# eMWu94/ReMo3D

Hardware: AMD Instinct MI355X
Metric: measurement points/sec (3D benchmark model) (higher is better)
Workload: dtype f64

## Files before the change

include/remo3d_hip_debug.h:

```cpp
#ifndef REMO3D_HIP_DEBUG_H
#define REMO3D_HIP_DEBUG_H

#include "remo3d_hip.h"

#ifdef __cplusplus
extern "C" {
#endif

int remo_debug_stream(remo_ctx_t *ctx, int64_t bytes, double *read_gbs, double *copy_gbs);
int remo_debug_clock(remo_ctx_t *ctx, double *gfma_per_wave);
int remo_debug_cache_gather(remo_ctx_t *ctx, int64_t bytes, double *gbs);
int remo_debug_device(remo_ctx_t *ctx, int64_t *out8);
int remo_debug_xcc(remo_ctx_t *ctx, int32_t *out, int32_t nblocks);


int remo_debug_patch_phases(remo_ctx_t *ctx, remo_batch_t *batch, int32_t fp32 , double *out16);

int remo_debug_patch_phases_p(remo_ctx_t *ctx, remo_batch_t *batch, int32_t fp32, double *out16);

int remo_debug_grid_barrier(remo_ctx_t *ctx, int32_t nblocks, int32_t nbar, double *out3);

int remo_debug_sens_timing(remo_ctx_t *ctx, double *out2);
int remo_debug_sens_group_timing(remo_ctx_t *ctx, double *out4);
int remo_debug_field_timing(remo_ctx_t *ctx, double *out2);
int remo_debug_point_location(remo_ctx_t *ctx);
int remo_debug_secondary_timing(remo_ctx_t *ctx, double *ms);

int remo_debug_tune(int32_t key, int32_t value);

#ifdef __cplusplus
}
#endif
#endif
```

remo3d_amd/_lib.py:

```python
from __future__ import annotations

import ctypes as C
import os

import numpy as np

_HERE = os.path.dirname(os.path.abspath(__file__))
LIB_PATH = os.environ.get("REMO_LIB") or os.path.join(_HERE, "libremo3d_hip.so")
REMO_MAX_RHS = 8


class RemoMesh(C.Structure):
    _fields_ = [("dim", C.c_int32), ("n_nodes", C.c_int64), ("coords", C.POINTER(C.c_double)),
                ("n_elems", C.c_int64), ("conn", C.POINTER(C.c_int32)), ("mat", C.POINTER(C.c_int32)),
                ("n_bfacets", C.c_int64), ("bconn", C.POINTER(C.c_int32)), ("bdirichlet", C.POINTER(C.c_uint8))]


class RemoOpts(C.Structure):
    _fields_ = [("preconditioner", C.c_int32), ("condense", C.c_int32), ("maxsteps", C.c_int32),
                ("check_every", C.c_int32), ("rtol", C.c_double), ("time_kernels", C.c_int32),
                ("coarse_degree", C.c_int32), ("coarse_ratio", C.c_int32), ("precision", C.c_int32), ("inner_digits", C.c_int32),
                ("serialize_solves", C.c_int32), ("op", C.c_int32), ("coarse", C.c_int32), ("assemble", C.c_int32), ("quadrature", C.c_int32)]


class RemoStats(C.Structure):
    _fields_ = [("n_dof", C.c_int64), ("n_free", C.c_int64), ("nnz", C.c_int64), ("n_edges", C.c_int64),
                ("n_faces", C.c_int64), ("n_rhs", C.c_int32), ("max_iterations", C.c_int32),
                ("iterations", C.c_int32 * REMO_MAX_RHS), ("relres", C.c_double * REMO_MAX_RHS),
                ("ms_symbolic", C.c_double), ("ms_h2d", C.c_double), ("ms_assemble", C.c_double),
                ("ms_solve", C.c_double), ("ms_eval", C.c_double), ("ms_total", C.c_double),
                ("spmv_ms", C.c_double), ("spmv_launches", C.c_int64), ("spmv_bytes", C.c_double),
                ("pcg_steps", C.c_int64), ("spmv_ms_raw", C.c_double), ("event_overhead_ms", C.c_double),
                ("refinement_cycles", C.c_int64), ("op_used", C.c_int32), ("coarse_used", C.c_int32),
                ("assembled", C.c_int32), ("patch_rounds", C.c_int32)]

    def as_dict(self):
        d = {}
        for name, _ in self._fields_:
            v = getattr(self, name)
            d[name] = list(v) if hasattr(v, "__len__") else v
        return d


class RemoJob(C.Structure):
    _dp, _ip = C.POINTER(C.c_double), C.POINTER(C.c_int32)
    _fields_ = [("size", C.c_uint32), ("tensor", C.c_int32), ("n_mat", C.c_int32), ("sigma", _dp),
                ("n_rhs", C.c_int32), ("src_ptr", _ip), ("src_p", _dp), ("src_I", _dp),
                ("eval_ptr", _ip), ("eval_p", _dp), ("u_out", _dp),
                ("n_fun", C.c_int32), ("fun_rhs", _ip), ("fun_ptr", _ip), ("fun_p", _dp), ("fun_w", _dp), ("J_out", _dp), ("dJ_out", _dp),
                ("n_group", C.c_int32), ("group", _ip), ("dJg_out", _dp),
                ("warm", C.c_void_p),
                ("n_pts", C.c_int32), ("pts", _dp), ("n_frhs", C.c_int32), ("field_rhs", _ip), ("u_f", _dp), ("grad_f", _dp), ("J_f", _dp),
                ("elem_f", _ip)]


class RemoJobSecondary(C.Structure):
    _fields_ = RemoJob._fields_ + [("secondary", C.c_int32), ("sec_quad", C.c_int32), ("sec_radius", C.c_double),
                                   ("sec_sigma0", C.POINTER(C.c_double))]


EXPORTS = ["remo_abi_version", "remo_opts_default", "remo_ctx_create", "remo_ctx_destroy", "remo_last_error",
           "remo_solve_batch", "remo_solve_batch_tensor", "remo_solve_batch_sens", "remo_solve_batch_sens_tensor", "remo_solve_batch_sens_groups", "remo_solve_batch_sens_groups_tensor",
           "remo_solve_batch_field", "remo_solve_batch_field_tensor", "remo_batch_field", "remo_host_field_element",
           "remo_warm_create", "remo_warm_destroy", "remo_warm_clear", "remo_warm_info", "remo_solve_batch_sens_warm", "remo_solve_batch_sens_warm_tensor", "remo_batch_create", "remo_batch_create_tensor", "remo_batch_run", "remo_batch_fetch", "remo_batch_destroy",
           "remo_batch_eval", "remo_batch_get_system", "remo_batch_get_vectors", "remo_batch_apply_coarse", "remo_batch_spmv",
           "remo_host_element_matrix", "remo_host_element_matrix_tensor", "remo_host_sens_element", "remo_host_factor_error", "remo_host_symbolic",
           "remo_solve_job", "remo_batch_create_job", "remo_host_point_shapes", "remo_host_secondary_element"]
DEBUG_EXPORTS = ["remo_debug_stream", "remo_debug_clock", "remo_debug_device", "remo_debug_cache_gather", "remo_debug_xcc", "remo_debug_tune", "remo_debug_patch_phases", "remo_debug_patch_phases_p", "remo_debug_grid_barrier", "remo_debug_sens_timing", "remo_debug_sens_group_timing", "remo_debug_field_timing", "remo_debug_point_location", "remo_debug_secondary_timing"]

JOB_HEAD = ["n_mat", "sigma", "n_rhs", "src_ptr", "src_p", "src_I", "eval_ptr", "eval_p"]
_SENS = ["u_out", "n_fun", "fun_rhs", "fun_ptr", "fun_p", "fun_w"]
LEGACY_MEMBERS = {"": ["u_out"],
                  "_sens": _SENS + ["J_out", "dJ_out"],
                  "_sens_warm": _SENS + ["J_out", "dJ_out", "warm"],
                  "_sens_groups": _SENS + ["n_group", "group", "J_out", "dJ_out", "dJg_out"],
                  "_field": ["u_out", "n_pts", "pts", "n_frhs", "field_rhs", "u_f", "grad_f", "J_f", "elem_f"]}


def legacy_args(job, kind=None):
    return [getattr(job, name) for name in JOB_HEAD + (LEGACY_MEMBERS[kind] if kind is not None else [])]


_lib = None


def load():
    global _lib
    if _lib is not None:
        return _lib
    if not os.path.exists(LIB_PATH):
        raise ImportError(f"{LIB_PATH} is missing: build it with `make -C remo3d_amd/csrc` "
                          "(or __graft_entry__.build()); remo3d_amd has no CPU fallback")
    L = C.CDLL(LIB_PATH)
    dp, ip, i64p, u8p = C.POINTER(C.c_double), C.POINTER(C.c_int32), C.POINTER(C.c_int64), C.POINTER(C.c_uint8)
    vp = C.c_void_p
    L.remo_abi_version.restype = C.c_int
    L.remo_opts_default.argtypes = [C.POINTER(RemoOpts)]
    L.remo_ctx_create.restype = vp
    L.remo_ctx_create.argtypes = [C.c_int]
    L.remo_ctx_destroy.argtypes = [vp]
    L.remo_last_error.restype = C.c_char_p
    L.remo_last_error.argtypes = [vp]
    member = dict(RemoJob._fields_)
    batch_args = [vp, C.POINTER(RemoMesh)] + [member[name] for name in JOB_HEAD]
    for kind, names in LEGACY_MEMBERS.items():
        for entry in (getattr(L, "remo_solve_batch" + kind), getattr(L, "remo_solve_batch" + kind + "_tensor")):
            entry.restype = C.c_int
            entry.argtypes = batch_args + [member[name] for name in names] + [C.POINTER(RemoOpts), C.POINTER(RemoStats)]
    L.remo_warm_create.restype = vp
    L.remo_warm_create.argtypes = [C.c_int]
    L.remo_warm_destroy.restype = None
    L.remo_warm_destroy.argtypes = [vp]
    L.remo_warm_clear.restype = None
    L.remo_warm_clear.argtypes = [vp]
    L.remo_warm_info.restype = C.c_int
    L.remo_warm_info.argtypes = [vp, i64p, ip, i64p, ip]
    L.remo_solve_job.restype = C.c_int
    L.remo_solve_job.argtypes = [vp, C.POINTER(RemoMesh), vp, C.POINTER(RemoOpts), C.POINTER(RemoStats)]
    L.remo_batch_create_job.restype = C.c_int
    L.remo_batch_create_job.argtypes = [vp, C.POINTER(RemoMesh), vp, C.POINTER(vp)]
    L.remo_host_point_shapes.restype = C.c_int
    L.remo_host_point_shapes.argtypes = [C.c_int32, dp, dp, dp]
    L.remo_batch_field.restype = C.c_int
    L.remo_batch_field.argtypes = [vp, vp, C.c_int32, C.c_int32, dp, dp, dp, dp, ip]
    L.remo_host_field_element.restype = C.c_int
    L.remo_host_field_element.argtypes = [C.c_int32, dp, dp, C.c_double, dp, dp, dp]
    L.remo_debug_field_timing.restype = C.c_int
    L.remo_debug_field_timing.argtypes = [vp, dp]
    L.remo_debug_point_location.restype = C.c_int
    L.remo_debug_point_location.argtypes = [vp]
    L.remo_host_secondary_element.restype = C.c_int
    L.remo_host_secondary_element.argtypes = [C.c_int32, dp, dp, C.c_double, C.c_double, C.c_double, dp, C.c_int32, dp]
    L.remo_debug_secondary_timing.restype = C.c_int
    L.remo_debug_secondary_timing.argtypes = [vp, dp]
    L.remo_debug_sens_group_timing.restype = C.c_int
    L.remo_debug_sens_group_timing.argtypes = [vp, dp]
    L.remo_host_sens_element.restype = C.c_int
    L.remo_host_sens_element.argtypes = [C.c_int32, dp, C.c_int32, dp, dp, dp]
    L.remo_debug_sens_timing.restype = C.c_int
    L.remo_debug_sens_timing.argtypes = [vp, dp]
    L.remo_batch_create.restype = C.c_int
    L.remo_batch_create.argtypes = batch_args + [C.POINTER(vp)]
    L.remo_batch_create_tensor.restype = C.c_int
    L.remo_batch_create_tensor.argtypes = batch_args + [C.POINTER(vp)]
    L.remo_batch_run.restype = C.c_int
    L.remo_batch_run.argtypes = [vp, vp, C.POINTER(RemoOpts), C.POINTER(RemoStats)]
    L.remo_batch_fetch.restype = C.c_int
    L.remo_batch_fetch.argtypes = [vp, vp, dp]
    L.remo_batch_destroy.argtypes = [vp, vp]
    L.remo_batch_eval.restype = C.c_int
    L.remo_batch_eval.argtypes = [vp, vp, C.c_int32, C.c_int32, dp, dp]
    L.remo_batch_get_system.restype = C.c_int
    L.remo_batch_get_system.argtypes = [vp, vp, ip, ip, dp, dp, ip]
    L.remo_batch_get_vectors.restype = C.c_int
    L.remo_batch_get_vectors.argtypes = [vp, vp, dp, dp, ip]
    L.remo_batch_apply_coarse.restype = C.c_int
    L.remo_batch_apply_coarse.argtypes = [vp, vp, C.c_int32, dp, dp, C.c_int32, i64p]
    L.remo_debug_patch_phases.restype = C.c_int
    L.remo_debug_patch_phases.argtypes = [vp, vp, C.c_int32, dp]
    L.remo_debug_patch_phases_p.restype = C.c_int
    L.remo_debug_patch_phases_p.argtypes = [vp, vp, C.c_int32, dp]
    L.remo_debug_grid_barrier.restype = C.c_int
    L.remo_debug_grid_barrier.argtypes = [vp, C.c_int32, C.c_int32, dp]
    L.remo_debug_xcc.restype = C.c_int
    L.remo_debug_xcc.argtypes = [vp, ip, C.c_int32]
    L.remo_debug_cache_gather.restype = C.c_int
    L.remo_debug_cache_gather.argtypes = [vp, C.c_int64, dp]
    L.remo_debug_device.restype = C.c_int
    L.remo_debug_device.argtypes = [vp, i64p]
    L.remo_debug_clock.restype = C.c_int
    L.remo_debug_clock.argtypes = [vp, dp]
    L.remo_debug_stream.restype = C.c_int
    L.remo_debug_stream.argtypes = [vp, C.c_int64, dp, dp]
    L.remo_batch_spmv.restype = C.c_int
    L.remo_batch_spmv.argtypes = [vp, vp, C.c_int32, dp, dp, C.c_int32, dp]
    L.remo_host_element_matrix.restype = C.c_int
    L.remo_host_element_matrix.argtypes = [C.c_int32, dp, C.c_double, dp]
    L.remo_host_element_matrix_tensor.restype = C.c_int
    L.remo_host_element_matrix_tensor.argtypes = [C.c_int32, dp, dp, dp]
    L.remo_host_factor_error.restype = C.c_double
    L.remo_host_symbolic.restype = C.c_int
    L.remo_host_symbolic.argtypes = [C.POINTER(RemoMesh), C.c_int32, i64p, ip, ip, ip]
    L.remo_debug_tune.restype = C.c_int
    L.remo_debug_tune.argtypes = [C.c_int32, C.c_int32]
    _lib = L
    return L


def ptr(a, t):
    return a.ctypes.data_as(C.POINTER(t))


def mesh_struct(mesh):
    coords = np.ascontiguousarray(mesh.coords, dtype=np.float64)
    conn = np.ascontiguousarray(mesh.conn, dtype=np.int32)
    mat = np.ascontiguousarray(mesh.mat, dtype=np.int32)
    bconn = np.ascontiguousarray(mesh.bconn, dtype=np.int32).reshape(-1, mesh.dim)
    bdir = np.ascontiguousarray(mesh.bdirichlet, dtype=np.uint8)
    m = RemoMesh(int(mesh.dim), coords.shape[0], ptr(coords, C.c_double), conn.shape[0], ptr(conn, C.c_int32),
                 ptr(mat, C.c_int32), bconn.shape[0], ptr(bconn, C.c_int32), ptr(bdir, C.c_uint8))
    return m, (coords, conn, mat, bconn, bdir)
```

remo3d_amd/csrc/batch_run.hip:

```cpp
#include <limits.h>

#include <algorithm>
#include <cmath>
#include <cstring>
#include <mutex>

#include "pcg_host.h"
#include "patch.h"
#include "sens.h"
#include "field.h"
#include "warm.h"
#include "secondary.h"

using namespace remo;

namespace {

std::mutex g_solve_mutex;
constexpr int64_t kCompactPerRow = 48;

struct Run {
    remo_ctx *ctx;
    remo_batch *b;
    const remo_opts_t &o;
    remo_stats_t *st;
    hipStream_t s;
    int dim, N, NT;
};

int checked_opts(remo_ctx *ctx, const remo_opts_t *opts_in, remo_opts_t &o) {
    if (opts_in) o = *opts_in; else remo_opts_default(&o);
    if (o.maxsteps <= 0 || !(o.rtol > 0.0)) return fail(ctx, REMO_ERR_ARG, "maxsteps and rtol must be positive");
    if (o.coarse < 0 || o.coarse > 3) return fail(ctx, REMO_ERR_ARG, "remo_opts_t.coarse must be 0 (by dimension), 1 (polynomial), 2 (multigrid cycle) or 3 (cycle, else polynomial)");
    if (o.op != 0 && o.op != 2 && o.op != 3)
        return fail(ctx, REMO_ERR_ARG, "remo_opts_t.op must be 0 (default), 2 (CSR product) or 3 (patch operator); 1, the round-2 element-wise operator, left the library with ABI 7");
    return REMO_OK;
}

struct Points {
    int dim = 0;
    std::vector<double> P, I;
    std::vector<double> z;
    std::vector<int32_t> rhs, chunk_begin, eval_slot;
    std::vector<std::pair<int32_t, int32_t>> fun_reads;
    int forward_chunks = 0;
    std::vector<int32_t> found_init;
    bool on_axis = true;
    FieldGrid grid{};
    size_t sort_bytes = 0, locate_bytes = 0;
    int n() const { return int(I.size()); }
};

Points gather_points(const remo_batch *b) {
    Points p;
    const int dim = p.dim = b->dim;
    auto add = [&](const std::vector<double> &from, int q, double I, int rhs, int slot) {
        p.P.insert(p.P.end(), from.begin() + size_t(q) * dim, from.begin() + size_t(q + 1) * dim);
        p.I.push_back(I); p.rhs.push_back(rhs); p.eval_slot.push_back(slot);
    };
    for (int c0 = 0; c0 < b->n_rhs; c0 += REMO_MAX_RHS) {
        p.chunk_begin.push_back(int32_t(p.n()));
        const int c1 = std::min(b->n_rhs, c0 + REMO_MAX_RHS);
        for (int r = c0; r < c1; ++r)
            for (int q = b->src_ptr[r]; q < b->src_ptr[r + 1]; ++q) add(b->src_p, q, b->src_I[q], r - c0, -1);
        for (int r = c0; r < c1; ++r)
            for (int q = b->eval_ptr[r]; q < b->eval_ptr[r + 1]; ++q) add(b->eval_p, q, 0.0, r - c0, q);
        if (const remo_sens_request *sn = b->sens)
            for (int j = 0; j < sn->n_fun; ++j)
                if (sn->fun_rhs[j] >= c0 && sn->fun_rhs[j] < c1)
                    for (int q = sn->fun_ptr[j]; q < sn->fun_ptr[j + 1]; ++q) {
                        p.fun_reads.emplace_back(int32_t(p.n()), q);
                        add(b->fun_p, q, 0.0, sn->fun_rhs[j] - c0, -1);
                    }
    }
    p.forward_chunks = int(p.chunk_begin.size());
    if (const remo_sens_request *sn = b->sens)
        for (int a0 = 0; a0 < sn->n_fun; a0 += REMO_MAX_RHS) {
            p.chunk_begin.push_back(int32_t(p.n()));
            for (int j = a0; j < std::min(sn->n_fun, a0 + REMO_MAX_RHS); ++j)
                for (int q = sn->fun_ptr[j]; q < sn->fun_ptr[j + 1]; ++q) add(b->fun_p, q, sn->fun_w[q], j - a0, -1);
        }
    p.chunk_begin.push_back(int32_t(p.n()));
    p.found_init.assign(size_t(p.n()), INT_MAX);
    for (int q = 0; q < p.n(); ++q)
        for (int k = 0; k + 1 < dim; ++k)
            if (p.P[size_t(q) * dim + k] != 0.0) p.on_axis = false;
    if (p.on_axis) {
        p.z.resize(size_t(p.n()));
        for (int q = 0; q < p.n(); ++q) p.z[size_t(q)] = p.P[size_t(q) * dim + dim - 1];
    }
    return p;
}

void plan_point_location(const remo_batch *b, Points &p) {
    if (p.on_axis || p.n() == 0) return;
    p.grid = field_grid(p.dim, p.n(), p.P.data());
    p.sort_bytes = field_sort_bytes(p.n(), p.grid.ncell);
    p.locate_bytes = field_locate_bytes(p.n(), b->nt, p.grid.ncell, p.sort_bytes);
}

struct Plan {
    int kmax = 0;
    bool x_ev_only = false;
    bool want_patch = false, want_amg = false;
    int64_t vertex_block_above = -1;
    size_t field_bytes = 0;
    size_t point_locate_bytes = 0;
    size_t secondary_bytes = 0;
    size_t arena_bytes = 0;
};

size_t arena_estimate(const remo_batch *b, const remo_opts_t &o, const Plan &p, int npts) {
    const int dim = b->dim, N = (dim == 2) ? 10 : 20, NT = (dim == 2) ? 9 : 6;
    const int64_t nt = b->nt, nv = b->nv;
    const size_t kmax = size_t(p.kmax);
    const int64_t ndof_max = nv + (dim == 2 ? 7 : 16) * nt, nnz_max = nt * int64_t(N) * N;
    size_t need = symbolic_gpu_arena_bytes(dim, nv, nt, b->nbf);
    need += size_t(nt) * NT * 8;
    need += size_t(nnz_max) * 8;
    need += size_t(ndof_max) * 8 * (1 + 5 * kmax);
    need += size_t(nv + 64) * 8 * 4 * kmax;
    if (p.want_patch)
        need += patch_arena_bytes(nt, ndof_max, p.kmax) + (size_t(nt) * 21 + 64) * kmax * 8;
    need += size_t(kMaxPartialBlocks) * 8 * 8 * 3;
    need += size_t(npts) * (N + 8) * 8;
    need += p.point_locate_bytes;
    need += p.secondary_bytes;
    need += p.field_bytes;
    need += (1 << 20);
    if (p.x_ev_only) {
        need -= size_t(ndof_max) * 8 * kmax;
        need += size_t(npts + 1) * N * 16;
    }
    need += size_t(nv + 64) * 200 * 20 + size_t(nv + 64) * 8;
    need += size_t(nv + 64) * kCompactPerRow * 16 + size_t(nv + 64) * 8;
    need += size_t(nv + 64) * kEllWidth * 12 + size_t(nv + 64) * 8;
    need += size_t(nv + 64) * (4 * 4 * kmax + 8);
    if (p.want_amg) need += size_t(nv + 64) * (dim == 2 ? 1536 : 3072) * 2 + (1 << 20);
    if (b->sens) {
        const size_t ncomp = size_t(b->sigma_comp);
        need += size_t(ndof_max) * 8 * size_t(b->n_rhs + b->sens->n_fun);
        need += size_t(b->sens->n_fun) * size_t(b->n_mat) * ncomp * 8 * (size_t(sens_grid(nt)) + 1);
        if (b->sens->group) {
            const size_t ng = size_t(b->sens->n_group);
            need += size_t(nt) * 4 * 5 + (ng + 2) * 4;
            need += sens_group_sort_bytes(nt, b->sens->n_group) + 256;
            need += size_t(nt) * ncomp * 8 + size_t(sens_group_chunks(nt)) * 2 * ncomp * 8;
            need += size_t(b->sens->n_fun) * ng * ncomp * 8 + 16 * 256;
        }
    }
    if (o.precision == 1) {
        need += size_t(nv + 64) * 200 * 8;
        need += size_t(nnz_max) * 4;
        need += size_t(ndof_max) * 4 * (1 + 5 * kmax);
        need += size_t(nv + 64) * 4 * 4 * kmax + (1 << 16);
    }
    return need;
}

Plan plan_batch(const remo_batch *b, const remo_opts_t &o, const Points &pts, size_t field_bytes, size_t secondary_bytes) {
    Plan p;
    const int dim = b->dim, npts = pts.n();
    p.field_bytes = field_bytes;
    p.secondary_bytes = secondary_bytes;
    p.point_locate_bytes = pts.on_axis ? 0 : align_up(size_t(npts + 1) * dim * 8) + align_up(pts.locate_bytes);
    p.kmax = std::min<int>(std::max(b->n_rhs, b->sens ? b->sens->n_fun : 0), REMO_MAX_RHS);
    p.x_ev_only = b->eval_only && !b->sens && !b->field && g_tune.x_ev && g_tune.x_in_direction && o.precision == 0;
    p.want_patch = dim == 3 && (o.op == 3 || o.op == 0);
    p.want_amg = o.preconditioner != 0 && g_tune.amg != 1 &&
                 (g_tune.amg == 2 || o.coarse == 2 || o.coarse == 3 || (o.coarse == 0 && dim == 2 && o.coarse_degree <= 0));
    p.vertex_block_above = (p.want_patch && o.assemble != 1) ? (o.assemble == 2 ? 0 : 200000) : -1;
    p.arena_bytes = arena_estimate(b, o, p, npts);
    return p;
}

int number_dofs(const Run &r, const Plan &plan, double t_start) {
    remo_batch *b = r.b;
    remo_stats_t *st = r.st;
    std::string err;
    DeviceSymbolic &sy = b->sym;
    int rc = build_symbolic_gpu(r.ctx->ar, r.s, r.dim, b->nv, b->nt, b->d_conn, b->nbf, b->d_bconn, b->d_bdir, r.o.condense != 0, r.ctx->d_err, sy, err,
                                plan.vertex_block_above);
    if (rc != REMO_OK) return fail(r.ctx, rc, err);
    st->ms_symbolic = now_ms() - t_start;
    st->n_dof = sy.ndof; st->n_free = sy.nfree; st->nnz = sy.vertex_block_only ? 0 : sy.nnz; st->n_edges = sy.ne; st->n_faces = sy.nf;
    st->n_rhs = b->n_rhs;
    return REMO_OK;
}

struct System {
    int64_t n = 0;
    bool lite = false;
    double *d_C = nullptr, *d_val = nullptr, *d_dinv = nullptr, *d_f = nullptr;
    const double *d_M = nullptr;
    int64_t pair_begin = 0, pair_end = 0;
    CsrView view(const DeviceSymbolic &sy) const { return CsrView{n, sy.nnz, sy.rowptr, sy.col, d_val}; }
};

System take_system(const Run &r, const Plan &plan) {
    const DeviceSymbolic &sy = r.b->sym;
    System sys;
    sys.n = sy.nfree;
    sys.lite = sy.vertex_block_only;
    sys.d_C = r.ctx->take<double>(r.b->nt * r.NT);
    sys.d_val = r.ctx->take<double>(sy.nnz + 2);
    sys.d_dinv = r.ctx->take<double>(sys.n);
    sys.d_f = r.ctx->take<double>(sys.n * plan.kmax);
    return sys;
}

void assemble_system(const Run &r, System &sys) {
    remo_batch *b = r.b;
    const DeviceSymbolic &sy = b->sym;
    const int dim = r.dim;
    sys.d_M = (dim == 2) ? (r.o.quadrature == 1 ? r.ctx->d_M2q : r.ctx->d_M2) : r.ctx->d_M3;
    b->d_M_last = sys.d_M;
    if (b->sigma_comp > 1)
        launch_metric_terms_tensor(dim, b->nt, b->d_coords, sy.conn, b->d_mat, sy.eperm, b->d_sigma, b->n_mat, sys.d_C, r.ctx->d_err, r.s);
    else
        launch_metric_terms(dim, b->nt, b->d_coords, sy.conn, b->d_mat, sy.eperm, b->d_sigma, b->n_mat, sys.d_C, r.ctx->d_err, r.s);
    if (sys.lite) {
        launch_assemble(dim, sy.condense, sy.nvfree, 0, 0, sy.rowptr, sy.col, sy.adjptr, sy.adj, sy.eldof, sys.d_C, sys.d_M, sys.d_val, sys.d_dinv, r.s);
        launch_diag_rows(dim, sy.nvfree, sys.n, sy.adjptr, sy.adj, sys.d_C, sys.d_M, sys.d_dinv, r.s);
    } else {
        if (sy.nvefree > sy.nvfree && ((sy.nvefree - sy.nvfree) & 1) == 0) { sys.pair_begin = sy.nvfree; sys.pair_end = sy.nvefree; }
        launch_assemble(dim, sy.condense, sys.n, sys.pair_begin, sys.pair_end, sy.rowptr, sy.col, sy.adjptr, sy.adj, sy.eldof, sys.d_C, sys.d_M, sys.d_val,
                        sys.d_dinv, r.s);
    }
}

struct ChebDefaults { int degree; double ratio; };

ChebDefaults cheb_defaults(int dim, int64_t nvfree) {
    const double nv_rel = double(nvfree > 0 ? nvfree : 1) / 12600.0;
    const double nv2 = double(nvfree > 0 ? nvfree : 1) / 25000.0;
    const int deg2 = 2 * int(std::min(16.0, std::max(8.0, std::floor(8.0 * std::sqrt(nv2) + 0.5))));
    int deg3 = int(std::min(16.0, std::max(5.0, std::floor(5.0 * std::sqrt(nv_rel) + 0.9))));
    if (deg3 > 8) deg3 &= ~1;
    if (dim == 3) return {deg3, std::min(1200.0, std::max(60.0, 90.0 * std::pow(nv_rel, 2.0 / 3.0)))};
    return {deg2, std::min(2400.0, std::max(600.0, 600.0 * nv2 * 1.25))};
}

struct Solve {
    PcgBuffers buf{};
    bool two_level = false;
    size_t nc = 0;
    double ratio_default = 0.0;
    unsigned long long *d_bound = nullptr;
};

void take_pcg_buffers(const Run &r, const Plan &plan, const System &sys, Solve &sv) {
    remo_ctx *ctx = r.ctx;
    const DeviceSymbolic &sy = r.b->sym;
    const int64_t n = sys.n;
    const int kmax = plan.kmax;
    PcgBuffers &buf = sv.buf;
    buf.x = plan.x_ev_only ? nullptr : ctx->take<double>(n * kmax);
    buf.r = ctx->take<double>(n * kmax);
    buf.p = ctx->take<double>(n * kmax); buf.q = ctx->take<double>(n * kmax);
    buf.dinv = sys.d_dinv;
    buf.part_pq = ctx->take<double>(kMaxPartialBlocks * 8);
    buf.part_rz = ctx->take<double>(kMaxPartialBlocks * 8 * 2);
    buf.rz0 = ctx->take<double>(kScalarSlots);
    sv.two_level = (r.o.preconditioner != 0) && sy.nvfree > 0;
    buf.nv_coarse = sv.two_level ? sy.nvfree : 0;
    const ChebDefaults cd = cheb_defaults(r.dim, sy.nvfree);
    sv.ratio_default = cd.ratio;
    buf.cheb_degree = sv.two_level ? (r.o.coarse_degree > 0 ? r.o.coarse_degree : cd.degree) : 0;
    buf.cheb_lmax = buf.cheb_lmin = 0.0;
    sv.nc = size_t(buf.nv_coarse) * kmax + 2;
    buf.cz = ctx->take<double>(sv.nc); buf.cres = ctx->take<double>(sv.nc);
    buf.cd[0] = ctx->take<double>(sv.nc); buf.cd[1] = ctx->take<double>(sv.nc);
    sv.d_bound = ctx->take<unsigned long long>(2);
}

void prepare_progress(const Run &r, PcgBuffers &buf) {
    remo_ctx *ctx = r.ctx;
    ctx->ensure_progress(r.o.maxsteps + 3);
    buf.progress = ctx->progress_dev;
    buf.progress_len = ctx->progress_len;
    if (r.o.time_kernels && ctx->spmv_ev.size() < 8192) {
        const size_t old = ctx->spmv_ev.size();
        ctx->spmv_ev.resize(8192);
        for (size_t i = old; i < ctx->spmv_ev.size(); ++i) HIP_TRY(hipEventCreate(&ctx->spmv_ev[i]));
    }
}

struct DevicePoints {
    int npts = 0;
    double *d_pz = nullptr, *d_pI = nullptr;
    int32_t *d_prhs = nullptr, *d_found = nullptr;
    double *d_phi = nullptr, *d_fint = nullptr, *d_out = nullptr;
    int64_t *d_ev_at = nullptr;
    double *d_x_ev = nullptr;
    FieldLocate loc{};
    bool full = false;
};

DevicePoints take_points(const Run &r, const Plan &plan, const Points &pts) {
    remo_ctx *ctx = r.ctx;
    const int npts = pts.n();
    DevicePoints p;
    p.npts = npts;
    p.full = !pts.on_axis;
    p.d_pz = ctx->take<double>(pts.on_axis ? size_t(npts + 1) : size_t(npts + 1) * r.dim); p.d_pI = ctx->take<double>(npts + 1);
    p.d_prhs = ctx->take<int32_t>(npts + 1); p.d_found = ctx->take<int32_t>(npts + 1);
    p.d_phi = ctx->take<double>(size_t(npts + 1) * r.N); p.d_fint = ctx->take<double>(npts + 1); p.d_out = ctx->take<double>(npts + 1);
    p.d_ev_at = plan.x_ev_only ? ctx->take<int64_t>(size_t(npts + 1) * r.N) : nullptr;
    p.d_x_ev = plan.x_ev_only ? ctx->take<double>(size_t(npts + 1) * r.N) : nullptr;
    if (!pts.on_axis && npts > 0) p.loc = field_locate_carve(ctx->take<char>(pts.locate_bytes), npts, r.b->nt, pts.grid.ncell, pts.sort_bytes);
    return p;
}

void upload_points(const Run &r, const Points &pts, const DevicePoints &dp) {
    const int npts = dp.npts;
    HIP_TRY(hipMemsetAsync(r.ctx->d_err, 0, sizeof(int32_t), r.s));
    if (npts > 0) {
        if (pts.on_axis) HIP_TRY(hipMemcpyAsync(dp.d_pz, pts.z.data(), sizeof(double) * npts, hipMemcpyHostToDevice, r.s));
        else HIP_TRY(hipMemcpyAsync(dp.d_pz, pts.P.data(), sizeof(double) * size_t(npts) * r.dim, hipMemcpyHostToDevice, r.s));
        HIP_TRY(hipMemcpyAsync(dp.d_pI, pts.I.data(), sizeof(double) * npts, hipMemcpyHostToDevice, r.s));
        HIP_TRY(hipMemcpyAsync(dp.d_prhs, pts.rhs.data(), sizeof(int32_t) * npts, hipMemcpyHostToDevice, r.s));
        HIP_TRY(hipMemcpyAsync(dp.d_found, pts.found_init.data(), sizeof(int32_t) * npts, hipMemcpyHostToDevice, r.s));
    }
}

void locate_points(const Run &r, const Points &pts, const DevicePoints &dp) {
    const remo_batch *b = r.b;
    const DeviceSymbolic &sy = b->sym;
    r.ctx->point_location = pts.on_axis ? 0 : 1;
    if (dp.npts <= 0) return;
    if (!pts.on_axis) {
        field_locate(r.dim, b->nt, b->d_coords, sy.conn, dp.npts, dp.d_pz, pts.grid, dp.loc, dp.d_found, r.s);
        launch_point_shapes_at(r.dim, dp.npts, dp.d_pz, dp.d_found, b->d_coords, sy.conn, dp.d_phi, r.ctx->d_err, r.s);
        return;
    }
    for (int q0 = 0; q0 < dp.npts; q0 += kMaxPoints)
        launch_locate(r.dim, b->nt, b->d_coords, sy.conn, std::min(kMaxPoints, dp.npts - q0), dp.d_pz + q0, dp.d_found + q0, r.s);
    launch_point_shapes(r.dim, dp.npts, dp.d_pz, dp.d_found, b->d_coords, sy.conn, dp.d_phi, r.ctx->d_err, r.s);
}

struct Secondary {
    bool on = false;
// ... 250 lines not shown
    const int kmax = plan.kmax;
    if (vb.want_compact && vb.h_vb[0] == 0 && vb.h_vb[1] > 0) { buf.vb_rowptr = vb.vb_rowptr; buf.vb_col = vb.vb_col; buf.vb_val = vb.vb_val; }
    if (sys.lite && sv.two_level) { buf.vb_rowptr = sy.rowptr; buf.vb_col = sy.col; buf.vb_val = sys.d_val; vb.h_vb[0] = 0; vb.h_vb[1] = int32_t(sy.nnz); }
    if (g_tune.chain32 && o.precision == 0 && buf.vb_rowptr && (buf.nv_coarse > 32768 || g_tune.chain32 == 2)) {
        float *v32c = ctx->take<float>(size_t(vb.h_vb[1]) + 4), *d32c = ctx->take<float>(size_t(buf.nv_coarse) + 4);
        launch_to_float(vb.h_vb[1], buf.vb_val, v32c, s);
        launch_to_float(buf.nv_coarse, sys.d_dinv, d32c, s);
        buf.c32_val = v32c; buf.c32_dinv = d32c;
        buf.c32_z = ctx->take<float>(sv.nc); buf.c32_res = ctx->take<float>(sv.nc);
        buf.c32_d[0] = ctx->take<float>(sv.nc); buf.c32_d[1] = ctx->take<float>(sv.nc);
    }
    if (g_tune.ell && sv.two_level && !plan.want_amg && !vb.want_square && r.dim == 3) {
        const int64_t nvc = buf.nv_coarse;
        const bool from_block = buf.vb_rowptr != nullptr;
        int32_t *ell_col = ctx->take<int32_t>(size_t(nvc) * kEllWidth + 8);
        int32_t *ell_tail = ctx->take<int32_t>(size_t(nvc) * 2 + 8);
        double *e64 = (o.precision == 0 && !buf.c32_val) ? ctx->take<double>(size_t(nvc) * kEllWidth + 8) : nullptr;
        float *e32 = (o.precision != 0 || buf.c32_val) ? ctx->take<float>(size_t(nvc) * kEllWidth + 8) : nullptr;
        launch_vblock_ell(nvc, from_block ? buf.vb_rowptr : sy.rowptr, from_block ? buf.vb_col : sy.col, from_block ? buf.vb_val : sys.d_val,
                          ell_col, ell_tail, e64, e32, s);
        buf.ell_col = ell_col; buf.ell_tail = ell_tail; buf.ell_val = e64; buf.c32_ell_val = e32;
    }
    if (sv.two_level && plan.want_amg) {
        std::string why;
        if (amg_setup(ctx->ar, s, r.dim, buf.nv_coarse, sy.rowptr, sy.col, sys.d_val, kmax, b->amg64, why)) buf.amg = &b->amg64;
        else if (o.coarse == 2 || g_tune.amg == 2) return fail(ctx, REMO_ERR_NUMERIC, "multigrid hierarchy of the vertex block: " + why);
    }
    if (buf.amg && (o.precision == 1 || g_tune.amg32)) {
        amg_to_float(ctx->ar, s, b->amg64, kmax, b->amg32);
        vb.amg32_ready = true;
        if (o.precision == 0) buf.amg32 = &b->amg32;
    }
    r.st->coarse_used = !sv.two_level ? 0 : (buf.amg ? 2 : 1);
    if (sv.two_level) {
        double lmax;
        std::memcpy(&lmax, &vb.h_bound, sizeof lmax);
        if (!(lmax > 0.0) || !std::isfinite(lmax)) return fail(ctx, REMO_ERR_NUMERIC, "vertex block has no positive spectrum bound");
        buf.cheb_lmax = lmax;
        buf.cheb_lmin = lmax / (o.coarse_ratio > 0 ? double(o.coarse_ratio) : sv.ratio_default);
    }
    if (vb.want_square && vb.h_sq[0] == 0) {
        buf.sq_rowptr = vb.sq_rowptr; buf.sq_col = vb.sq_col; buf.sq_a = vb.sq_a; buf.sq_b = vb.sq_b;
        const double avg = double(vb.h_sq[1]) / double(buf.nv_coarse > 0 ? buf.nv_coarse : 1);
        buf.sq_lanes = g_tune.sq_lanes ? g_tune.sq_lanes : (avg > 40.0 ? 32 : (avg > 24.0 ? 16 : 8));
    }
    return REMO_OK;
}

int choose_operator(const Run &r, const Plan &plan, const System &sys, const Solve &sv, VertexBlock &vb, bool &patch_op) {
    remo_ctx *ctx = r.ctx;
    remo_batch *b = r.b;
    const DeviceSymbolic &sy = b->sym;
    const int64_t n = sys.n;
    const int kmax = plan.kmax;
    PatchTables &ptab = vb.ptab;
    const int32_t *h_patch = vb.h_patch;
    b->A = sys.view(sy);
    b->A.pair_begin = sys.pair_begin; b->A.pair_end = sys.pair_end;
    b->A.vertex_block_only = sys.lite;
    const bool x_fits = uint64_t(n) * uint64_t(kmax) * 8 < 0xFFFFF000ull;
    const size_t patch_lds = patch_lds_bytes(h_patch[1], kmax);
    const bool patch_ok = plan.want_patch && h_patch[0] == 0 && h_patch[1] > 0 && x_fits && n < (int64_t(1) << 24) && h_patch[2] < 0x7FFFFFF0 && patch_lds <= kPatchLdsLimit;
    if (sys.lite && !patch_ok) return fail(ctx, REMO_ERR_ARG, "only the P1 block was assembled but the patch operator cannot run on this batch: rerun with remo_opts_t.assemble = 1");
    if (r.o.op == 3 && r.dim == 3 && !patch_ok) return fail(ctx, REMO_ERR_ARG, "patch operator: a patch of the element list touches more distinct rows than its tables hold (or the mesh is too large)");
    patch_op = patch_ok;
    r.st->op_used = patch_op ? 3 : 0;
    r.st->patch_rounds = patch_op ? ptab.rounds : 0;
    r.st->assembled = sys.lite ? 2 : 1;
    if (patch_op) {
        ptab.nslot_cap = h_patch[2] > 0 ? h_patch[2] : 1;
        b->patch64 = PatchOpT<double>{ptab, ctx->take<double>(size_t(ptab.nslot_cap) * size_t(kmax) + 8), ctx->take<double>(size_t(ptab.npatch) * 8 + 8), h_patch[1]};
        b->A.patch = &b->patch64;
    }
    b->d_val = sys.d_val;
    b->d_dinv = sys.d_dinv;
    b->d_x = sv.buf.x;
    b->d_f = sys.d_f;
    b->d_C = sys.d_C;
    b->k_last = 0;
    b->has_system = true;
    return REMO_OK;
}

void set_launch_shape(const Run &r, const System &sys, bool patch_op, PcgBuffers &buf) {
    remo_batch *b = r.b;
    const int lpr = choose_lanes_per_row(sys.n, b->sym.nnz);
    buf.nb_spmv = spmv_grid(sys.n, lpr);
    buf.nb_vec = vec_grid(sys.n);
    buf.defer_q = patch_op && g_tune.defer_q && !pcg_update_folds(buf);
    buf.x_in_direction = g_tune.x_in_direction != 0;
    buf.pq_bins = buf.defer_q && g_tune.dot_bins != 0;
    if (patch_op) b->patch64.dot_bins = buf.pq_bins;
}

MixedBuffers mixed_buffers(const Run &r, const Plan &plan, const System &sys, const Solve &sv, const VertexBlock &vb, bool patch_op) {
    remo_ctx *ctx = r.ctx;
    remo_batch *b = r.b;
    hipStream_t s = r.s;
    const DeviceSymbolic &sy = b->sym;
    const PcgBuffers &buf = sv.buf;
    const size_t nk = size_t(sys.n) * plan.kmax;
    MixedBuffers mx;
    float *v32 = ctx->take<float>(size_t(sy.nnz) + 2);
    float *dinv32 = ctx->take<float>(size_t(sys.n));
    launch_to_float(sy.nnz, sys.d_val, v32, s);
    launch_to_float(sys.n, sys.d_dinv, dinv32, s);
    mx.A32 = CsrViewT<float>{sys.n, sy.nnz, sy.rowptr, sy.col, v32};
    mx.A32.pair_begin = b->A.pair_begin; mx.A32.pair_end = b->A.pair_end; mx.A32.vertex_block_only = sys.lite;
    PcgBuffersT<float> &f = mx.b32;
    f.x = ctx->take<float>(nk); f.r = ctx->take<float>(nk);
    f.p = ctx->take<float>(nk + 4); f.q = ctx->take<float>(nk);
    mx.f32 = ctx->take<float>(nk);
    f.dinv = dinv32;
    f.part_pq = buf.part_pq; f.part_rz = buf.part_rz; f.rz0 = buf.rz0;
    f.nv_coarse = buf.nv_coarse; f.cheb_degree = buf.cheb_degree; f.cheb_lmax = buf.cheb_lmax; f.cheb_lmin = buf.cheb_lmin;
    f.cz = ctx->take<float>(sv.nc); f.cres = ctx->take<float>(sv.nc);
    f.cd[0] = ctx->take<float>(sv.nc); f.cd[1] = ctx->take<float>(sv.nc);
    f.progress = buf.progress; f.progress_len = buf.progress_len;
    f.nb_spmv = buf.nb_spmv; f.nb_vec = buf.nb_vec;
    if (buf.amg && vb.amg32_ready) f.amg = &b->amg32;
    if (buf.vb_rowptr) {
        float *vb32 = ctx->take<float>(size_t(vb.h_vb[1]) + 1);
        launch_to_float(vb.h_vb[1], buf.vb_val, vb32, s);
        f.vb_rowptr = buf.vb_rowptr; f.vb_col = buf.vb_col; f.vb_val = vb32;
    }
    f.ell_col = buf.ell_col; f.ell_tail = buf.ell_tail; f.ell_val = buf.c32_ell_val;
    if (buf.sq_rowptr) {
        float *a32 = ctx->take<float>(size_t(vb.h_sq[1]) + 1), *b32 = ctx->take<float>(size_t(vb.h_sq[1]) + 1);
        launch_to_float(vb.h_sq[1], buf.sq_a, a32, s);
        launch_to_float(vb.h_sq[1], buf.sq_b, b32, s);
        f.sq_rowptr = buf.sq_rowptr; f.sq_col = buf.sq_col; f.sq_a = a32; f.sq_b = b32; f.sq_lanes = buf.sq_lanes;
    }
    f.defer_q = buf.defer_q; f.x_in_direction = buf.x_in_direction; f.pq_bins = buf.pq_bins;
    if (patch_op) {
        b->patch32 = patch_view32(b->patch64);
        b->patch32.dot_bins = f.pq_bins;
        mx.A32.patch = &b->patch32;
    }
    return mx;
}

struct RunTotals {
    int ret = REMO_OK;
    size_t ev_used = 0;
    float ms_solve = 0.f, ms_eval = 0.f;
};

int solve_chunk(const Run &r, const Plan &plan, const System &sys, const DevicePoints &dp, Solve &sv, MixedBuffers *mx, int k, int q0, int nq,
                std::vector<double> &h_out, RunTotals &tot, double *x_prev = nullptr, const Secondary *sec = nullptr, int chunk = 0) {
    remo_ctx *ctx = r.ctx;
    remo_batch *b = r.b;
    remo_stats_t *st = r.st;
    hipStream_t s = r.s;
    const DeviceSymbolic &sy = b->sym;
    const int dim = r.dim, N = r.N;
    PcgBuffers &buf = sv.buf;
    HIP_TRY(hipEventRecord(ctx->ev[4], s));
    HIP_TRY(hipMemsetAsync(sys.d_f, 0, sizeof(double) * sys.n * k, s));
    if (sec) {
        if (nq > 0) HIP_TRY(hipMemsetAsync(dp.d_fint + q0, 0, sizeof(double) * nq, s));
        build_secondary_rhs(r, sys, *sec, chunk, k);
    } else if (nq > 0)
        launch_build_rhs(dim, sy.condense, nq, dp.d_prhs + q0, dp.d_pI + q0, dp.d_found + q0, dp.d_phi + size_t(q0) * N, sy.eldof, sys.d_C, sys.d_M, k,
                         sys.d_f, dp.d_fint + q0, s);
    if (plan.x_ev_only) {
        launch_eval_slots(dim, sy.condense, nq, dp.d_prhs + q0, dp.d_found + q0, sy.eldof, k, dp.d_ev_at, s);
        if (nq > 0) HIP_TRY(hipMemsetAsync(dp.d_x_ev, 0, sizeof(double) * size_t(nq) * N, s));
        buf.x_ev_at = dp.d_ev_at; buf.x_ev = dp.d_x_ev; buf.x_ev_n = nq * N;
    }
    HIP_TRY(hipEventRecord(ctx->ev[5], s));
    ChunkResult cr = mx ? run_pcg_mixed(ctx, b->A, k, sys.d_f, buf, *mx, r.o, st, tot.ev_used)
                        : (x_prev ? run_pcg_warm(ctx, b->A, k, sys.d_f, buf, x_prev, r.o, st, tot.ev_used) : run_pcg(ctx, b->A, k, sys.d_f, buf, r.o, st, tot.ev_used));
    HIP_TRY(hipEventRecord(ctx->ev[6], s));
    if (nq > 0)
        launch_eval(dim, sy.condense, nq, dp.d_prhs + q0, dp.d_pI + q0, dp.d_found + q0, dp.d_phi + size_t(q0) * N, sy.eldof, sys.d_C, sys.d_M, k, buf.x,
// ... 175 lines not shown
    if (!b) return fail(ctx, REMO_ERR_ARG, "null batch");
    remo_opts_t o;
    if (int rc = checked_opts(ctx, opts_in, o)) return rc;
    remo_stats_t local;
    if (!st) st = &local;
    std::memset(st, 0, sizeof *st);
    std::fill(b->u_out.begin(), b->u_out.end(), std::nan(""));
    if (b->sens) {
        if (o.precision == 1) return fail(ctx, REMO_ERR_ARG, "sensitivities are computed in fp64: remo_opts_t.precision = 1 (mixed) is not supported by remo_solve_batch_sens");
        if (int64_t(b->n_mat) * b->sigma_comp > kSensMaxAcc) return fail(ctx, REMO_ERR_ARG, "too many materials for the sensitivity contraction");
    }
    if (b->secondary) {
        if (o.precision == 1) return fail(ctx, REMO_ERR_ARG, "the secondary formulation is fp64: remo_opts_t.precision = 1 (mixed) is not supported with remo_job_secondary_t.secondary");
        if (b->sens || b->field || b->warm) return fail(ctx, REMO_ERR_ARG, "remo_job_secondary_t.secondary does not combine with functionals, groups, a warm object or field points");
        ctx->sec_ms = 0.0;
    }
    if (b->field && o.precision == 1)
        return fail(ctx, REMO_ERR_ARG, "field sections are formed from the fp64 solution: remo_opts_t.precision = 1 (mixed) is not supported by remo_solve_batch_field");
    b->has_system = false;
    b->amg64 = AmgT<double>{};
    b->amg32 = AmgT<float>{};
    b->run_id = ++ctx->run_id;
    const double t_start = now_ms();
    try {
        HIP_TRY(hipSetDevice(ctx->device));
        const Run r{ctx, b, o, st, ctx->stream, b->dim, (b->dim == 2) ? 10 : 20, (b->dim == 2) ? 9 : 6};
        hipStream_t s = r.s;

        Points points = gather_points(b);
        const int npts = points.n();
        for (double c : points.P)
            if (!std::isfinite(c)) return fail(ctx, REMO_ERR_POINT, "non-finite point coordinate");
        plan_point_location(b, points);
        Field fld = field_plan(b);
        Secondary sec;
        if (int rc = plan_secondary(ctx, b, sec)) return rc;
        const int kmax_plan = std::min<int>(std::max(b->n_rhs, b->sens ? b->sens->n_fun : 0), REMO_MAX_RHS);
        const Plan plan = plan_batch(b, o, points, fld.bytes(b->dim), sec.bytes(b, kmax_plan));
        ctx->reserve(plan.arena_bytes);

        if (int rc = number_dofs(r, plan, t_start)) return rc;
        System sys = take_system(r, plan);
        Solve sv;
        take_pcg_buffers(r, plan, sys, sv);
        const DevicePoints dp = take_points(r, plan, points);
        take_secondary(r, plan, sec);
        field_take(r, fld);
        prepare_progress(r, sv.buf);
        HIP_TRY(hipEventRecord(ctx->ev[0], s));
        upload_points(r, points, dp);
        upload_secondary(r, sec);
        HIP_TRY(hipEventRecord(ctx->ev[1], s));
        assemble_system(r, sys);
        HIP_TRY(hipEventRecord(ctx->ev[2], s));
        locate_points(r, points, dp);
        check_secondary_sources(r, sec);
        field_locate_points(r, fld);
        HIP_TRY(hipEventRecord(ctx->ev[3], s));
        VertexBlock vb;
        vertex_block_enqueue(r, plan, sys, sv, vb);
        HIP_TRY(hipStreamSynchronize(s));
        patch_tables_one_round(r, plan, sys, vb);

        if (int rc = vertex_block_accept(r, plan, sys, sv, vb)) return rc;
        if (vb.h_err & 1) return fail(ctx, REMO_ERR_MESH, "degenerate element or material index out of range");
        if (vb.h_err & 2) return fail(ctx, REMO_ERR_POINT, "source or evaluation point outside the mesh");
        if (vb.h_err & 4) return fail(ctx, REMO_ERR_POINT, "secondary formulation: a source lies in or on an element whose conductivity differs from sigma0 (the integrand is singular there)");
        bool patch_op = false;
        if (int rc = choose_operator(r, plan, sys, sv, vb, patch_op)) return rc;
        const Sens sens = b->sens ? sens_take(r, sys) : Sens{};
        remo_warm *warm = b->sens ? b->warm : nullptr;
        Sens prev{};
        bool warm_hit = false;
        if (warm) {
            warm_hit = warm_matches(warm, b, o.condense != 0, sys.n);
            warm->filled = false;
            warm->used_last = warm_hit ? 1 : 0;
            if (!warm_hit) warm_reserve(warm, warm_doubles(sys.n, b->n_rhs, b->sens->n_fun));
            prev.keep = warm->d;
        }

        std::unique_lock<std::mutex> solve_turn(g_solve_mutex, std::defer_lock);
        if (o.serialize_solves) solve_turn.lock();
        set_launch_shape(r, sys, patch_op, sv.buf);
        const bool mixed = (o.precision == 1);
        MixedBuffers mx;
        if (mixed) mx = mixed_buffers(r, plan, sys, sv, vb, patch_op);
        std::vector<double> h_out(npts, std::nan(""));
        RunTotals tot;
        int chunk = 0;
        for (int c0 = 0; c0 < b->n_rhs; c0 += REMO_MAX_RHS, ++chunk) {
            const int k = std::min(b->n_rhs - c0, REMO_MAX_RHS);
            const int q0 = points.chunk_begin[chunk], nq = points.chunk_begin[chunk + 1] - q0;
            if (b->sens) b->d_x = sv.buf.x = sens.block(sys.n, b->n_rhs, false, chunk);
            if (int rc = solve_chunk(r, plan, sys, dp, sv, mixed ? &mx : nullptr, k, q0, nq, h_out, tot,
                                     warm_hit ? prev.block(sys.n, b->n_rhs, false, chunk) : nullptr, sec.on ? &sec : nullptr, chunk)) return rc;
            if (b->field) field_eval_chunk(r, sys, dp, sv.buf.x, fld, c0, k, q0, nq);
        }
        if (b->field) field_fetch(r, fld);
        for (int q = 0; q < npts; ++q)
            if (points.eval_slot[q] >= 0) b->u_out[points.eval_slot[q]] = h_out[q];
        if (const remo_sens_request *rq = b->sens) {
            for (int a0 = 0, ca = 0; a0 < rq->n_fun; a0 += REMO_MAX_RHS, ++ca, ++chunk) {
                const int k = std::min(rq->n_fun - a0, REMO_MAX_RHS);
                const int q0 = points.chunk_begin[chunk], nq = points.chunk_begin[chunk + 1] - q0;
                b->d_x = sv.buf.x = sens.block(sys.n, b->n_rhs, true, ca);
                if (int rc = solve_chunk(r, plan, sys, dp, sv, nullptr, k, q0, nq, h_out, tot, warm_hit ? prev.block(sys.n, b->n_rhs, true, ca) : nullptr)) return rc;
            }
            if (warm) {
                if (!warm_hit) HIP_TRY(hipMemcpyAsync(warm->d, sens.keep, sizeof(double) * (warm_doubles(sys.n, b->n_rhs, rq->n_fun) - 64), hipMemcpyDeviceToDevice, s));
                warm_label(warm, b, o.condense != 0, sys.n);
            }
            std::vector<double> h_dJ;
            sens_contract(r, sys, dp, points, sens, h_dJ);
            for (int j = 0; j < rq->n_fun; ++j) rq->J_out[j] = 0.0;
            for (const auto &fr : points.fun_reads) {
                int j = 0;
                while (fr.second >= rq->fun_ptr[j + 1]) ++j;
                rq->J_out[j] += rq->fun_w[fr.second] * h_out[fr.first];
            }
            if (!h_dJ.empty()) std::memcpy(rq->dJ_out, h_dJ.data(), sizeof(double) * h_dJ.size());
        }
        fill_timing_stats(r, plan, sys, mixed, patch_op, tot);
        st->ms_total = now_ms() - t_start;
        if (tot.ret == REMO_NOT_CONVERGED) ctx->err = "PCG did not reach rtol within maxsteps";
        return tot.ret;
    } catch (const std::exception &ex) {
        std::fill(b->u_out.begin(), b->u_out.end(), std::nan(""));
        return fail(ctx, REMO_ERR_DEVICE, ex.what());
    }
}
```

remo3d_amd/csrc/kernels.h:

```cpp
#pragma once
#include <hip/hip_runtime.h>
#include <stdint.h>

namespace remo {

constexpr int kMaxPartialBlocks = 1024;
constexpr int kMaxPoints = 256;

struct PcgProgress {
    double rz[8];
    int32_t step;
    int32_t pad;
};

template <class T> struct AmgT;

template <class T> struct PcgBuffersT {
    T *x, *r, *p, *q;
    const T *dinv;
    double *part_pq;
    double *part_rz;
    double *rz0;
    int64_t nv_coarse;
    int cheb_degree;
    double cheb_lmax, cheb_lmin;
    T *cz, *cres;
    T *cd[2];
    const int32_t *sq_rowptr = nullptr, *sq_col = nullptr;
    const T *sq_a = nullptr, *sq_b = nullptr;
    int sq_lanes = 16;
    const int32_t *vb_rowptr = nullptr, *vb_col = nullptr;
    const T *vb_val = nullptr;
    const float *c32_val = nullptr, *c32_dinv = nullptr;
    const int32_t *ell_col = nullptr, *ell_tail = nullptr;
    const T *ell_val = nullptr;
    const float *c32_ell_val = nullptr;
    float *c32_z = nullptr, *c32_res = nullptr, *c32_d[2] = {nullptr, nullptr};
    const AmgT<T> *amg = nullptr;
    const AmgT<float> *amg32 = nullptr;
    bool defer_q = false;
    bool x_in_direction = false;
    bool pq_bins = false;
    const int64_t *x_ev_at = nullptr;
    T *x_ev = nullptr;
    int x_ev_n = 0;
    PcgProgress *progress;
    int progress_len;
    int nb_spmv, nb_vec;
};
using PcgBuffers = PcgBuffersT<double>;
constexpr int kPqBins = 256;
constexpr int kScalarSlots = 48;
constexpr int kDoneSlot = 4 * 8;

struct PatchTables {
    int64_t nt = 0, n = 0, npatch = 0;
    int E = 0;
    int rows_cap = 0;
    int block = 256;
    int trim = 1;
    int spread = 4;
    const uint16_t *lidx = nullptr;
    const int32_t *pcount = nullptr;
    const int32_t *prow = nullptr;
    const int32_t *pout = nullptr;
    const int32_t *pboff = nullptr;
    int all_slab = 1;
    const int32_t *row4 = nullptr;
    const int32_t *bptr = nullptr;
    const int32_t *bslot = nullptr;
    const double *C = nullptr;
    int64_t nslot_cap = 0;
    int stagger = 0;
    int rounds = 1;
};
template <class T> struct PatchOpT {
    PatchTables t;
    T *Yb = nullptr;
    double *ppart = nullptr;
    int lds_rows = 0;
    bool dot_bins = false;
};
#ifndef REMO_PATCH_PASSES
#define REMO_PATCH_PASSES 12
#endif
constexpr int kPatchPasses = REMO_PATCH_PASSES;
constexpr int kPatchBlock = 256;
inline size_t patch_lds_bytes(int lds_rows, int k) { return size_t(lds_rows + 2) * size_t(k) * 8; }
constexpr size_t kPatchLdsLimit = 63 * 1024;


template <class T> struct CsrViewT {
    int64_t n;
    int64_t nnz;
    const int32_t *rowptr;
    const int32_t *col;
    const T *val;
    int64_t pair_begin = 0, pair_end = 0;
    const PatchOpT<T> *patch = nullptr;
    bool vertex_block_only = false;
};
using CsrView = CsrViewT<double>;

void launch_metric_terms(int dim, int64_t nt, const double *coords, const int32_t *conn, const int32_t *mat, const int32_t *eperm ,
                         const double *sigma, int nmat, double *C, int32_t *errflag, hipStream_t s);
void launch_metric_terms_tensor(int dim, int64_t nt, const double *coords, const int32_t *conn, const int32_t *mat, const int32_t *eperm ,
                                const double *sigma_tensor, int nmat, double *C, int32_t *errflag, hipStream_t s);
void launch_diag_rows(int dim, int64_t row0, int64_t nfree, const int32_t *adjptr, const uint32_t *adj, const double *C, const double *M, double *dinv, hipStream_t s);
void launch_assemble(int dim, bool condense, int64_t nfree, int64_t pair_begin, int64_t pair_end, const int32_t *rowptr, const int32_t *col,
                     const int32_t *adjptr, const uint32_t *adj, const int32_t *eldof, const double *C,
                     const double *M, double *val, double *dinv, hipStream_t s);

int spmv_grid(int64_t n, int lanes_per_row);
int vec_grid(int64_t n);
void set_fold_first(int v);
void set_spmm_tuning(int key, int value);
int choose_lanes_per_row(int64_t n, int64_t nnz);
template <class T> bool patch_applies(const CsrViewT<T> &A, int k);
template <class T> void launch_spmm(const CsrViewT<T> &A, int k, const T *x, T *y, double *part, const double *scal, int nblocks, hipStream_t s, int step = 0, bool defer = false);

template <class T> void launch_patch_spmm(const CsrViewT<T> &A, int k, const T *x, T *y, double *part, const double *scal, int nblocks, hipStream_t s, int step, bool defer);
template <class T> bool pcg_update_folds(const PcgBuffersT<T> &b);
void set_slab_masked(int v);
void set_flat_direction(int v);
void set_tile_update(int v);
void set_slab_ahead(int v);

template <class T> void launch_pcg_init(const CsrViewT<T> &A, int k, const T *f, const PcgBuffersT<T> &b, hipStream_t s);
template <class T> void launch_pcg_update(const CsrViewT<T> &A, int k, int step, double tol2, const PcgBuffersT<T> &b, hipStream_t s);
template <class T> void launch_pcg_direction(const CsrViewT<T> &A, int k, int step, double tol2, const PcgBuffersT<T> &b, hipStream_t s, bool add_x = true);
template <class T> void launch_pcg_final(int k, int step, const PcgBuffersT<T> &b, hipStream_t s);
void launch_vblock_bound(int64_t nv, const CsrView &A, const double *dinv, unsigned long long *out_bits, hipStream_t s);
constexpr int kSquareSlots = 512;
void launch_vblock_square(int64_t nv, const CsrView &A, const double *dinv, int32_t *sq_rowptr, int32_t *sq_col, double *sq_a, double *sq_b,
                          int64_t capacity, int32_t *flag, hipStream_t s);
int cheb_grid(int64_t nv);

void launch_barrier_probe(int nblocks, int nbar, unsigned *counter, int *fail, float *buf, int *mismatch, hipStream_t s);
constexpr int kEllWidth = 24;
void launch_vblock_ell(int64_t nv, const int32_t *rowptr, const int32_t *col, const double *val, int32_t *ecol, int32_t *tail, double *eval64,
                       float *eval32, hipStream_t s);


void launch_to_float(int64_t n, const double *src, float *dst, hipStream_t s);
void launch_vblock_compact(int64_t nv, const CsrView &A, int32_t *vb_rowptr, int32_t *vb_col, double *vb_val, int64_t capacity, int32_t *flag,
                           hipStream_t s);
void launch_mixed_residual(int64_t n, const double *f, const double *q , float *r32, hipStream_t s);
void launch_mixed_accumulate(int64_t n, double *x, float *e, int zero_e, hipStream_t s);
void launch_pcg_replace(const CsrViewT<float> &A, const CsrViewT<double> &A64, int k, int step, double tol2, const PcgBuffersT<float> &b,
                        const double *f64, double *x64, double *q64, hipStream_t s);

void launch_locate(int dim, int64_t nt, const double *coords, const int32_t *conn, int npts, const double *pz,
                   int32_t *found, hipStream_t s);
void launch_point_shapes(int dim, int npts, const double *pz, const int32_t *found, const double *coords,
                         const int32_t *conn, double *phi, int32_t *errflag, hipStream_t s);
void launch_point_shapes_at(int dim, int npts, const double *pp, const int32_t *found, const double *coords,
                            const int32_t *conn, double *phi, int32_t *errflag, hipStream_t s);
void launch_build_rhs(int dim, bool condense, int npts, const int32_t *pt_rhs, const double *pt_I,
                      const int32_t *found, const double *phi, const int32_t *eldof, const double *C,
                      const double *M, int k, double *f, double *fint, hipStream_t s);
void launch_eval(int dim, bool condense, int npts, const int32_t *pt_rhs, const double *pt_I, const int32_t *found,
                 const double *phi, const int32_t *eldof, const double *C, const double *M, int k,
                 const double *x, const double *fint, double *out, hipStream_t s, const double *x_ev = nullptr,
                 const double *fbub = nullptr);
void launch_eval_slots(int dim, bool condense, int npts, const int32_t *pt_rhs, const int32_t *found, const int32_t *eldof, int k,
                       int64_t *at, hipStream_t s);

}
```

remo3d_amd/csrc/patch.hip:

```cpp
#include <hip/hip_runtime.h>
#include <limits.h>

#include <rocprim/device/device_scan.hpp>

#include "kernels.h"
#include "kutil.h"
#include "patch.h"
#include <stdexcept>
#include <type_traits>
#include "symbolic_gpu.h"
#include "wave_util.h"

#define REMO_ELEM_NS elem_tables_patch
#include "build/elem_apply.inc"

namespace remo {

namespace {

constexpr int kPatchDotBlocks = 32;
constexpr uint32_t kSlotBits = 13;
constexpr uint64_t kNoRow = uint64_t(0x7FFFFFFF);

__global__ void __launch_bounds__(256) k_patch_row_slots(int64_t n, int E, const int32_t *__restrict__ adjptr, const uint32_t *__restrict__ adj,
// ... 25 lines not shown
        if (j < nslots) {
            const int32_t r = eldof[e0 * 20 + j];
            k = ((r >= 0 ? uint64_t(uint32_t(r)) : kNoRow) << kSlotBits) | uint64_t(j);
        }
        keys[j] = k;
    }
    for (int size = 2; size <= npad; size <<= 1)
        for (int stride = size >> 1; stride > 0; stride >>= 1) {
            __syncthreads();
            for (int t = tid; t < npad / 2; t += 256) {
                const int lo = 2 * t - (t & (stride - 1)), hi = lo + stride;
                const bool up = (lo & size) == 0;
                const uint64_t a = keys[lo], b = keys[hi];
                if ((a > b) == up) { keys[lo] = b; keys[hi] = a; }
            }
        }
    __syncthreads();
    const int per = npad / 256, j0 = tid * per;
    auto row_at = [&](int j) -> uint64_t { return keys[j] >> kSlotBits; };
    int heads = 0;
    for (int j = j0; j < j0 + per; ++j) {
        const uint64_t r = row_at(j);
        heads += (j < nslots && r < kNoRow && (j == 0 || row_at(j - 1) != r)) ? 1 : 0;
    }
    cnts[tid] = heads;
    __syncthreads();
    int before = 0, total = 0;
    for (int t = 0; t < 256; ++t) { const int c = cnts[t]; before += t < tid ? c : 0; total += c; }
    if (tid == 0) {
        pcount[p] = total;
        atomicMax(max_rows, total);
        if (total > rows_cap) atomicOr(flag, 1);
        pbcnt[p] = ((total < rows_cap ? total : rows_cap) + 15) & ~15;
    }
    int id = before - 1;
    for (int j = j0; j < j0 + per && j < nslots; ++j) {
        const uint64_t r = row_at(j);
        const int slot = int(keys[j] & ((uint64_t(1) << kSlotBits) - 1));
        if (r >= kNoRow) { lidx[e0 * 20 + slot] = 0xFFFF; continue; }
        const bool head = (j == 0 || row_at(j - 1) != r);
        id += head ? 1 : 0;
        lidx[e0 * 20 + slot] = uint16_t(id < 0xFFFF ? id : 0xFFFE);
        if (head && id < rows_cap) prow[p * rows_cap + id] = int32_t(r);
    }
}

__global__ void __launch_bounds__(256) k_patch_zero_rows(int64_t nslots, uint16_t *__restrict__ lidx, const int32_t *__restrict__ max_rows) {
    const uint16_t z = uint16_t(max_rows[0] < 0xFFFF ? max_rows[0] : 0xFFFE);
    for (int64_t j = int64_t(blockIdx.x) * blockDim.x + threadIdx.x; j < nslots; j += int64_t(gridDim.x) * blockDim.x)
        if (lidx[j] == 0xFFFF) lidx[j] = z;
}

__global__ void __launch_bounds__(256) k_patch_slots(int E, int rows_cap, const int32_t *__restrict__ pcount, const int32_t *__restrict__ pboff,
                                                     const int32_t *__restrict__ prow, int32_t *__restrict__ pout, const int32_t *__restrict__ adjptr,
                                                     const uint32_t *__restrict__ adj, const int32_t *__restrict__ bptr, int32_t *__restrict__ bslot,
                                                     int32_t *__restrict__ row4) {
    const int64_t p = blockIdx.x;
    const int mp = pcount[p] < rows_cap ? pcount[p] : rows_cap;
    for (int m = threadIdx.x; m < mp; m += 256) {
        const int32_t row = prow[p * rows_cap + m], slot = pboff[p] + m;
        int32_t last = -1, rank = 0;
        for (int32_t a = adjptr[row]; a < adjptr[row + 1]; ++a) {
            const int32_t q = int32_t((adj[a] >> 5) / uint32_t(E));
            if (q >= p) break;
            rank += q != last;
            last = q;
        }
        pout[p * rows_cap + m] = slot;
        bslot[bptr[row] + rank] = slot;
        const int32_t cnt = bptr[row + 1] - bptr[row];
        if (rank < 3 || (rank == 3 && cnt <= 4)) row4[int64_t(row) * 4 + rank] = slot;
        else if (rank == 3) row4[int64_t(row) * 4 + 3] = -2;
    }
}

template <class T> __device__ __forceinline__ void lds_add(T *p, T v) {
    (void)__hip_atomic_fetch_add(p, v, __ATOMIC_RELAXED, __HIP_MEMORY_SCOPE_WORKGROUP);
}

#ifndef REMO_LEAN_WAVES
#define REMO_LEAN_WAVES 5
#endif
constexpr int kPatchPasses2 = 20;
template <class T, int K, int MODE = 0, bool LEAN = false, int ROUNDS = 1>
__global__ void __launch_bounds__(kPatchBlock, (LEAN ? REMO_LEAN_WAVES : 1)) k_patch_apply(PatchTables tb, int rows, const T *__restrict__ x, T *__restrict__ y, T *__restrict__ Yb,
                                                     double *__restrict__ ppart, const double *__restrict__ scal, int step, long long *__restrict__ stamps,
                                                     double *__restrict__ pbins) {
    (void)y;
    int done_word = 0;
    if (scal) done_word = load_as_vector(reinterpret_cast<const int *>(scal + kDoneSlot));
#define REMO_STAMP(k) if constexpr (MODE == 4) { if (threadIdx.x == 0) stamps[(int64_t(blockIdx.x) << 3) + (k)] = __builtin_readcyclecounter(); }
    REMO_STAMP(0)
    constexpr int NL = K;
    static_assert(ROUNDS == 1 || (ROUNDS == 2 && MODE == 0 && !LEAN), "two rounds: the plain order of the product only");
    constexpr int U = ROUNDS == 2 ? kPatchPasses2 : kPatchPasses;
    constexpr int BLK = kPatchBlock;
    constexpr int EK = BLK / K;
    constexpr uint32_t S = sizeof(T);
    extern __shared__ double lds_raw[];
    T *xs = reinterpret_cast<T *>(lds_raw);
    __shared__ double smem[16 * K];
    const int tid = threadIdx.x;
    const int64_t per = (tb.npatch + 7) >> 3;
    const int64_t p = int64_t(blockIdx.x & 7) * per + int64_t(blockIdx.x >> 3);
    if (p >= tb.npatch) return;
    const int32_t *prow = tb.prow + p * tb.rows_cap;
    const int el = tid / NL, c0 = tid - el * NL;
    const int32_t off_mask = tid < EK * K ? 0 : int32_t(0x80000000);
    const rsrc_t rpr = make_rsrc(prow, uint64_t(tb.rows_cap) * 4);
    int32_t r0[U];
    const int rows_own_v = load_as_vector(tb.pcount + p);
    const int slab0_v = load_as_vector(tb.pboff + p);
#pragma unroll
    for (int u = 0; u < U; ++u) {
        int32_t t[1];
        buf_load<int32_t, 1>(rpr, off_mask == 0 ? uint32_t(el + EK * u) * 4u : kOutOfRange, t);
        r0[u] = t[0];
    }
    const int R = tb.spread > 1 ? tb.spread : 1;
    const int EL = ROUNDS == 2 ? (tb.E >> 1) : tb.E;
    const int run = el % R, base = EL / R, extra = EL % R;
    const int elp = R > 1 ? (run * base + (run < extra ? run : extra) + el / R) : el;
    const int64_t e = p * tb.E + elp;
    const bool active = el < EL && e < tb.nt;
    const int64_t eB = e + EL;
    const bool activeB = ROUNDS == 2 && el < EL && eB < tb.nt;
    uint32_t li[10];
    double cm[6];
#pragma unroll
    for (int q = 0; q < 10; ++q) li[q] = 0u;
#pragma unroll
    for (int q = 0; q < 6; ++q) cm[q] = 0.0;
    const rsrc_t rli = make_rsrc(tb.lidx, uint64_t(tb.nt) * 40), rcm = make_rsrc(tb.C, uint64_t(tb.nt) * 48);
    buf_load<uint32_t, 10>(rli, active ? uint32_t(e) * 40u : kOutOfRange, li);
    if constexpr (!(LEAN && MODE != 2)) buf_load<double, 6>(rcm, active ? uint32_t(e) * 48u : kOutOfRange, cm);
    uint32_t liB[ROUNDS == 2 ? 10 : 1];
    double cmB[ROUNDS == 2 ? 6 : 1];
    if constexpr (ROUNDS == 2) {
#pragma unroll
        for (int q = 0; q < 10; ++q) liB[q] = 0u;
#pragma unroll
        for (int q = 0; q < 6; ++q) cmB[q] = 0.0;
        buf_load<uint32_t, 10>(rli, activeB ? uint32_t(eB) * 40u : kOutOfRange, liB);
        buf_load<double, 6>(rcm, activeB ? uint32_t(eB) * 48u : kOutOfRange, cmB);
    }
    const int rows_own = __builtin_amdgcn_readfirstlane(rows_own_v);
    if (__builtin_amdgcn_readfirstlane(done_word) != 0 && __builtin_amdgcn_readfirstlane(done_word) <= step) return;
    const int rows_p = (tb.trim && rows_own < rows) ? rows_own : rows;
    const int npass = (rows_p + EK - 1) / EK;
    REMO_STAMP(1)
    const rsrc_t rx = make_rsrc(x, uint64_t(tb.n) * K * S);
    const uint32_t slack = uint32_t((rows + 1) * K + c0);
#define REMO_PASSES_UP_TO_12(fn)                                                                                          \
        case 1: fn(std::integral_constant<int, 1>{}, 0); break;   case 2: fn(std::integral_constant<int, 2>{}, 0); break;   \
        case 3: fn(std::integral_constant<int, 3>{}, 0); break;   case 4: fn(std::integral_constant<int, 4>{}, 0); break;   \
        case 5: fn(std::integral_constant<int, 5>{}, 0); break;   case 6: fn(std::integral_constant<int, 6>{}, 0); break;   \
        case 7: fn(std::integral_constant<int, 7>{}, 0); break;   case 8: fn(std::integral_constant<int, 8>{}, 0); break;   \
        case 9: fn(std::integral_constant<int, 9>{}, 0); break;   case 10: fn(std::integral_constant<int, 10>{}, 0); break; \
        case 11: fn(std::integral_constant<int, 11>{}, 0); break; case 12: fn(std::integral_constant<int, 12>{}, 0); break;
#define REMO_PASSES(fn)                                                                                                   \
    if constexpr (ROUNDS == 2) {                                                                                          \
        switch (npass) {                                                                                                  \
            REMO_PASSES_UP_TO_12(fn)                                                                                      \
            case 13: fn(std::integral_constant<int, 13>{}, 0); break; case 14: fn(std::integral_constant<int, 14>{}, 0); break; \
            case 15: fn(std::integral_constant<int, 15>{}, 0); break; case 16: fn(std::integral_constant<int, 16>{}, 0); break; \
            case 17: fn(std::integral_constant<int, 17>{}, 0); break; case 18: fn(std::integral_constant<int, 18>{}, 0); break; \
            case 19: fn(std::integral_constant<int, 19>{}, 0); break; case 20: fn(std::integral_constant<int, 20>{}, 0); break; \
            default:                                                                                                      \
                for (int m0 = 0; m0 < rows_p; m0 += U * EK) fn(std::integral_constant<int, U>{}, m0);                     \
        }                                                                                                                 \
    } else {                                                                                                              \
        switch (npass) {                                                                                                  \
            REMO_PASSES_UP_TO_12(fn)                                                                                      \
            default:                                                                                                      \
                for (int m0 = 0; m0 < rows_p; m0 += U * EK) fn(std::integral_constant<int, U>{}, m0);                     \
        }                                                                                                                 \
    }
    static_assert(kPatchPasses == 12 && kPatchPasses2 == 20, "REMO_PASSES lists the cases 1 .. U");
    auto stage = [&](auto np_c, int m0) {
        constexpr int NP = decltype(np_c)::value;
        int32_t r[NP];
        T v[NP][1];
        if (m0 == 0) {
#pragma unroll
            for (int u = 0; u < NP; ++u) r[u] = r0[u];
        } else {
#pragma unroll
            for (int u = 0; u < NP; ++u) {
                int32_t t[1];
                buf_load<int32_t, 1>(rpr, off_mask == 0 ? uint32_t(m0 + el + EK * u) * 4u : kOutOfRange, t);
                r[u] = t[0];
            }
        }
#pragma unroll
        for (int u = 0; u < NP; ++u) r[u] = (off_mask == 0 && m0 + el + EK * u < rows_own) ? r[u] : -1;
#pragma unroll
        for (int u = 0; u < NP; ++u)
            buf_load<T, 1>(rx, r[u] >= 0 ? __umul24(uint32_t(r[u]), K * S) + uint32_t(c0) * S : kOutOfRange, v[u]);
#pragma unroll
        for (int u = 0; u < NP; ++u) xs[r[u] >= 0 ? uint32_t((m0 + el + EK * u) * K + c0) : slack] = v[u][0];
    };
    REMO_PASSES(stage)
    if (tid < 2 * K) xs[rows * K + tid] = T(0);
    __syncthreads();
    REMO_STAMP(2)
    double d0 = 0.0;
    double *ya = lds_raw;
#define REMO_PATCH_L(i) ((li[(i) >> 1] >> (16 * ((i) & 1))) & 0xFFFFu)
    if constexpr (LEAN && MODE != 2) {
        typedef const T __attribute__((address_space(4))) *ctab_t;
        ctab_t tgi = (ctab_t)ElemTables2<T>::grad_in(), tdo = (ctab_t)ElemTables2<T>::div_out();
        if constexpr (sizeof(T) == 8) { asm volatile("" : "+s"(tgi)); asm volatile("" : "+s"(tdo)); }
        T g[30];
#define REMO_PATCH_XL(i) xs[REMO_PATCH_L(i) * K + c0]
#define REMO_BAR_ON __builtin_amdgcn_sched_barrier(0);
#define REMO_BAR_OFF
        if constexpr (sizeof(T) == 4) { REMO_ELEM_GRAD_IN(T, REMO_PATCH_XL, g, tgi, REMO_BAR_ON) }
        else { REMO_ELEM_GRAD_IN(T, REMO_PATCH_XL, g, tgi, REMO_BAR_OFF) }
#undef REMO_PATCH_XL
#pragma unroll
        for (int j = 0; j < 30; ++j) asm volatile("" : "+v"(g[j]));
        __builtin_amdgcn_sched_barrier(0);
        if (active) {
            const double *ce = tb.C + e * 6;
#pragma unroll
            for (int q = 0; q < 6; ++q) cm[q] = ce[q];
        }
        __syncthreads();
        REMO_STAMP(3)
        for (int j = 2 * tid; j < rows_p * K; j += 2 * BLK) { ya[j] = 0.0; ya[j + 1] = 0.0; }
        if (tid < K) ya[rows * K + tid] = 0.0;
        __syncthreads();
        REMO_STAMP(4)
        if (active) {
            const T c11 = T(cm[0]), c12 = T(cm[1]), c13 = T(cm[2]), c22 = T(cm[3]), c23 = T(cm[4]), c33 = T(cm[5]);
            T dd = T(0);
#pragma unroll
            for (int m = 0; m < 10; ++m) {
                const T g1 = g[m], g2 = g[10 + m], g3 = g[20 + m];
                const T h1 = c11 * g1 + c12 * g2 + c13 * g3, h2 = c12 * g1 + c22 * g2 + c23 * g3, h3 = c13 * g1 + c23 * g2 + c33 * g3;
                dd += g1 * h1 + g2 * h2 + g3 * h3;
                g[m] = h1; g[10 + m] = h2; g[20 + m] = h3;
            }
            d0 = double(dd);
            if constexpr (sizeof(T) == 8) {
                const uint32_t *pl2 = reinterpret_cast<const uint32_t *>(tb.lidx + e * 20);
#pragma unroll
                for (int q = 0; q < 10; ++q) li[q] = __builtin_nontemporal_load(pl2 + q);
            }
#define REMO_PATCH_EMIT(i, v) { if constexpr (MODE == 1) ya[REMO_PATCH_L(i) * K + c0] = double(v); else lds_add(ya + REMO_PATCH_L(i) * K + c0, double(v)); }
            if constexpr (sizeof(T) == 4) { REMO_ELEM_DIV_OUT(T, g, tdo, REMO_PATCH_EMIT, REMO_BAR_ON) }
            else { REMO_ELEM_DIV_OUT(T, g, tdo, REMO_PATCH_EMIT, REMO_BAR_OFF) }
#undef REMO_PATCH_EMIT
#undef REMO_BAR_ON
#undef REMO_BAR_OFF
        }
    } else if constexpr (ROUNDS == 2) {
        typedef const T __attribute__((address_space(4))) *ctab_t;
        ctab_t tgrad = (ctab_t)ElemTables<T>::grad(), tdiv = (ctab_t)ElemTables<T>::div();
        if constexpr (sizeof(T) == 8) { asm volatile("" : "+s"(tgrad)); asm volatile("" : "+s"(tdiv)); }
        auto element = [&](const T (&xe)[20], const double (&ce)[6], T (&ye)[20]) -> double {
            const T c11 = T(ce[0]), c12 = T(ce[1]), c13 = T(ce[2]), c22 = T(ce[3]), c23 = T(ce[4]), c33 = T(ce[5]);
            T g[30];
            REMO_ELEM_GRAD(T, xe, g, tgrad)
            T dd = T(0);
#pragma unroll
            for (int m = 0; m < 10; ++m) {
                const T g1 = g[m], g2 = g[10 + m], g3 = g[20 + m];
                const T h1 = c11 * g1 + c12 * g2 + c13 * g3, h2 = c12 * g1 + c22 * g2 + c23 * g3, h3 = c13 * g1 + c23 * g2 + c33 * g3;
                dd += g1 * h1 + g2 * h2 + g3 * h3;
                g[m] = h1; g[10 + m] = h2; g[20 + m] = h3;
            }
            REMO_ELEM_DIV(T, g, ye, tdiv)
            return double(dd);
        };
        auto emit = [&](int64_t ee, const T (&ye)[20]) {
            uint32_t lq[10];
            const uint32_t *pl2 = reinterpret_cast<const uint32_t *>(tb.lidx + ee * 20);
#pragma unroll
            for (int q = 0; q < 10; ++q) lq[q] = __builtin_nontemporal_load(pl2 + q);
#pragma unroll
            for (int i = 0; i < 20; ++i) lds_add(ya + ((lq[i >> 1] >> (16 * (i & 1))) & 0xFFFFu) * K + c0, double(ye[i]));
        };
        T yA[20], xB[20];
        double dA = 0.0;
        if (active) {
            T xA[20];
#pragma unroll
            for (int i = 0; i < 20; ++i) xA[i] = xs[REMO_PATCH_L(i) * K + c0];
            dA = element(xA, cm, yA);
#pragma unroll
            for (int i = 0; i < 20; ++i) asm volatile("" : "+v"(yA[i]));
        }
        if (activeB) {
#pragma unroll
            for (int i = 0; i < 20; ++i) xB[i] = xs[((liB[i >> 1] >> (16 * (i & 1))) & 0xFFFFu) * K + c0];
        }
        __syncthreads();
        REMO_STAMP(3)
        for (int j = 2 * tid; j < rows_p * K; j += 2 * BLK) { ya[j] = 0.0; ya[j + 1] = 0.0; }
        if (tid < K) ya[rows * K + tid] = 0.0;
        __syncthreads();
        REMO_STAMP(4)
        if (active) emit(e, yA);
        d0 = dA;
        if (activeB) {
            T yB[20];
            d0 += element(xB, cmB, yB);
            emit(eB, yB);
        }
    } else {
    T xv[20];
    if (active) {
#pragma unroll
        for (int i = 0; i < 20; ++i) xv[i] = xs[REMO_PATCH_L(i) * K + c0];
    }
    __syncthreads();
    REMO_STAMP(3)
    for (int j = 2 * tid; j < rows_p * K; j += 2 * BLK) { ya[j] = 0.0; ya[j + 1] = 0.0; }
    if (tid < K) ya[rows * K + tid] = 0.0;
    __syncthreads();
    REMO_STAMP(4)
    if (active) {
        const T c11 = T(cm[0]), c12 = T(cm[1]), c13 = T(cm[2]), c22 = T(cm[3]), c23 = T(cm[4]), c33 = T(cm[5]);
        T g[30], yv[20];
        if constexpr (MODE == 2) {
#pragma unroll
            for (int i = 0; i < 20; ++i) yv[i] = xv[i] * c11;
        } else {
            typedef const T __attribute__((address_space(4))) *ctab_t;
            ctab_t tgrad = (ctab_t)ElemTables<T>::grad(), tdiv = (ctab_t)ElemTables<T>::div();
            if constexpr (sizeof(T) == 8) { asm volatile("" : "+s"(tgrad)); asm volatile("" : "+s"(tdiv)); }
            REMO_ELEM_GRAD(T, xv, g, tgrad)
            T dd = T(0);
#pragma unroll
            for (int m = 0; m < 10; ++m) {
                const T g1 = g[m], g2 = g[10 + m], g3 = g[20 + m];
                const T h1 = c11 * g1 + c12 * g2 + c13 * g3, h2 = c12 * g1 + c22 * g2 + c23 * g3, h3 = c13 * g1 + c23 * g2 + c33 * g3;
                dd += g1 * h1 + g2 * h2 + g3 * h3;
                g[m] = h1; g[10 + m] = h2; g[20 + m] = h3;
            }
            d0 = double(dd);
            REMO_ELEM_DIV(T, g, yv, tdiv)
        }
        {
            const uint32_t *pl2 = reinterpret_cast<const uint32_t *>(tb.lidx + e * 20);
#pragma unroll
            for (int q = 0; q < 10; ++q) li[q] = __builtin_nontemporal_load(pl2 + q);
        }
#pragma unroll
        for (int i = 0; i < 20; ++i) {
            const uint32_t l = REMO_PATCH_L(i);
            if constexpr (MODE == 1) ya[l * K + c0] = double(yv[i]);
            else lds_add(ya + l * K + c0, double(yv[i]));
        }
    }
    }
#undef REMO_PATCH_L
    __syncthreads();
    REMO_STAMP(5)
    if (MODE != 3) {
        constexpr int VEC = 16 / int(S);
        const rsrc_t rp = make_rsrc(Yb + int64_t(__builtin_amdgcn_readfirstlane(slab0_v)) * K, uint64_t(rows_own) * K * S);
        auto put = [&](auto np_c, int m0) {
            constexpr int NP = decltype(np_c)::value;
            constexpr int NQ = (NP * EK * K + VEC * BLK - 1) / (VEC * BLK);
            T v[NQ][VEC];
#pragma unroll
            for (int q = 0; q < NQ; ++q) {
                const int j = m0 * K + VEC * (tid + BLK * q);
#pragma unroll
                for (int i = 0; i < VEC; ++i) v[q][i] = T(ya[j + i]);
            }
#pragma unroll
            for (int q = 0; q < NQ; ++q) buf_store<T, VEC>(rp, uint32_t(m0 * K + VEC * (tid + BLK * q)) * S, v[q]);
        };
        REMO_PASSES(put)
    }
    REMO_STAMP(6)
    if (ppart) {
        double dot[K];
#pragma unroll
        for (int c = 0; c < K; ++c) dot[c] = (c == c0) ? d0 : 0.0;
        const double mine = block_sum_column<K>(dot, smem);
        if (tid < K) {
            if (pbins) (void)__hip_atomic_fetch_add(pbins + (p % kPqBins) * K + tid, mine, __ATOMIC_RELAXED, __HIP_MEMORY_SCOPE_AGENT);
            else ppart[p * K + tid] = mine;
        }
    }
    REMO_STAMP(7)
#undef REMO_STAMP
#undef REMO_PASSES
#undef REMO_PASSES_UP_TO_12
}

template <class T, int K, bool DOT>
__global__ void __launch_bounds__(256) k_patch_reduce(int64_t n, int64_t npatch, const int32_t *__restrict__ bptr, const int32_t *__restrict__ bslot,
                                                      const T *__restrict__ Yb,
// ... 115 lines not shown
    int32_t *row4 = ar.lo<int32_t>(size_t(n) * 4 + 4);
    (void)hipMemsetAsync(row4, 0xFF, sizeof(int32_t) * size_t(n) * 4, s);
    const size_t mark = ar.hi_mark();
    int32_t *bcnt = ar.hi<int32_t>(size_t(n) + 2);
    int32_t *pboff = ar.lo<int32_t>(size_t(out.npatch) + 2);
    int32_t *pbcnt = ar.hi<int32_t>(size_t(out.npatch) + 2);
    (void)hipMemsetAsync(flag_and_max, 0, 3 * sizeof(int32_t), s);
    (void)hipMemsetAsync(prow, 0xFF, sizeof(int32_t) * (size_t(out.npatch) * rows_cap + 1), s);
    (void)hipMemsetAsync(pbcnt + out.npatch, 0, sizeof(int32_t), s);
    hipLaunchKernelGGL(k_patch_row_slots, dim3(int((n + 1 + 255) / 256)), dim3(256), 0, s, n, E, sy.adjptr, sy.adj, bcnt);
    hipLaunchKernelGGL(k_patch_build, dim3(int(out.npatch)), dim3(256), size_t(npad) * 8, s, nt, E, rows_cap, npad, sy.eldof, lidx, pcount, pbcnt,
                       prow, flag_and_max, flag_and_max + 1);
    size_t tb1 = 0, tb2 = 0;
    (void)rocprim::exclusive_scan(nullptr, tb1, bcnt, bptr, int32_t(0), size_t(n + 1), rocprim::plus<int32_t>(), s);
    (void)rocprim::exclusive_scan(nullptr, tb2, pbcnt, pboff, int32_t(0), size_t(out.npatch + 1), rocprim::plus<int32_t>(), s);
    void *tmp = ar.hi<char>((tb1 > tb2 ? tb1 : tb2) + 256);
    (void)rocprim::exclusive_scan(tmp, tb1, bcnt, bptr, int32_t(0), size_t(n + 1), rocprim::plus<int32_t>(), s);
    (void)rocprim::exclusive_scan(tmp, tb2, pbcnt, pboff, int32_t(0), size_t(out.npatch + 1), rocprim::plus<int32_t>(), s);
    hipLaunchKernelGGL(k_patch_zero_rows, dim3(1024), dim3(256), 0, s, nt * 20, lidx, (const int32_t *)(flag_and_max + 1));
    hipLaunchKernelGGL(k_patch_slots, dim3(int(out.npatch)), dim3(256), 0, s, E, rows_cap, (const int32_t *)pcount, (const int32_t *)pboff, (const int32_t *)prow, pout,
                       sy.adjptr, sy.adj, (const int32_t *)bptr, bslot, row4);
    (void)hipMemcpyAsync(flag_and_max + 2, pboff + out.npatch, sizeof(int32_t), hipMemcpyDeviceToDevice, s);
    ar.hi_release(mark);
    out.lidx = lidx; out.pcount = pcount; out.prow = prow; out.pout = pout; out.pboff = pboff; out.row4 = row4; out.bptr = bptr; out.bslot = bslot;
}

template <class T, int K> static void patch_dispatch(const CsrViewT<T> &A, const T *x, T *y, double *part, const double *scal, int step, int nb, hipStream_t s, bool defer) {
    const PatchOpT<T> &P = *A.patch;
    const PatchTables &tb = P.t;
    const int64_t per = (tb.npatch + 7) / 8;
    double *pp = part ? P.ppart : nullptr;
    double *bins = (part && defer && P.dot_bins) ? part + (step & 1) * (kPqBins * 8) : nullptr;
    auto launch = [&](auto kernel) {
        const size_t bytes = patch_lds_bytes(P.lds_rows, K);
        hipLaunchKernelGGL(kernel, dim3(int(per * 8)), dim3(kPatchBlock), bytes, s, tb, P.lds_rows, x, y, P.Yb, pp, scal, step, g_patch_stamps, bins);
    };
    bool launched = false;
#ifdef REMO_PROBES
    launched = launch_patch_persistent<T, K>(P, g_patch_mode, g_patch_stamps, x, y, pp, scal, step, bins, s);
    if constexpr (K == 5) {
        if (!launched && tb.rounds == 1 && g_patch_mode >= 1 && g_patch_mode <= 3 + (g_patch_stamps ? 1 : 0)) {
            launched = true;
            if (g_patch_mode == 1) launch(k_patch_apply<T, 5, 1>);
            else if (g_patch_mode == 2) launch(k_patch_apply<T, 5, 2>);
            else if (g_patch_mode == 3) launch(k_patch_apply<T, 5, 3>);
            else launch(k_patch_apply<T, 5, 4>);
        }
    }
    if (!launched && tb.rounds == 1 && ((g_patch_lean == 1) != (sizeof(T) == 4)) && g_patch_lean >= 0) {
        if (sizeof(T) == 4) launch(k_patch_apply<T, K, 0>); else launch(k_patch_apply<T, K, 0, true>);
        launched = true;
    }
#endif
    if (!launched) {
        if constexpr (sizeof(T) == 4) {
            if (tb.rounds != 1) throw std::logic_error("patch operator: tables of two rounds in fp32 storage (they are built for fp64 solves only)");
            launch(k_patch_apply<T, K, 0, true>);
        } else {
            if (tb.rounds == 2) launch(k_patch_apply<T, K, 0, false, 2>);
            else launch(k_patch_apply<T, K, 0>);
        }
    }
    if (bins) return;
    if (part && defer) {
        hipLaunchKernelGGL(k_patch_dot<K>, dim3(nb < kPatchDotBlocks ? nb : kPatchDotBlocks), dim3(256), 0, s, tb.npatch, (const double *)P.ppart, part, scal, step);
        return;
    }
    if (part) hipLaunchKernelGGL((k_patch_reduce<T, K, true>), dim3(nb), dim3(256), 0, s, A.n, tb.npatch, tb.bptr, tb.bslot, (const T *)P.Yb, y, (const double *)P.ppart, part, scal, step);
    else hipLaunchKernelGGL((k_patch_reduce<T, K, false>), dim3(nb), dim3(256), 0, s, A.n, tb.npatch, tb.bptr, tb.bslot, (const T *)P.Yb, y, (const double *)nullptr, part, scal, step);
}

template <class T> void launch_patch_spmm(const CsrViewT<T> &A, int k, const T *x, T *y, double *part, const double *scal, int nb, hipStream_t s, int step, bool defer) {
    switch (k) {
        case 1: patch_dispatch<T, 1>(A, x, y, part, scal, step, nb, s, defer); break;
        case 2: patch_dispatch<T, 2>(A, x, y, part, scal, step, nb, s, defer); break;
        case 3: patch_dispatch<T, 3>(A, x, y, part, scal, step, nb, s, defer); break;
        case 4: patch_dispatch<T, 4>(A, x, y, part, scal, step, nb, s, defer); break;
        case 5: patch_dispatch<T, 5>(A, x, y, part, scal, step, nb, s, defer); break;
        case 6: patch_dispatch<T, 6>(A, x, y, part, scal, step, nb, s, defer); break;
        case 7: patch_dispatch<T, 7>(A, x, y, part, scal, step, nb, s, defer); break;
        default: patch_dispatch<T, 8>(A, x, y, part, scal, step, nb, s, defer); break;
    }
}
template void launch_patch_spmm<double>(const CsrViewT<double> &, int, const double *, double *, double *, const double *, int, hipStream_t, int, bool);
template void launch_patch_spmm<float>(const CsrViewT<float> &, int, const float *, float *, double *, const double *, int, hipStream_t, int, bool);

}
```

remo3d_amd/csrc/pcg_host.hip:

```cpp
#include <atomic>
#include <cmath>
#include <cstring>
#include <thread>
#include <type_traits>

#include "pcg_host.h"
#include "warm.h"

namespace remo {

namespace {

struct RefineHooks {
    const CsrView *A64 = nullptr;
    const double *f64 = nullptr;
    double *x64 = nullptr, *q64 = nullptr;
    double factor2 = 1e-6;
    int replacements = 0;
};

template <class T>
ChunkResult run_pcg_t(remo_ctx *ctx, const CsrViewT<T> &A, int k, const T *d_f, PcgBuffersT<T> &buf, double tol2, const double *floor,
                      int maxit, int check, int time_kernels, remo_stats_t *st, size_t &ev_used, double *rz_first, double *rz_last,
                      RefineHooks *hooks = nullptr) {
    ChunkResult res;
    bool replace_next = false, have_ref = false;
    double rz_ref[REMO_MAX_RHS] = {0};
    hipStream_t s = ctx->stream;
    if (check <= 0) check = 10;
    for (int i = 0; i < ctx->progress_len; ++i) ctx->progress[i].step = -1;
    std::atomic_thread_fence(std::memory_order_seq_cst);
    HIP_TRY(hipMemsetAsync(buf.rz0, 0, kScalarSlots * sizeof(double), s));
    if (buf.defer_q) HIP_TRY(hipMemsetAsync(buf.part_pq, 0, sizeof(double) * kMaxPartialBlocks * 8, s));
    if (floor) {
        std::memcpy(ctx->floor_stage, floor, sizeof(double) * REMO_MAX_RHS);
        HIP_TRY(hipMemcpyAsync(buf.rz0 + 5 * 8, ctx->floor_stage, sizeof(double) * REMO_MAX_RHS, hipMemcpyHostToDevice, s));
    }
    launch_pcg_init(A, k, d_f, buf, s);
    volatile int32_t *done_step = &ctx->progress[ctx->progress_len - 1].step;
    int step = 0;
    bool done = false;
    for (; step < maxit && !done;) {
        if (time_kernels > 0 && (step % time_kernels) == (time_kernels / 2) && ev_used + 2 <= ctx->spmv_ev.size()) {
            HIP_TRY(hipEventRecord(ctx->spmv_ev[ev_used], s));
            launch_spmm(A, k, (const T *)buf.p, buf.q, buf.part_pq, (const double *)buf.rz0, buf.nb_spmv, s, step, buf.defer_q);
            HIP_TRY(hipEventRecord(ctx->spmv_ev[ev_used + 1], s));
            ev_used += 2;
        } else {
            launch_spmm(A, k, (const T *)buf.p, buf.q, buf.part_pq, (const double *)buf.rz0, buf.nb_spmv, s, step, buf.defer_q);
        }
#ifdef REMO_PROBES
        for (int extra = 0; extra < g_tune.extra_apply; ++extra)
            launch_spmm(A, k, (const T *)buf.p, buf.q, (double *)nullptr, (const double *)buf.rz0, buf.nb_spmv, s, step, false);
#endif
        bool replaced = false;
        if constexpr (std::is_same<T, float>::value) {
            if (hooks && replace_next) {
                launch_pcg_replace(A, *hooks->A64, k, step, tol2, buf, hooks->f64, hooks->x64, hooks->q64, s);
                hooks->replacements += 1;
                replace_next = false;
                replaced = true;
            }
        }
        if (!replaced) launch_pcg_update(A, k, step, tol2, buf, s);
        launch_pcg_direction(A, k, step, tol2, buf, s, !replaced);
        ++step;
        if (*done_step >= 0) { done = true; break; }
        if (step % check == 0) {
            const int target = step - check;
            if (target >= 0) {
                volatile int32_t *flag = &ctx->progress[target % (ctx->progress_len - 1)].step;
                const double t0 = now_ms();
                int spins = 0;
                while (*flag != target && *done_step < 0) {
                    if (++spins > 64) {
                        std::this_thread::yield();
                        if (now_ms() - t0 > 2000.0) {
                            HIP_TRY(hipStreamSynchronize(s));
                            if (*flag != target && *done_step < 0) throw std::runtime_error("PCG progress record not visible to the host");
                        }
                    }
                }
                std::atomic_thread_fence(std::memory_order_acquire);
                if (*done_step >= 0) { done = true; break; }
                const PcgProgress &pr = ctx->progress[target % (ctx->progress_len - 1)];
                for (int c = 0; c < k; ++c)
                    if (!std::isfinite(pr.rz[c])) { res.finite = false; done = true; }
                if (hooks) {
                    if (!have_ref) {
                        for (int c = 0; c < k; ++c) rz_ref[c] = pr.rz[c];
                        have_ref = true;
                    } else {
                        bool hit = false;
                        for (int c = 0; c < k; ++c)
                            if (rz_ref[c] > 0.0 && pr.rz[c] > 0.0 && pr.rz[c] <= hooks->factor2 * rz_ref[c]) hit = true;
                        if (hit) {
                            replace_next = true;
                            for (int c = 0; c < k; ++c) rz_ref[c] = pr.rz[c];
                        }
                    }
                }
            }
        }
    }
    launch_pcg_final(k, step, buf, s);
    HIP_TRY(hipStreamSynchronize(s));
    std::atomic_thread_fence(std::memory_order_acquire);
    const PcgProgress &dn = ctx->progress[ctx->progress_len - 1];
    const int last = (dn.step >= 0) ? dn.step : step;
    const PcgProgress &fin = (dn.step >= 0) ? dn : ctx->progress[step % (ctx->progress_len - 1)];
    res.steps = (dn.step >= 0) ? dn.step : step;
    const PcgProgress &p0 = (last == 0) ? fin : ctx->progress[0];
    res.converged = true;
    for (int c = 0; c < k; ++c) {
        res.iters[c] = last;
        const double r0 = p0.rz[c];
        const double thr = std::max(tol2 * r0, floor ? floor[c] : 0.0);
        for (int i = 0; i <= last; ++i) {
            const PcgProgress &pr = (i == last) ? fin : ctx->progress[i % (ctx->progress_len - 1)];
            if (i != last && pr.step != i) continue;
            if (!std::isfinite(pr.rz[c])) res.finite = false;
            if (!(pr.rz[c] > thr)) { res.iters[c] = i; break; }
        }
        const double rl = fin.rz[c];
        res.relres[c] = (r0 > 0.0) ? std::sqrt(rl / r0) : 0.0;
        if (rl > thr) res.converged = false;
        if (!std::isfinite(rl)) res.finite = false;
        if (rz_first) rz_first[c] = r0;
        if (rz_last) rz_last[c] = rl;
    }
    if (st) st->pcg_steps += res.steps;
    return res;
}

}
// ... 75 lines not shown
```

remo3d_amd/csrc/pcg_kernels.hip:

```cpp
#include "kernels.h"
#include "amg.h"

#include <math.h>

#include "wave_util.h"
#include "kutil.h"

namespace remo {

#ifdef REMO_PROBES
constexpr bool kProbes = true;
#else
constexpr bool kProbes = false;
#endif

__device__ __forceinline__ void publish_progress(PcgProgress *pr, const double *rz, int k, int step) {
    for (int c = 0; c < k; ++c) __hip_atomic_store(&pr->rz[c], rz[c], __ATOMIC_RELAXED, __HIP_MEMORY_SCOPE_SYSTEM);
    __asm__ volatile("s_waitcnt vmcnt(0)" ::: "memory");
    __hip_atomic_store(&pr->step, step, __ATOMIC_RELAXED, __HIP_MEMORY_SCOPE_SYSTEM);
}


template <class T> struct ChebArgsT {
    int64_t nv;
    double inv_theta;
    T *z, *res;
    T *d0;
};
template <class T> struct QViewT {
    const int32_t *bptr = nullptr, *bslot = nullptr;
    const T *Yb = nullptr;
    int skip_x = 0;
    const int32_t *row4 = nullptr;
    uint64_t slab_bytes = 0;
};
template <class T> struct EvSlotsT {
    const int64_t *at = nullptr;
    T *x = nullptr;
    int n = 0;
};
template <class T> struct FoldArgsT {
    int nb_flat = 0;
    const int32_t *rowptr = nullptr, *col = nullptr;
    const T *val = nullptr;
    T *d_new = nullptr, *stage = nullptr;
    double c1 = 0.0, c2 = 0.0;
};
template <class T> struct UpdHeadT {
    int step = 0;
    double tol2 = 0.0;
    int nb_spmv = 0, nb_rz = 0;
    const double *part_pq = nullptr, *part_rz_cur = nullptr;
    double *rz0 = nullptr;
    PcgProgress *progress = nullptr;
    int progress_len = 0;
    double *clear_bins = nullptr;
    EvSlotsT<T> ev;
};
constexpr int kFloorSlot = 5 * 8;

template <class T, int K>
__global__ void __launch_bounds__(256) k_pcg_init(int64_t n, ChebArgsT<T> ch, const T *__restrict__ f, const T *__restrict__ dinv,
                                                  T *__restrict__ x, T *__restrict__ r, T *__restrict__ p,
                                                  double *__restrict__ part_rz) {
    __shared__ double smem[16 * K];
    double rz[K];
#pragma unroll
    for (int c = 0; c < K; ++c) rz[c] = 0.0;
    for (int64_t i = int64_t(blockIdx.x) * blockDim.x + threadIdx.x; i < n; i += int64_t(gridDim.x) * blockDim.x) {
        const T d = dinv[i];
        const bool coarse = i < ch.nv;
#pragma unroll
        for (int c = 0; c < K; ++c) {
            const T ri = f[i * K + c];
            const T zi = d * ri;
            if (x) x[i * K + c] = T(0);
            r[i * K + c] = ri;
            p[i * K + c] = coarse ? T(0) : zi;
            rz[c] += coarse ? 0.0 : double(ri) * double(zi);
        }
    }
    block_sum<K>(rz, smem);
    if (threadIdx.x < K) part_rz[blockIdx.x * K + threadIdx.x] = rz[threadIdx.x];
}


template <class T, int K>
__device__ __forceinline__ bool pcg_update_head(const UpdHeadT<T> &hd, const T *__restrict__ p, double (&alpha)[K], double *smem ) {
    double *scal = hd.rz0;
    const int step = hd.step;
    if (solve_done(scal, step)) return false;
    double pq[K], rz[K], unused[K];
    if (step == 0) {
        reduce_partials3<K>(hd.part_pq, hd.nb_spmv, hd.part_rz_cur, hd.nb_rz, nullptr, 0, pq, rz, unused, smem);
    } else {
        reduce_partials<K>(hd.part_pq, hd.nb_spmv, pq, smem);
#pragma unroll
        for (int c = 0; c < K; ++c) rz[c] = scal[16 + 8 * (step & 1) + c];
    }
#pragma unroll
    for (int c = 0; c < K; ++c) {
        const double r0 = (step == 0) ? rz[c] : hd.rz0[c];
        const bool live = (rz[c] > hd.tol2 * r0) && (rz[c] > scal[kFloorSlot + c]) && (pq[c] > 0.0);
        alpha[c] = live ? rz[c] / pq[c] : 0.0;
    }
    if (blockIdx.x == 0 && threadIdx.x == 0) {
        bool any_live = false;
#pragma unroll
        for (int c = 0; c < K; ++c) any_live |= (alpha[c] != 0.0);
        if (!any_live) {
            reinterpret_cast<int *>(scal + kDoneSlot)[0] = step + 1;
            publish_progress(hd.progress + (hd.progress_len - 1), rz, K, step);
        }
#pragma unroll
        for (int c = 0; c < K; ++c) scal[8 + c] = pq[c];
        if (step == 0)
#pragma unroll
            for (int c = 0; c < K; ++c) { hd.rz0[c] = rz[c]; scal[16 + c] = rz[c]; }
        publish_progress(hd.progress + (step % (hd.progress_len - 1)), rz, K, step);
    }
    if (hd.clear_bins) {
        for (int i = int(blockIdx.x) * int(blockDim.x) + int(threadIdx.x); i < kPqBins * K; i += int(gridDim.x) * int(blockDim.x)) hd.clear_bins[i] = 0.0;
    }
    for (int j = int(blockIdx.x) * int(blockDim.x) + int(threadIdx.x); j < hd.ev.n; j += int(gridDim.x) * int(blockDim.x)) {
        const int64_t at = hd.ev.at[j];
        if (at < 0) continue;
        const int col = int(at % K);
        double a = 0.0;
#pragma unroll
        for (int c = 0; c < K; ++c) a = (c == col) ? alpha[c] : a;
        const T xv = hd.ev.x[j], pv = p[at];
        hd.ev.x[j] = xv + T(a) * pv;
    }
    return true;
}

#ifndef REMO_UPD_UNROLL
#define REMO_UPD_UNROLL 2
#endif
template <class T, int K, bool MASKED, bool AHEAD>
__device__ __forceinline__ void pcg_update_rows(int64_t i0, int64_t n, int nb, int64_t nv, const double (&alpha)[K], const T *__restrict__ p,
                                                const T *__restrict__ q, T *__restrict__ x, T *__restrict__ r, const T *__restrict__ dinv,
                                                const QViewT<T> &qv, double *__restrict__ part_rz_next, double *smem ) {
    double acc[K];
#pragma unroll
    for (int c = 0; c < K; ++c) acc[c] = 0.0;
#pragma unroll REMO_UPD_UNROLL
    for (int64_t i = i0 + int64_t(blockIdx.x) * blockDim.x + threadIdx.x; i < n; i += int64_t(nb) * blockDim.x) {
        const T d = dinv[i];
        const bool coarse = i < nv;
        T qi[K];
        int32_t b0 = 0, b1 = 0;
        if (qv.bptr) { b0 = qv.bptr[i]; b1 = qv.bptr[i + 1]; }
        T xv[K], pv[K], rv[K];
        if (qv.skip_x) {
#pragma unroll
            for (int c = 0; c < K; ++c) { xv[c] = T(0); pv[c] = T(0); rv[c] = r[i * K + c]; }
        } else {
#pragma unroll
            for (int c = 0; c < K; ++c) { xv[c] = x[i * K + c]; pv[c] = p[i * K + c]; rv[c] = r[i * K + c]; }
        }
        if (b1 > b0) {
            constexpr int kSlabAhead = 4;
            if constexpr (AHEAD) {
                int32_t at[kSlabAhead];
#pragma unroll
                for (int j = 0; j < kSlabAhead; ++j) at[j] = qv.bslot[b0 + j < b1 ? b0 + j : b0];
                T part[kSlabAhead][K];
                if constexpr (MASKED) {
                    const rsrc_t rs = make_rsrc(qv.Yb, qv.slab_bytes);
#pragma unroll
                    for (int j = 0; j < kSlabAhead; ++j)
                        buf_load<T, K>(rs, b0 + j < b1 ? uint32_t(at[j]) * uint32_t(K * sizeof(T)) : kOutOfRange, part[j]);
#pragma unroll
                    for (int c = 0; c < K; ++c) qi[c] = part[0][c];
#pragma unroll
                    for (int j = 1; j < kSlabAhead; ++j)
#pragma unroll
                        for (int c = 0; c < K; ++c) qi[c] += part[j][c];
                } else {
#pragma unroll
                    for (int j = 0; j < kSlabAhead; ++j)
#pragma unroll
                        for (int c = 0; c < K; ++c) part[j][c] = qv.Yb[int64_t(at[j]) * K + c];
#pragma unroll
                    for (int c = 0; c < K; ++c) qi[c] = part[0][c];
#pragma unroll
                    for (int j = 1; j < kSlabAhead; ++j) {
                        const T w = b0 + j < b1 ? T(1) : T(0);
#pragma unroll
                        for (int c = 0; c < K; ++c) qi[c] += w * part[j][c];
                    }
                }
            } else {
#pragma unroll
                for (int c = 0; c < K; ++c) qi[c] = T(0);
            }
            for (int32_t sl = b0 + (AHEAD ? kSlabAhead : 0); sl < b1; ++sl) {
                const int64_t a2 = qv.bslot[sl];
#pragma unroll
                for (int c = 0; c < K; ++c) qi[c] += qv.Yb[a2 * K + c];
            }
        } else {
#pragma unroll
            for (int c = 0; c < K; ++c) qi[c] = q[i * K + c];
        }
#pragma unroll
        for (int c = 0; c < K; ++c) {
            const T a = T(alpha[c]);
            const T xi = xv[c] + a * pv[c];
            const T ri = rv[c] - a * qi[c];
            if (!qv.skip_x) x[i * K + c] = xi;
            r[i * K + c] = ri;
            acc[c] += coarse ? 0.0 : double(ri) * double(ri) * double(d);
        }
    }
    __syncthreads();
    block_sum<K>(acc, smem);
    if (threadIdx.x < K) part_rz_next[blockIdx.x * K + threadIdx.x] = acc[threadIdx.x];
}

template <class T, int K, bool MASKED, bool AHEAD = true>
__global__ void __launch_bounds__(256) k_pcg_update(int64_t n, UpdHeadT<T> hd, int64_t nv, double *__restrict__ part_rz_next,
                                                        const T *__restrict__ p, const T *__restrict__ q, T *__restrict__ x, T *__restrict__ r,
                                                        const T *__restrict__ dinv, QViewT<T> qv) {
    __shared__ double smem[16 * 3 * K];
    double alpha[K];
    if (!pcg_update_head<T, K>(hd, p, alpha, smem)) return;
    pcg_update_rows<T, K, MASKED, AHEAD>(0, n, int(gridDim.x), nv, alpha, p, q, x, r, dinv, qv, part_rz_next, smem);
}

template <class T, int K>
__global__ void __launch_bounds__(256) k_pcg_update_x(int64_t n, UpdHeadT<T> hd, const T *__restrict__ p, T *__restrict__ x) {
    __shared__ double smem[16 * 3 * K];
    double alpha[K];
    if (!pcg_update_head<T, K>(hd, p, alpha, smem)) return;
    for (int64_t i = int64_t(blockIdx.x) * blockDim.x + threadIdx.x; i < n; i += int64_t(gridDim.x) * blockDim.x) {
#pragma unroll
        for (int c = 0; c < K; ++c) x[i * K + c] += T(alpha[c]) * p[i * K + c];
    }
}

template <class T, int K>
__device__ __forceinline__ void pcg_update_vertex_rows(const ChebArgsT<T> &ch, const FoldArgsT<T> &fold, int skip_x, const double (&alpha)[K],
                                                       const T *__restrict__ p, const T *__restrict__ q, T *__restrict__ x, const T *__restrict__ r,
                                                       const T *__restrict__ dinv) {
    constexpr int LPR = 8, RPB = 256 / LPR;
    static_assert(K <= LPR, "one column per lane after the transposing reduction");
    const int nb_flat = fold.nb_flat;
    const int sub = threadIdx.x % LPR, grp = threadIdx.x / LPR;
    int idx[K], own[K];
    towner_init<K, LPR>(idx, own, sub);
    const int mycol = idx[0];
    const bool mine = own[0] != 0;
    const T inv_theta = T(ch.inv_theta), c1 = T(fold.c1), c2 = T(fold.c2);
    T al[K], a_mine = T(0);
#pragma unroll
    for (int c = 0; c < K; ++c) { al[c] = T(alpha[c]); a_mine = (c == mycol) ? al[c] : a_mine; }
    const int64_t nv = ch.nv;
    for (int64_t row = int64_t(int(blockIdx.x) - nb_flat) * RPB + grp; row < nv; row += int64_t(int(gridDim.x) - nb_flat) * RPB) {
        const int32_t rs = fold.rowptr[row], re = fold.rowptr[row + 1];
        const int64_t at = row * K + mycol;
        T di = T(0), rn = T(0);
        if (mine) {
            di = dinv[row];
            if (!skip_x) x[at] += a_mine * p[at];
            rn = r[at] - a_mine * q[at];
        }
        T t[K];
#pragma unroll
        for (int c = 0; c < K; ++c) t[c] = T(0);
        for (int32_t pp = rs + sub; pp < re; pp += LPR) {
            const int32_t j = fold.col[pp];
            if (j >= nv) break;
            const T v = fold.val[pp] * dinv[j] * inv_theta;
            const T *rj = r + int64_t(j) * K, *qj = q + int64_t(j) * K;
#pragma unroll
            for (int c = 0; c < K; ++c) t[c] += v * (rj[c] - al[c] * qj[c]);
        }
        TReduce<K, LPR>::run(t, sub);
        if (mine) {
            const T dold = di * rn * inv_theta;
            const T ri = rn - t[0];
            ch.z[at] = dold;
            ch.res[at] = ri;
            fold.d_new[at] = c1 * dold + c2 * di * ri;
            fold.stage[at] = rn;
        }
    }
}

template <class T, int K>
__global__ void __launch_bounds__(256) k_pcg_update_folded(int64_t n, UpdHeadT<T> hd, ChebArgsT<T> ch, double *__restrict__ part_rz_next,
                                                           const T *__restrict__ p, const T *__restrict__ q, T *__restrict__ x, T *__restrict__ r,
                                                           const T *__restrict__ dinv, FoldArgsT<T> fold, int skip_x) {
    __shared__ double smem[16 * 3 * K];
    double alpha[K];
    if (!pcg_update_head<T, K>(hd, p, alpha, smem)) return;
    if (int(blockIdx.x) >= fold.nb_flat) {
        pcg_update_vertex_rows<T, K>(ch, fold, skip_x, alpha, p, q, x, r, dinv);
        return;
    }
    QViewT<T> qv;
    qv.skip_x = skip_x;
    pcg_update_rows<T, K, false, true>(ch.nv, n, fold.nb_flat, ch.nv, alpha, p, q, x, r, dinv, qv, part_rz_next, smem);
}

template <class T, int K>
__global__ void __launch_bounds__(256) k_pcg_update_tile(int64_t n, UpdHeadT<T> hd, int64_t nv, double *__restrict__ part_rz_next,
                                                         const T *__restrict__ p, T *__restrict__ r, const T *__restrict__ dinv, QViewT<T> qv) {
    __shared__ double smem[16 * 3 * K];
    __shared__ double ex_lds[4 * 64 * K];
    double alpha[K], acc[K];
    if (!pcg_update_head<T, K>(hd, p, alpha, smem)) return;
    constexpr uint32_t S = sizeof(T);
    __syncthreads();
    if (threadIdx.x == 0) {
#pragma unroll
        for (int c = 0; c < K; ++c) smem[c] = alpha[c];
    }
    __syncthreads();
    const uint32_t lane = threadIdx.x & 63, wave = threadIdx.x >> 6;
    const uint32_t N = uint32_t(n) * K, NV = uint32_t(nv) * K;
    const rsrc_t rr = make_rsrc(r, uint64_t(N) * S), rd = make_rsrc(dinv, uint64_t(n) * S), rs = make_rsrc(qv.Yb, qv.slab_bytes),
                 r4 = make_rsrc(qv.row4, uint64_t(n) * 16);
    uint32_t rowof[K], colof[K];
    T al[K];
    double accv[K];
#pragma unroll
    for (int t = 0; t < K; ++t) {
        const uint32_t v = 64u * t + lane;
        rowof[t] = v / uint32_t(K); colof[t] = v - rowof[t] * uint32_t(K);
        al[t] = T(smem[colof[t]]); accv[t] = 0.0;
    }
    double *exw = ex_lds + wave * (64 * K);
    const uint32_t nwaves = uint32_t(gridDim.x) * 4u;
    int32_t w4n[4];
    {
        const uint32_t row0 = (uint32_t(blockIdx.x) * 4u + wave) * 64u + lane;
        buf_load<int32_t, 4>(r4, row0 < uint32_t(n) ? row0 * 16u : kOutOfRange, w4n);
    }
    for (uint32_t R0 = (uint32_t(blockIdx.x) * 4u + wave) * 64u; R0 < uint32_t(n); R0 += nwaves * 64u) {
        const uint32_t myrow = R0 + lane;
        int32_t w4[4];
#pragma unroll
        for (int j = 0; j < 4; ++j) w4[j] = myrow < uint32_t(n) ? w4n[j] : -1;
        {
            const uint32_t nrow = myrow + nwaves * 64u;
            buf_load<int32_t, 4>(r4, nrow < uint32_t(n) ? nrow * 16u : kOutOfRange, w4n);
        }
        const uint32_t e0 = R0 * uint32_t(K);
        T rv[K], dv[K], part[K][4];
#pragma unroll
        for (int t = 0; t < K; ++t) {
            const uint32_t e = e0 + 64u * t + lane;
            T one[1];
            buf_load<T, 1>(rr, e < N ? e * S : kOutOfRange, one);
            rv[t] = one[0];
            buf_load<T, 1>(rd, e < N ? (R0 + rowof[t]) * S : kOutOfRange, one);
            dv[t] = one[0];
#pragma unroll
            for (int j = 0; j < 4; ++j) {
                const int32_t sj = __builtin_amdgcn_ds_bpermute(int(rowof[t] << 2), w4[j]);
                buf_load<T, 1>(rs, sj >= 0 ? (uint32_t(sj) * uint32_t(K) + colof[t]) * S : kOutOfRange, one);
                part[t][j] = one[0];
            }
        }
        const bool more = w4[3] == -2;
        const bool any_more = __builtin_amdgcn_ballot_w64(more) != 0;
        if (any_more) {
#pragma unroll
            for (int c = 0; c < K; ++c) exw[lane * K + c] = 0.0;
            if (more) {
                const int32_t c0 = qv.bptr[myrow], c1 = qv.bptr[myrow + 1];
                for (int32_t sl = c0 + 3; sl < c1; ++sl) {
                    const int64_t a2 = qv.bslot[sl];
#pragma unroll
                    for (int c = 0; c < K; ++c) exw[lane * K + c] += double(qv.Yb[a2 * K + c]);
                }
            }
            asm volatile("s_waitcnt lgkmcnt(0)" ::: "memory");
        }
#pragma unroll
        for (int t = 0; t < K; ++t) {
            const uint32_t e = e0 + 64u * t + lane;
            T qi = part[t][0];
#pragma unroll
            for (int j = 1; j < 4; ++j) qi += part[t][j];
            if (any_more) qi += T(exw[64 * t + lane]);
            const T ri = rv[t] - al[t] * qi;
            T one[1] = {ri};
            buf_store<T, 1>(rr, e < N ? e * S : kOutOfRange, one);
            accv[t] += (e < NV || e >= N) ? 0.0 : double(ri) * double(ri) * double(dv[t]);
        }
        if (any_more) asm volatile("s_waitcnt lgkmcnt(0)" ::: "memory");
    }
#pragma unroll
// ... 53 lines not shown
            if (!FIRST) { dold_in = d_old[at]; z_in = zc[at]; res_in = res[at]; }
        }
        TC t[K];
#pragma unroll
        for (int c = 0; c < K; ++c) t[c] = TC(0);
        if constexpr (ELL) {
#pragma unroll
            for (int u = 0; u < NE; ++u) {
                const int32_t j = ej[u];
                const TC v = FIRST ? ev[u] * dinv[j] * inv_theta : ev[u];
                if (FIRST) {
                    const T *dj = r + int64_t(j) * K;
#pragma unroll
                    for (int c = 0; c < K; ++c) t[c] += v * TC(dj[c]);
                } else {
                    const TC *dj = d_old + int64_t(j) * K;
#pragma unroll
                    for (int c = 0; c < K; ++c) t[c] += v * dj[c];
                }
            }
        }
        for (int32_t p = rs + sub; p < re; p += LPR) {
            const int32_t j = col[p];
            if (j >= nv) break;
            const TC v = FIRST ? val[p] * dinv[j] * inv_theta : val[p];
            if (FIRST) {
                const T *dj = r + int64_t(j) * K;
#pragma unroll
                for (int c = 0; c < K; ++c) t[c] += v * TC(dj[c]);
            } else {
                const TC *dj = d_old + int64_t(j) * K;
#pragma unroll
                for (int c = 0; c < K; ++c) t[c] += v * dj[c];
            }
        }
        TReduce<K, LPR>::run(t, sub);
        if (mine) {
            const TC dold = FIRST ? di * TC(rr) * inv_theta : dold_in;
            TC zi = FIRST ? dold : z_in + dold;
            const TC ri = (FIRST ? TC(rr) : res_in) - t[0];
            const TC dn = c1 * dold + c2 * di * ri;
            if (LAST == 2) zi += dn;
            if (LAST) z[at] = T(zi / di);
            else {
                zc[at] = zi;
                res[at] = ri;
                d_new[at] = dn;
            }
            if (LAST) dot += double(rr) * double(zi);
        }
    }
    if (LAST) {
        __shared__ double smem[16 * K];
        double dcol[K];
#pragma unroll
        for (int c = 0; c < K; ++c) dcol[c] = (mine && c == mycol) ? dot : 0.0;
        block_sum<K>(dcol, smem);
#pragma unroll
        for (int c = 0; c < K; ++c)
            if (threadIdx.x == c) part[blockIdx.x * K + c] = dcol[c];
    }
}


template <int K>
__device__ __forceinline__ bool pcg_direction_head(int step, double tol2, int nb_rz, const double *__restrict__ part_rz_new, double *__restrict__ scal,
                                                   double (&beta)[K], double (&alpha)[K], double *smem ) {
    if (solve_done(scal, step)) return false;
    double rzn[K];
    reduce_partials<K>(part_rz_new, nb_rz, rzn, smem);
#pragma unroll
    for (int c = 0; c < K; ++c) {
        const double pq = scal[8 + c], rzo = scal[16 + 8 * (step & 1) + c];
        const bool live = (rzo > tol2 * scal[c]) && (rzo > scal[kFloorSlot + c]) && (pq > 0.0);
        beta[c] = live ? rzn[c] / rzo : 0.0;
        alpha[c] = live ? rzo / pq : 0.0;
    }
    if (blockIdx.x == 0 && threadIdx.x == 0)
#pragma unroll
        for (int c = 0; c < K; ++c) scal[16 + 8 * ((step + 1) & 1) + c] = rzn[c];
    return true;
}

template <class T, int K>
__global__ void __launch_bounds__(256) k_pcg_direction_flat(int64_t n, int first, int step, double tol2, int nb_rz, ChebArgsT<T> ch,
                                                            const double *__restrict__ part_rz_new, double *__restrict__ scal,
                                                            const T *__restrict__ r, T *__restrict__ p,
                                                            const T *__restrict__ dinv, T *__restrict__ x) {
    __shared__ double smem[16 * K];
    double beta[K], alpha[K];
    if (!pcg_direction_head<K>(step, tol2, nb_rz, part_rz_new, scal, beta, alpha, smem)) return;
    constexpr int VEC = 16 / int(sizeof(T));
    constexpr uint32_t S = sizeof(T);
    constexpr int UF = 4;
    __syncthreads();
    if (threadIdx.x == 0) {
#pragma unroll
        for (int c = 0; c < K; ++c) { smem[c] = beta[c]; smem[K + c] = alpha[c]; }
    }
    __syncthreads();
    const uint32_t N = uint32_t(n) * K, NV = uint32_t(ch.nv) * K;
    const rsrc_t rr = make_rsrc(r, uint64_t(N) * S), rz = make_rsrc(ch.z, uint64_t(NV) * S), rp = make_rsrc(p, uint64_t(N) * S),
                 rd = make_rsrc(dinv, uint64_t(n) * S), rx = make_rsrc(x ? x : p, uint64_t(N) * S);
    const bool with_x = x != nullptr && !first;
    const uint32_t span = uint32_t(gridDim.x) * blockDim.x * VEC;
    for (uint32_t g0 = (uint32_t(blockIdx.x) * blockDim.x + threadIdx.x) * VEC; g0 < N; g0 += UF * span) {
        T zv[UF][VEC], pv[UF][VEC], xv[UF][VEC], dv[UF][VEC];
#pragma unroll
        for (int u = 0; u < UF; ++u) {
            const uint32_t e0 = g0 + u * span;
            const uint32_t off = e0 < N ? e0 * S : kOutOfRange;
            buf_load<T, VEC>(rr, off, zv[u]);
            {
                T zz[VEC];
                buf_load<T, VEC>(rz, e0 < NV ? e0 * S : kOutOfRange, zz);
#pragma unroll
                for (int v = 0; v < VEC; ++v) zv[u][v] = (e0 + v < NV) ? zz[v] : zv[u][v];
            }
#pragma unroll
            for (int v = 0; v < VEC; ++v) {
                T one[1];
                buf_load<T, 1>(rd, e0 < N ? ((e0 + v) / uint32_t(K)) * S : kOutOfRange, one);
                dv[u][v] = one[0];
            }
            if (!first) buf_load<T, VEC>(rp, off, pv[u]);
            else {
#pragma unroll
                for (int v = 0; v < VEC; ++v) pv[u][v] = T(0);
            }
            if (with_x) buf_load<T, VEC>(rx, off, xv[u]);
            else {
#pragma unroll
                for (int v = 0; v < VEC; ++v) xv[u][v] = T(0);
            }
        }
#pragma unroll
        for (int u = 0; u < UF; ++u) {
            const uint32_t e0 = g0 + u * span;
            const uint32_t off = e0 < N ? e0 * S : kOutOfRange;
            T pn[VEC], xn[VEC];
#pragma unroll
            for (int v = 0; v < VEC; ++v) {
                const uint32_t c = (e0 + v) % uint32_t(K);
                const T zi = dv[u][v] * zv[u][v];
                pn[v] = first ? zi : zi + T(smem[c]) * pv[u][v];
                xn[v] = xv[u][v] + T(smem[K + c]) * pv[u][v];
            }
            buf_store<T, VEC>(rp, off, pn);
            if (with_x) buf_store<T, VEC>(rx, off, xn);
        }
    }
}

#ifndef REMO_DIR_U
#define REMO_DIR_U 4
#endif
template <class T, int K>
__global__ void __launch_bounds__(256) k_pcg_direction_row(int64_t n, int first, int step, double tol2, int nb_rz, ChebArgsT<T> ch,
                                                           const double *__restrict__ part_rz_new, double *__restrict__ scal,
                                                           const T *__restrict__ r, T *__restrict__ p,
                                                           const T *__restrict__ dinv, T *__restrict__ x) {
    __shared__ double smem[16 * K];
    double beta[K], alpha[K];
    if (first) {
        if (solve_done(scal, step)) return;
#pragma unroll
        for (int c = 0; c < K; ++c) { beta[c] = 0.0; alpha[c] = 0.0; }
    } else if (!pcg_direction_head<K>(step, tol2, nb_rz, part_rz_new, scal, beta, alpha, smem)) {
        return;
    }
    constexpr int U = REMO_DIR_U;
    const int64_t stride = int64_t(gridDim.x) * blockDim.x;
    for (int64_t i0 = int64_t(blockIdx.x) * blockDim.x + threadIdx.x; i0 < n; i0 += U * stride) {
        T d[U], zv[U][K], pv[U][K], xv[U][K];
#pragma unroll
        for (int u = 0; u < U; ++u) {
            const int64_t i = i0 + u * stride;
            d[u] = T(0);
#pragma unroll
            for (int c = 0; c < K; ++c) { zv[u][c] = T(0); pv[u][c] = T(0); xv[u][c] = T(0); }
            if (i < n) {
                d[u] = dinv[i];
                const T *src = (i < ch.nv) ? ch.z : r;
#pragma unroll
                for (int c = 0; c < K; ++c) zv[u][c] = src[i * K + c];
                if (!first)
#pragma unroll
                    for (int c = 0; c < K; ++c) pv[u][c] = p[i * K + c];
                if (x && !first)
#pragma unroll
                    for (int c = 0; c < K; ++c) xv[u][c] = x[i * K + c];
            }
        }
#pragma unroll
        for (int u = 0; u < U; ++u) {
            const int64_t i = i0 + u * stride;
            if (i < n)
#pragma unroll
                for (int c = 0; c < K; ++c) {
                    const T zi = d[u] * zv[u][c];
                    p[i * K + c] = first ? zi : zi + T(beta[c]) * pv[u][c];
                    if (x && !first) x[i * K + c] = xv[u][c] + T(alpha[c]) * pv[u][c];
                }
        }
    }
}

template <int K>
__global__ void __launch_bounds__(256) k_pcg_final(int step, int nb_rz, const double *__restrict__ part_rz, const double *__restrict__ scal,
                                                   PcgProgress *progress, int progress_len) {
    __shared__ double smem[16 * K];
    if (solve_done(scal, step)) return;
    double rz[K];
    reduce_partials<K>(part_rz, nb_rz, rz, smem);
    if (threadIdx.x == 0) publish_progress(progress + (step % (progress_len - 1)), rz, K, step);
}

template <class T, int K, int LPR, bool FIRST, bool LAST>
__global__ void __launch_bounds__(256) k_cheb_pair(int64_t nv, const int32_t *__restrict__ rowptr, const int32_t *__restrict__ col,
                                                   const T *__restrict__ va, const T *__restrict__ vb, const T *__restrict__ dinv,
                                                   const T *__restrict__ w_old, T *__restrict__ w_new, T *__restrict__ z, double ab_sum_, double ab_prod_,
                                                   const T *__restrict__ r, double *__restrict__ part, const double *__restrict__ scal, int step) {
    constexpr int RPB = 256 / LPR, U = 2;
    static_assert(K <= LPR, "one column per lane after the transposing reduction");
    if (solve_done(scal, step)) return;
    const T ab_sum = T(ab_sum_), ab_prod = T(ab_prod_);
    const int sub = threadIdx.x % LPR, grp = threadIdx.x / LPR;
    int idx[K], own[K];
    towner_init<K, LPR>(idx, own, sub);
    const int mycol = idx[0];
    const bool mine = own[0] != 0;
    double dot = 0.0;
    for (int64_t row = int64_t(blockIdx.x) * RPB + grp; row < nv; row += int64_t(gridDim.x) * RPB) {
        const int32_t rs = rowptr[row], re = rowptr[row + 1];
        const int64_t at = row * K + mycol;
        T di = T(0), wi = T(0), zi = T(0), rr = T(0);
        if (mine) {
            di = dinv[row];
            if (FIRST || LAST) rr = r[at];
            wi = FIRST ? di * rr : w_old[at];
            if (!FIRST) zi = z[at];
        }
        T t1[K], t2[K];
#pragma unroll
        for (int c = 0; c < K; ++c) { t1[c] = T(0); t2[c] = T(0); }
        for (int32_t p0 = rs + sub; p0 < re; p0 += U * LPR) {
            int32_t j[U];
            T a[U], b[U], w[U][K];
#pragma unroll
            for (int u = 0; u < U; ++u) {
                const int32_t p = p0 + u * LPR;
                j[u] = -1; a[u] = T(0); b[u] = T(0);
                if (p < re) { j[u] = col[p]; a[u] = va[p]; b[u] = vb[p]; }
            }
#pragma unroll
            for (int u = 0; u < U; ++u) {
#pragma unroll
                for (int c = 0; c < K; ++c) w[u][c] = T(0);
                if (j[u] >= 0) {
                    const T *wj = (FIRST ? r : w_old) + int64_t(j[u]) * K;
                    const T dj = FIRST ? dinv[j[u]] : T(1);
#pragma unroll
                    for (int c = 0; c < K; ++c) w[u][c] = FIRST ? dj * wj[c] : wj[c];
                }
            }
#pragma unroll
            for (int u = 0; u < U; ++u)
#pragma unroll
                for (int c = 0; c < K; ++c) { t1[c] += a[u] * w[u][c]; t2[c] += b[u] * w[u][c]; }
        }
        TReduce<K, LPR>::run(t1, sub);
        TReduce<K, LPR>::run(t2, sub);
        if (mine) {
            const T zn = zi + ab_sum * wi - ab_prod * di * t1[0];
            z[at] = LAST ? zn / di : zn;
            if (!LAST) w_new[at] = wi - ab_sum * di * t1[0] + ab_prod * di * t2[0];
            if (LAST) dot += double(rr) * double(zn);
        }
    }
    if (LAST) {
        __shared__ double smem[16 * K];
        double dcol[K];
#pragma unroll
        for (int c = 0; c < K; ++c) dcol[c] = (mine && c == mycol) ? dot : 0.0;
        block_sum<K>(dcol, smem);
#pragma unroll
        for (int c = 0; c < K; ++c)
            if (threadIdx.x == c) part[blockIdx.x * K + c] = dcol[c];
    }
}
// ... 58 lines not shown
                return;
            }
        }
        launch_amg_cycle<T, T>(*b.amg, k, step, (const T *)b.r, b.cz, part_slot + int64_t(b.nb_vec) * k, cheb_grid(b.nv_coarse), (const double *)b.rz0, s);
        return;
    }
    if (b.sq_rowptr && (b.cheb_degree & 1) == 0) {
        const double theta = 0.5 * (b.cheb_lmax + b.cheb_lmin), delta = 0.5 * (b.cheb_lmax - b.cheb_lmin);
        const int m = b.cheb_degree, np = m / 2;
        const int g_last = cheb_grid(b.nv_coarse);
        double *part = part_slot + int64_t(b.nb_vec) * k;
        for (int j = 0; j < np; ++j) {
            const double r1 = theta - delta * cos(M_PI * (2.0 * (j + 1) - 1.0) / (2.0 * m));
            const double r2 = theta - delta * cos(M_PI * (2.0 * (m - j) - 1.0) / (2.0 * m));
            const double a = 1.0 / r1, bb = 1.0 / r2;
            const T *wold = b.cd[j & 1];
            T *wnew = b.cd[(j + 1) & 1];
            const bool first = (j == 0), last = (j + 1 == np);
            auto grid_for = [&](int lpr) { int64_t gg = (b.nv_coarse + 256 / lpr - 1) / (256 / lpr); if (last && gg > g_last) gg = g_last; if (gg > 4096) gg = 4096; return int(gg); };
#define REMO_CHEB2(LPRV, F, L)                                                                                                                        \
    REMO_K_SWITCH(k, hipLaunchKernelGGL((k_cheb_pair<T, KK, LPRV, F, L>), dim3(grid_for(LPRV)), dim3(256), 0, s, b.nv_coarse, b.sq_rowptr, b.sq_col, b.sq_a, \
                                        b.sq_b, b.dinv, wold, wnew, b.cz, a + bb, a * bb, b.r, part, b.rz0, step))
#define REMO_CHEB2_FL(LPRV)                                 \
    if (first && last) { REMO_CHEB2(LPRV, true, true); }    \
    else if (first) { REMO_CHEB2(LPRV, true, false); }      \
    else if (last) { REMO_CHEB2(LPRV, false, true); }       \
    else { REMO_CHEB2(LPRV, false, false); }
            if (b.sq_lanes >= 32) { REMO_CHEB2_FL(32) }
            else if (b.sq_lanes >= 16) { REMO_CHEB2_FL(16) }
            else { REMO_CHEB2_FL(8) }
#undef REMO_CHEB2_FL
#undef REMO_CHEB2
        }
        return;
    }
    const double theta = 0.5 * (b.cheb_lmax + b.cheb_lmin), delta = 0.5 * (b.cheb_lmax - b.cheb_lmin);
    const double sig = theta / delta, inv_theta = 1.0 / theta;
    double rho = 1.0 / sig;
    const int g = cheb_grid(b.nv_coarse);
    double *part = part_slot + int64_t(b.nb_vec) * k;
    const int launches = b.cheb_degree > 1 ? b.cheb_degree - 1 : 1;
    const int32_t *vrow = b.vb_rowptr ? b.vb_rowptr : A.rowptr, *vcol = b.vb_rowptr ? b.vb_col : A.col;
    const T *vval = b.vb_rowptr ? b.vb_val : A.val;
    const bool chain32 = sizeof(T) == 8 && b.c32_val != nullptr && b.vb_rowptr != nullptr && !first_done;
    const bool ell = b.ell_col != nullptr && b.ell_tail != nullptr && (chain32 ? b.c32_ell_val != nullptr : b.ell_val != nullptr);
    for (int j = 0; j < launches; ++j) {
        const double rho_new = 1.0 / (2.0 * sig - rho);
        const double c1 = rho_new * rho, c2 = 2.0 * rho_new / delta;
        rho = rho_new;
        const T *dold = b.cd[j & 1];
        T *dnew = b.cd[(j + 1) & 1];
        const bool first = (j == 0), last = (j + 1 == launches);
        if (first && first_done) continue;
        const int commit = (first_done && j == 1) ? 1 : 0;
        const int64_t g_rows = (b.nv_coarse + 31) / 32;
        const int gl = last ? g : int(g_rows < 8192 ? g_rows : 8192);
#define REMO_CHEB_E(F, L, E)                                                                                                                        \
    if (chain32) {                                                                                                                                  \
        REMO_K_SWITCH(k, hipLaunchKernelGGL((k_cheb_step<T, float, KK, F, L, E>), dim3(gl), dim3(256), 0, s, b.nv_coarse, E ? b.ell_tail : vrow, vcol, b.c32_val, b.c32_dinv, \
                                            (const float *)b.c32_d[j & 1], b.c32_d[(j + 1) & 1], b.c32_z, b.c32_res, b.cz, c1, c2, inv_theta, b.r, part, b.rz0, 0, step, \
                                            b.ell_col, b.c32_ell_val));                                                                             \
    } else {                                                                                                                                        \
        REMO_K_SWITCH(k, hipLaunchKernelGGL((k_cheb_step<T, T, KK, F, L, E>), dim3(gl), dim3(256), 0, s, b.nv_coarse, E ? b.ell_tail : vrow, vcol, vval, b.dinv, dold, dnew, \
                                            b.cz, b.cres, b.cz, c1, c2, inv_theta, b.r, part, b.rz0, commit, step, b.ell_col, b.ell_val));               \
    }
#define REMO_CHEB(F, L)                \
    if (ell) { REMO_CHEB_E(F, L, true) } \
    else { REMO_CHEB_E(F, L, false) }
        if (first && last) { if (b.cheb_degree == 1) { REMO_CHEB(true, 1); } else { REMO_CHEB(true, 2); } }
        else if (first) { REMO_CHEB(true, 0); }
        else if (last) { REMO_CHEB(false, 2); }
        else { REMO_CHEB(false, 0); }
#undef REMO_CHEB
#undef REMO_CHEB_E
    }
}

template <class T> static int nb_rz(const PcgBuffersT<T> &b) { return b.nb_vec + ((b.cheb_degree > 0 && b.nv_coarse > 0) ? cheb_grid(b.nv_coarse) : 0); }

template <class T> void launch_pcg_init(const CsrViewT<T> &A, int k, const T *f, const PcgBuffersT<T> &b, hipStream_t s) {
    const int64_t n = A.n;
    const int g = b.nb_vec;
    const ChebArgsT<T> ch = cheb_args(b);
    REMO_K_SWITCH(k, hipLaunchKernelGGL((k_pcg_init<T, KK>), dim3(g), dim3(256), 0, s, n, ch, f, b.dinv, b.x, b.r, b.p, b.part_rz));
    launch_cheb(A, k, 0, b, b.part_rz, s);
    if (ch.nv > 0)
        REMO_K_SWITCH(k, hipLaunchKernelGGL((k_pcg_direction_row<T, KK>), dim3(g), dim3(256), 0, s, n, 1, 0, 0.0, nb_rz(b), ch, b.part_rz, b.rz0, b.r, b.p, b.dinv, (T *)nullptr));
}

template <class T> static UpdHeadT<T> update_head(const CsrViewT<T> &A, int step, double tol2, const PcgBuffersT<T> &b) {
    UpdHeadT<T> hd;
    const bool bins = b.pq_bins && b.defer_q && A.patch && !cheb_first_folds(b);
    hd.step = step; hd.tol2 = tol2;
    hd.nb_spmv = bins ? kPqBins : b.nb_spmv; hd.nb_rz = nb_rz(b);
    hd.part_pq = bins ? b.part_pq + (step & 1) * (kPqBins * 8) : b.part_pq;
    hd.part_rz_cur = b.part_rz + (step & 1) * (kMaxPartialBlocks * 8);
    hd.rz0 = b.rz0;
    hd.progress = b.progress; hd.progress_len = b.progress_len;
    hd.clear_bins = bins ? b.part_pq + ((step + 1) & 1) * (kPqBins * 8) : nullptr;
    return hd;
}

template <class T> void launch_pcg_update(const CsrViewT<T> &A, int k, int step, double tol2, const PcgBuffersT<T> &b, hipStream_t s) {
    const int64_t n = A.n;
    const int g = b.nb_vec;
    double *nxt = b.part_rz + ((step + 1) & 1) * (kMaxPartialBlocks * 8);
    constexpr uint64_t kBufferLimit = 0xFFFFF000ull;
    const bool folded = cheb_first_folds(b);
    const bool slab = b.defer_q && A.patch && !folded;
    const bool skip_x = b.x_in_direction;
    uint64_t slab_bytes = 0;
    if (slab && g_slab_masked) {
        const uint64_t bytes = uint64_t(A.patch->t.nslot_cap) * uint64_t(k) * sizeof(T);
        slab_bytes = bytes < kBufferLimit ? bytes : 0;
    }
    const bool masked = slab_bytes != 0;
    const bool tile = g_tile_update && sizeof(T) == 8 && masked && A.patch->t.row4 && skip_x && uint64_t(n) * uint64_t(k) * sizeof(T) < kBufferLimit &&
                      uint64_t(n) * 16 < kBufferLimit;
    const bool one_by_one = kProbes && slab && !g_slab_ahead;
    UpdHeadT<T> hd = update_head(A, step, tol2, b);
    hd.ev = EvSlotsT<T>{b.x_ev_at, b.x_ev, b.x_ev_n};
    const ChebArgsT<T> ch = cheb_args(b);
    QViewT<T> qv;
    qv.skip_x = skip_x ? 1 : 0;
    if (slab) { qv.bptr = A.patch->t.bptr; qv.bslot = A.patch->t.bslot; qv.Yb = A.patch->Yb; }
    if (masked) { qv.slab_bytes = slab_bytes; qv.row4 = A.patch->t.row4; }
    if (folded) {
        FoldArgsT<T> fold;
        const double theta = 0.5 * (b.cheb_lmax + b.cheb_lmin), delta = 0.5 * (b.cheb_lmax - b.cheb_lmin);
        const double sig = theta / delta, rho = 1.0 / sig, rho_new = 1.0 / (2.0 * sig - rho);
        fold.nb_flat = g;
        fold.rowptr = b.vb_rowptr ? b.vb_rowptr : A.rowptr; fold.col = b.vb_rowptr ? b.vb_col : A.col; fold.val = b.vb_rowptr ? b.vb_val : A.val;
        fold.d_new = b.cd[1]; fold.stage = b.cd[0];
        fold.c1 = rho_new * rho; fold.c2 = 2.0 * rho_new / delta;
        const int grid = g + int((b.nv_coarse + 31) / 32);
        REMO_K_SWITCH(k, hipLaunchKernelGGL((k_pcg_update_folded<T, KK>), dim3(grid), dim3(256), 0, s, n, hd, ch, nxt, b.p, b.q, b.x, b.r, b.dinv, fold, qv.skip_x));
    } else if (tile) {
        if constexpr (sizeof(T) == 8) REMO_K_SWITCH(k, hipLaunchKernelGGL((k_pcg_update_tile<T, KK>), dim3(g), dim3(256), 0, s, n, hd, ch.nv, nxt, b.p, b.r, b.dinv, qv));
    } else if (one_by_one) {
        if constexpr (kProbes) REMO_K_SWITCH(k, hipLaunchKernelGGL((k_pcg_update<T, KK, false, false>), dim3(g), dim3(256), 0, s, n, hd, ch.nv, nxt, b.p, b.q, b.x, b.r, b.dinv, qv));
    } else if (masked) {
        REMO_K_SWITCH(k, hipLaunchKernelGGL((k_pcg_update<T, KK, true>), dim3(g), dim3(256), 0, s, n, hd, ch.nv, nxt, b.p, b.q, b.x, b.r, b.dinv, qv));
    } else {
        REMO_K_SWITCH(k, hipLaunchKernelGGL((k_pcg_update<T, KK, false>), dim3(g), dim3(256), 0, s, n, hd, ch.nv, nxt, b.p, b.q, b.x, b.r, b.dinv, qv));
    }
    launch_cheb(A, k, step, b, nxt, s, folded);
}

template <int K>
__global__ void __launch_bounds__(256) k_mixed_replace(int64_t n, int64_t nv, const double *__restrict__ f, const double *__restrict__ q64,
                                                       float *__restrict__ r, const float *__restrict__ dinv, double *__restrict__ part_rz_next,
                                                       const double *__restrict__ scal, int step) {
    __shared__ double smem[16 * K];
    if (solve_done(scal, step)) return;
    double acc[K];
#pragma unroll
    for (int c = 0; c < K; ++c) acc[c] = 0.0;
    for (int64_t i = int64_t(blockIdx.x) * blockDim.x + threadIdx.x; i < n; i += int64_t(gridDim.x) * blockDim.x) {
        const float d = dinv[i];
        const bool coarse = i < nv;
#pragma unroll
        for (int c = 0; c < K; ++c) {
            const float ri = float(f[i * K + c] - q64[i * K + c]);
            r[i * K + c] = ri;
            acc[c] += coarse ? 0.0 : double(ri) * double(ri) * double(d);
        }
    }
    block_sum<K>(acc, smem);
    if (threadIdx.x < K) part_rz_next[blockIdx.x * K + threadIdx.x] = acc[threadIdx.x];
}

void launch_pcg_replace(const CsrViewT<float> &A, const CsrViewT<double> &A64, int k, int step, double tol2, const PcgBuffersT<float> &b,
                        const double *f64, double *x64, double *q64, hipStream_t s) {
    const int64_t n = A.n;
    const int g = b.nb_vec;
    double *nxt = b.part_rz + ((step + 1) & 1) * (kMaxPartialBlocks * 8);
    const ChebArgsT<float> ch = cheb_args(b);
    const UpdHeadT<float> hd = update_head(A, step, tol2, b);
    REMO_K_SWITCH(k, hipLaunchKernelGGL((k_pcg_update_x<float, KK>), dim3(g), dim3(256), 0, s, n, hd, b.p, b.x));
    launch_mixed_accumulate(n * k, x64, b.x, 1, s);
    launch_spmm(A64, k, (const double *)x64, q64, (double *)nullptr, (const double *)nullptr, b.nb_spmv, s, 0);
    REMO_K_SWITCH(k, hipLaunchKernelGGL((k_mixed_replace<KK>), dim3(g), dim3(256), 0, s, n, ch.nv, f64, q64, b.r, b.dinv, nxt, b.rz0, step));
    launch_cheb(A, k, step, b, nxt, s);
}

template <class T> void launch_pcg_direction(const CsrViewT<T> &A, int k, int step, double tol2, const PcgBuffersT<T> &b, hipStream_t s, bool add_x) {
    const int64_t n = A.n;
    const int g = b.nb_vec;
    const double *nw = b.part_rz + ((step + 1) & 1) * (kMaxPartialBlocks * 8);
    const ChebArgsT<T> ch = cheb_args(b);
    T *xp = (add_x && b.x_in_direction) ? b.x : nullptr;
    const bool flat = g_flat_direction && uint64_t(n) * uint64_t(k) * sizeof(T) < 0xFFFFF000ull;
    if (flat) {
        REMO_K_SWITCH(k, hipLaunchKernelGGL((k_pcg_direction_flat<T, KK>), dim3(g), dim3(256), 0, s, n, 0, step, tol2, nb_rz(b), ch, nw, b.rz0, b.r, b.p, b.dinv, xp));
    } else {
        REMO_K_SWITCH(k, hipLaunchKernelGGL((k_pcg_direction_row<T, KK>), dim3(g), dim3(256), 0, s, n, 0, step, tol2, nb_rz(b), ch, nw, b.rz0, b.r, b.p, b.dinv, xp));
    }
}

template <class T> void launch_pcg_final(int k, int step, const PcgBuffersT<T> &b, hipStream_t s) {
    const double *cur = b.part_rz + (step & 1) * (kMaxPartialBlocks * 8);
    REMO_K_SWITCH(k, hipLaunchKernelGGL(k_pcg_final<KK>, dim3(1), dim3(256), 0, s, step, nb_rz(b), cur, b.rz0, b.progress, b.progress_len));
}

#define REMO_INSTANTIATE_PCG(T)                                                                                          \
    template void launch_pcg_init<T>(const CsrViewT<T> &, int, const T *, const PcgBuffersT<T> &, hipStream_t);          \
    template void launch_pcg_update<T>(const CsrViewT<T> &, int, int, double, const PcgBuffersT<T> &, hipStream_t);      \
    template void launch_pcg_direction<T>(const CsrViewT<T> &, int, int, double, const PcgBuffersT<T> &, hipStream_t, bool);   \
    template void launch_pcg_final<T>(int, int, const PcgBuffersT<T> &, hipStream_t);
REMO_INSTANTIATE_PCG(double)
REMO_INSTANTIATE_PCG(float)
#undef REMO_INSTANTIATE_PCG

}
```

remo3d_amd/csrc/remo_debug.hip:

```cpp
#include <limits.h>

#include <algorithm>
#include <vector>

#include "../../include/remo3d_hip_debug.h"
#include "remo_internal.h"
#include "patch.h"

using namespace remo;

namespace remo {
Tune g_tune;
}

extern "C" {

namespace {
__global__ void __launch_bounds__(256) k_stream_read(const double2 *__restrict__ x, int64_t n2, double *__restrict__ out) {
    double a = 0.0, b = 0.0;
    for (int64_t i = int64_t(blockIdx.x) * blockDim.x + threadIdx.x; i < n2; i += int64_t(gridDim.x) * blockDim.x) {
        const double2 v = x[i];
        a += v.x; b += v.y;
    }
    a += b;
// ... 264 lines not shown
            PatchProbe pr(ctx, b, fp32 != 0, size_t(grid) * 8);
            pr.stamped_runs();
            for (int mode = 0; mode <= 3; ++mode) {
                set_patch_mode(mode);
                out16[10 + mode] = pr.timed_us();
            }
            set_patch_mode(0);
            h = pr.stamps();
        }
        for (int i = 0; i < 10; ++i) out16[i] = 0.0;
        long long lo = LLONG_MAX, hi = 0;
        int64_t cnt = 0;
        for (int64_t w = 0; w < grid; ++w) {
            const long long *s8 = h.data() + w * 8;
            if (s8[0] == 0 || s8[7] == 0) continue;
            for (int q = 0; q < 7; ++q) out16[q] += double(s8[q + 1] - s8[q]);
            out16[7] += double(s8[7] - s8[0]);
            lo = std::min(lo, s8[0]); hi = std::max(hi, s8[7]);
            ++cnt;
        }
        for (int q = 0; q < 8; ++q) out16[q] /= double(cnt > 0 ? cnt : 1);
        out16[8] = double(hi - lo);
        out16[9] = double(cnt);
        return REMO_OK;
    } catch (const std::exception &ex) {
        set_patch_mode(0); set_patch_stamps(nullptr);
        return fail(ctx, REMO_ERR_DEVICE, ex.what());
    }
#endif
}

int remo_debug_patch_phases_p(remo_ctx_t *ctx, remo_batch_t *b, int32_t fp32, double *out16) {
    if (!ctx || !b || !out16) return REMO_ERR_ARG;
#ifndef REMO_PROBES
    (void)fp32;
    return fail(ctx, REMO_ERR_ARG, "remo_debug_patch_phases_p: the library was built without -DREMO_PROBES (make -C remo3d_amd/csrc probes)");
#else
    if (int rc = patch_probe_check(ctx, b)) return rc;
    const int64_t slots = 8192;
    try {
        HIP_TRY(hipSetDevice(ctx->device));
        std::vector<long long> h;
        double us = 0.0;
        {
            PatchProbe pr(ctx, b, fp32 != 0, size_t(slots) * 12);
            pr.stamped_runs();
            us = pr.timed_us();
            h = pr.stamps();
        }
        for (int i = 0; i < 16; ++i) out16[i] = 0.0;
        double patches = 0, wgs = 0, longest = 0;
        for (int64_t w = 0; w < slots; ++w) {
            const long long *s12 = h.data() + w * 12;
            if (s12[10] <= 0) continue;
            double tot = 0;
            for (int q = 0; q < 10; ++q) { out16[q] += double(s12[q]); tot += double(s12[q]); }
            patches += double(s12[10]); wgs += 1; longest = std::max(longest, tot);
        }
        for (int q = 0; q < 10; ++q) out16[q] /= (patches > 0 ? patches : 1);
        out16[10] = patches; out16[11] = wgs; out16[12] = longest; out16[13] = us;
        return REMO_OK;
    } catch (const std::exception &ex) {
        set_patch_mode(0); set_patch_stamps(nullptr);
        return fail(ctx, REMO_ERR_DEVICE, ex.what());
    }
#endif
}

int remo_debug_tune(int32_t key, int32_t value) {
    switch (key) {
        case 3: set_spmm_tuning(3, value); return 0;
        case 6: g_tune.square = value; return 0;
        case 9: set_fold_first(value); return 0;
        case 13: g_tune.compact = value; return 0;
        case 15: g_tune.chain32 = value; return 0;
        case 16: g_tune.amg = value; return 0;
        case 17: g_tune.amg32 = value; return 0;
        case 18: set_element_order(value); return 0;
        case 31: set_tile_update(value); return 0;
        case 30: set_flat_direction(value); return 0;
        case 29: set_slab_masked(value); return 0;
        case 25: g_tune.x_in_direction = value; return 0;
        case 39: g_tune.x_ev = value; return 0;
        case 22: g_tune.defer_q = value; return 0;
        case 24: g_tune.ell = value; return 0;
        case 40: set_patch_rounds(value); return 0;
        default: break;
    }
#ifdef REMO_PROBES
    if (key == 7) g_tune.sq_lanes = value;
    else if (key == 8) set_symbolic_tuning(value);
    else if (key == 21) set_patch_mode(value);
    else if (key == 26) set_patch_lean(value);
    else if (key == 27) set_slab_ahead(value);
    else if (key == 28) g_tune.dot_bins = value;
    else if (key == 32) set_patch_spread(value);
    else if (key == 33) set_patch_trim(value);
    else if (key == 34) set_patch_persist(value);
    else if (key == 35) set_patch_wgs_per_xcd(value);
    else if (key == 36) g_tune.extra_apply = value;
    else if (key == 0 || key == 1 || key == 2 || key == 4 || key == 5) set_spmm_tuning(key, value);
    else return -1;
    return 0;
#else
    (void)value;
    return -1;
#endif
}

int remo_debug_sens_timing(remo_ctx_t *ctx, double *out2) {
    if (!ctx || !out2) return REMO_ERR_ARG;
    out2[0] = ctx->sens_ms;
    out2[1] = ctx->sens_bytes;
    return REMO_OK;
}

int remo_debug_sens_group_timing(remo_ctx_t *ctx, double *out4) {
    if (!ctx || !out4) return REMO_ERR_ARG;
    for (int i = 0; i < 4; ++i) out4[i] = ctx->sens_group_ms[i];
    return REMO_OK;
}

int remo_debug_field_timing(remo_ctx_t *ctx, double *out2) {
    if (!ctx || !out2) return REMO_ERR_ARG;
    out2[0] = ctx->field_ms[0];
    out2[1] = ctx->field_ms[1];
    return REMO_OK;
}

int remo_debug_point_location(remo_ctx_t *ctx) { return ctx ? ctx->point_location : REMO_ERR_ARG; }
int remo_debug_secondary_timing(remo_ctx_t *ctx, double *ms) {
    if (!ctx || !ms) return REMO_ERR_ARG;
    *ms = ctx->sec_ms;
    return REMO_OK;
}

}
```

remo3d_amd/csrc/remo_internal.h:

```cpp
#pragma once
#include <hip/hip_runtime.h>
#include <stdint.h>

#include <chrono>
#include <cstdio>
#include <stdexcept>
#include <string>
#include <vector>

#include "../../include/remo3d_hip.h"
#include "kernels.h"
#include "amg.h"
#include "symbolic_gpu.h"

#define HIP_TRY(expr)                                                                                   \
    do {                                                                                                \
        hipError_t e__ = (expr);                                                                        \
        if (e__ != hipSuccess) {                                                                        \
            char buf__[512];                                                                            \
            snprintf(buf__, sizeof buf__, "%s failed: %s (%s:%d)", #expr, hipGetErrorString(e__), __FILE__, __LINE__); \
            throw std::runtime_error(buf__);                                                            \
        }                                                                                               \
    } while (0)

namespace remo {

inline double now_ms() {
    using namespace std::chrono;
    return duration<double, std::milli>(steady_clock::now().time_since_epoch()).count();
}

inline size_t align_up(size_t x, size_t a = 256) { return (x + a - 1) / a * a; }

extern thread_local std::string g_create_error;

bool tensor_ok(int dim, const double *S);

struct Tune {
    int square = 1;
    int sq_lanes = 0;
    int compact = 1;
    int chain32 = 1;
    int amg = 0;
    int amg32 = 1;
    int defer_q = 1;
    int ell = 1;
    int x_in_direction = 1;
    int dot_bins = 1;
    int x_ev = 1;
#ifdef REMO_PROBES
    int extra_apply = 0;
#endif
};
extern Tune g_tune;

struct DeviceTemp {
    std::vector<void *> held;
    DeviceTemp() = default;
    DeviceTemp(const DeviceTemp &) = delete;
    ~DeviceTemp() { for (void *p : held) (void)hipFree(p); }
    template <class T> T *alloc(size_t count) {
        held.push_back(nullptr);
        HIP_TRY(hipMalloc(&held.back(), sizeof(T) * count));
        return static_cast<T *>(held.back());
    }
};

inline PatchOpT<float> patch_view32(const PatchOpT<double> &p) {
    return PatchOpT<float>{p.t, reinterpret_cast<float *>(p.Yb), p.ppart, p.lds_rows};
}

}

struct remo_ctx {
    int device = 0;
    hipStream_t stream = nullptr;
    std::string err;
    remo::Arena ar;
    double *d_M2 = nullptr, *d_M3 = nullptr, *d_M2q = nullptr;
    double *d_B3 = nullptr;
    double sens_ms = 0.0, sens_bytes = 0.0;
    double sens_group_ms[4] = {};
    double field_ms[2] = {};
    hipEvent_t fev[4] = {};
    double sec_ms = 0.0;
    int point_location = 0;
    remo::PcgProgress *progress = nullptr;
    remo::PcgProgress *progress_dev = nullptr;
    int progress_len = 0;
    int32_t *d_err = nullptr;
    hipEvent_t ev[8] = {};
    std::vector<hipEvent_t> spmv_ev;
    uint64_t run_id = 0;
    char *in_pool = nullptr;
    size_t in_cap = 0;
    double floor_stage[REMO_MAX_RHS] = {};

    template <class T> T *take(size_t count) { return ar.lo<T>(count); }
    void reserve(size_t bytes) {
        ar.reset();
        if (bytes <= ar.cap) return;
        HIP_TRY(hipStreamSynchronize(stream));
        if (ar.base) HIP_TRY(hipFree(ar.base));
        ar.base = nullptr;
        ar.cap = 0;
        const size_t want = remo::align_up(bytes + bytes / 4, 4096);
        HIP_TRY(hipMalloc(reinterpret_cast<void **>(&ar.base), want));
        ar.cap = want;
    }
    void ensure_progress(int len) {
        if (len <= progress_len) return;
        if (progress) HIP_TRY(hipHostFree(progress));
        progress = nullptr;
        progress_len = 0;
        HIP_TRY(hipHostMalloc(reinterpret_cast<void **>(&progress), sizeof(remo::PcgProgress) * size_t(len),
                              hipHostMallocMapped | hipHostMallocCoherent));
        HIP_TRY(hipHostGetDevicePointer(reinterpret_cast<void **>(&progress_dev), progress, 0));
        progress_len = len;
    }
};

struct remo_sens_request {
    int n_fun = 0;
    const int32_t *fun_rhs = nullptr, *fun_ptr = nullptr;
    const double *fun_w = nullptr;
    double *J_out = nullptr, *dJ_out = nullptr;
    int32_t n_group = 0;
    const int32_t *group = nullptr;
    double *dJg_out = nullptr;
};

struct remo_field_request {
    int64_t n_pts = 0;
    const double *pts = nullptr;
    int32_t n_frhs = 0;
    const int32_t *field_rhs = nullptr;
    double *u = nullptr, *grad = nullptr, *J = nullptr;
    int32_t *elem = nullptr;
};

struct remo_warm;

struct remo_batch {
    int dim = 0;
    int64_t nv = 0, nt = 0, nbf = 0;
    int n_mat = 0;
    int sigma_comp = 1;
    int n_rhs = 0;
    std::vector<int32_t> src_ptr, eval_ptr;
    std::vector<double> src_p, src_I, eval_p;
    std::vector<double> fun_p;
    double *d_coords = nullptr, *d_sigma = nullptr;
    int32_t *d_mat = nullptr, *d_conn = nullptr, *d_bconn = nullptr;
    uint8_t *d_bdir = nullptr;
    bool pooled = false;
    const remo_sens_request *sens = nullptr;
    remo_warm *warm = nullptr;
    const remo_field_request *field = nullptr;
    bool secondary = false;
    int sec_quad = 0;
    double sec_radius = 0.0;
    std::vector<double> sec_sigma0;
    bool eval_only = false;
    bool has_system = false;
    remo::DeviceSymbolic sym;
    remo::CsrView A{};
    double *d_val = nullptr, *d_dinv = nullptr;
    double *d_x = nullptr, *d_C = nullptr;
    double *d_f = nullptr;
// ... 24 lines not shown
```

remo3d_amd/solver.py:

```python
from __future__ import annotations

import ctypes as C
from typing import Optional

import numpy as np

from . import _lib
from ._lib import RemoOpts, RemoStats, ptr

REMO_OK = 0
REMO_NOT_CONVERGED = 1
REMO_ERR_ARG = -1


class RemoError(RuntimeError):
    def __init__(self, code, msg):
        super().__init__(f"libremo3d_hip error {code}: {msg}")
        self.code = code


def make_opts(preconditioner="multigrid", condense=True, maxsteps=1000, rtol=1e-8, check_every=5,
              time_kernels=False, coarse_degree=0, coarse_ratio=0, precision="fp64", inner_digits=0,
              serialize_solves=False, op="auto", coarse="auto", quadrature="exact", assemble="auto") -> RemoOpts:
    L = _lib.load()
# ... 197 lines not shown
        except Exception:
            pass

    def last_error(self) -> str:
        return (self._L.remo_last_error(self._h) or b"").decode()

    def _one_shot(self, kind, mesh, sigma, sources, evals, opts, raise_on_error, functionals=None, groups=None, n_group=None, warm=None,
                  points=None, field_rhs=None, secondary=None):
        job = secondary is not None or _off_axis([z for (z, _) in sources], evals, [z for (_, z, _) in functionals] if functionals else [])
        (handle, ms, j), sigma, tensor, eval_ptr, keep = _batch_args(self._h, mesh, sigma, sources, evals, job, secondary)
        d, nc = int(mesh.dim), (sigma.shape[1] if tensor else 1)
        out = np.full(int(eval_ptr[-1]), np.nan)
        j.u_out = ptr(out, C.c_double)
        J, grads, field = [], [], []
        if kind == "_field":
            points = _field_points(points, d)
            field_rhs = np.ascontiguousarray(np.arange(len(sources)) if field_rhs is None else field_rhs, dtype=np.int32).ravel()
            n_pts, n_f = points.shape[0], field_rhs.size
            field = [dict(u=np.full((n_f, n_pts), np.nan), grad=np.full((n_f, n_pts, d), np.nan), J=np.full((n_f, n_pts, d), np.nan),
                          elem=np.full(n_pts, -1, dtype=np.int32))]
            j.n_pts, j.pts, j.n_frhs, j.field_rhs = n_pts, ptr(points, C.c_double), n_f, ptr(field_rhs, C.c_int32)
            j.u_f, j.grad_f, j.J_f = (ptr(field[0][name], C.c_double) for name in ("u", "grad", "J"))
            j.elem_f = ptr(field[0]["elem"], C.c_int32)
        elif kind:
            n_fun = len(functionals)
            fun_rhs, fun_ptr, fz, fw = _functional_arrays(functionals, d if job else 0)
            j.n_fun, j.fun_rhs, j.fun_ptr, j.fun_p, j.fun_w = n_fun, ptr(fun_rhs, C.c_int32), ptr(fun_ptr, C.c_int32), ptr(fz, C.c_double), ptr(fw, C.c_double)
            J, grads = [np.full(n_fun, np.nan)], [np.full((n_fun, len(sigma), nc), np.nan)]
            j.J_out, j.dJ_out = ptr(J[0], C.c_double), ptr(grads[0], C.c_double)
            if kind == "_sens_groups":
                groups = np.ascontiguousarray(groups, dtype=np.int32).ravel()
                if groups.size != keep[1][1].shape[0]:
                    raise ValueError("groups must hold one id per element")
                n_group = int(groups.max(initial=-1)) + 1 if n_group is None else int(n_group)
                grads.append(np.full((n_fun, max(n_group, 0), nc), np.nan))
                j.n_group, j.group, j.dJg_out = n_group, ptr(groups, C.c_int32), ptr(grads[1], C.c_double)
            if kind == "_sens_warm":
                j.warm = warm._h
        st = RemoStats()
        o = opts if opts is not None else make_opts()
        if not job:
            entry = getattr(self._L, "remo_solve_batch" + kind + ("_tensor" if tensor else ""))
            rc = entry(handle, ms, *_lib.legacy_args(j, kind), C.byref(o), C.byref(st))
        elif secondary is not None and not _secondary_members(secondary, len(sources))[3]:
            rc, msg = REMO_ERR_ARG, "secondary: sigma0 must be positive and finite (None: the conductivity at the source)"
            if raise_on_error:
                raise RemoError(rc, msg)
        else:
            rc = self._L.remo_solve_job(handle, ms, C.byref(j), C.byref(o), C.byref(st))
        if rc < 0 and raise_on_error:
            raise RemoError(rc, self.last_error())
        potentials = [out[eval_ptr[k]:eval_ptr[k + 1]] for k in range(len(evals))]
        return (potentials, *J, *[_symmetric_gradient(g, d, tensor) for g in grads], *field, st.as_dict(), rc)

    def solve_batch(self, mesh, sigma, sources, evals, opts: Optional[RemoOpts] = None, raise_on_error=True, secondary=None):
        return self._one_shot("", mesh, sigma, sources, evals, opts, raise_on_error, secondary=secondary)

    def solve_batch_sens(self, mesh, sigma, sources, evals, functionals, opts: Optional[RemoOpts] = None, raise_on_error=True,
                         warm: Optional[WarmState] = None):
        if warm is not None:
            return self._one_shot("_sens_warm", mesh, sigma, sources, evals, opts, raise_on_error, functionals, warm=warm)
        return self._one_shot("_sens", mesh, sigma, sources, evals, opts, raise_on_error, functionals)

    def solve_batch_sens_groups(self, mesh, sigma, sources, evals, functionals, groups, n_group=None, opts: Optional[RemoOpts] = None,
                                raise_on_error=True):
        return self._one_shot("_sens_groups", mesh, sigma, sources, evals, opts, raise_on_error, functionals, groups, n_group)

    def solve_batch_field(self, mesh, sigma, sources, evals, points, field_rhs=None, opts: Optional[RemoOpts] = None, raise_on_error=True):
        return self._one_shot("_field", mesh, sigma, sources, evals, opts, raise_on_error, points=points, field_rhs=field_rhs)

    def field_timing(self):
        out = np.zeros(2)
        self._L.remo_debug_field_timing(self._h, ptr(out, C.c_double))
        return float(out[0]), float(out[1])

    def secondary_timing(self) -> float:
        ms = C.c_double(0.0)
        self._L.remo_debug_secondary_timing(self._h, C.byref(ms))
        return float(ms.value)

    def point_location(self) -> int:
        return int(self._L.remo_debug_point_location(self._h))

    def sens_group_timing(self):
        out = np.zeros(4)
        self._L.remo_debug_sens_group_timing(self._h, ptr(out, C.c_double))
        return tuple(float(v) for v in out)

    def sens_timing(self):
        out = np.zeros(2)
        self._L.remo_debug_sens_timing(self._h, ptr(out, C.c_double))
        return float(out[0]), float(out[1])

    def batch(self, mesh, sigma, sources, evals, secondary=None) -> "Batch":
        return Batch(self, mesh, sigma, sources, evals, secondary)


class Batch:

    def __init__(self, ctx: Context, mesh, sigma, sources, evals, secondary=None):
        self.ctx = ctx
        self._L = ctx._L
        job = secondary is not None or _off_axis([z for (z, _) in sources], evals)
        if secondary is not None and not _secondary_members(secondary, len(sources))[3]:
            raise RemoError(REMO_ERR_ARG, "secondary: sigma0 must be positive and finite (None: the conductivity at the source)")
        (handle, ms, j), _, tensor, self._eval_ptr, keep = _batch_args(ctx._h, mesh, sigma, sources, evals, job, secondary)
        h = C.c_void_p()
        if job:
            rc = self._L.remo_batch_create_job(handle, ms, C.byref(j), C.byref(h))
        else:
            rc = (self._L.remo_batch_create_tensor if tensor else self._L.remo_batch_create)(handle, ms, *_lib.legacy_args(j), C.byref(h))
        if rc != 0:
            raise RemoError(rc, ctx.last_error())
        self._h = h
        self.dim = int(mesh.dim)
        self.n_rhs = len(sources)
        self.stats = None

    def run(self, opts: Optional[RemoOpts] = None, raise_on_error=True, ctx: Optional["Context"] = None):
        st = RemoStats()
        o = opts if opts is not None else make_opts()
        if ctx is not None:
            self.ctx = ctx
        rc = self._L.remo_batch_run(self.ctx._h, self._h, C.byref(o), C.byref(st))
        self.stats = st.as_dict()
        if rc < 0 and raise_on_error:
            raise RemoError(rc, self.ctx.last_error())
        return rc

    def fetch(self):
        eval_ptr = self._eval_ptr
        out = np.full(int(eval_ptr[-1]), np.nan)
        rc = self._L.remo_batch_fetch(self.ctx._h, self._h, ptr(out, C.c_double))
        if rc != 0:
            raise RemoError(rc, self.ctx.last_error())
        return [out[eval_ptr[k]:eval_ptr[k + 1]] for k in range(self.n_rhs)]

    def eval(self, rhs: int, z):
        z = np.ascontiguousarray(np.atleast_1d(z), dtype=np.float64)
        out = np.full(z.size, np.nan)
        rc = self._L.remo_batch_eval(self.ctx._h, self._h, int(rhs), z.size, ptr(z, C.c_double), ptr(out, C.c_double))
        if rc != 0:
            raise RemoError(rc, self.ctx.last_error())
        return out

    def field(self, rhs: int, points):
        d = self.dim
        points = _field_points(points, d)
        n = points.shape[0]
        out = dict(u=np.full(n, np.nan), grad=np.full((n, d), np.nan), J=np.full((n, d), np.nan), elem=np.full(n, -1, dtype=np.int32))
        rc = self._L.remo_batch_field(self.ctx._h, self._h, int(rhs), n, ptr(points, C.c_double), ptr(out["u"], C.c_double),
                                      ptr(out["grad"], C.c_double), ptr(out["J"], C.c_double), ptr(out["elem"], C.c_int32))
        if rc != 0:
            raise RemoError(rc, self.ctx.last_error())
        return out

    def system(self):
        s = self.stats
        n, nnz, ndof = int(s["n_free"]), int(s["nnz"]), int(s["n_dof"])
        rowptr = np.zeros(n + 1, dtype=np.int32); col = np.zeros(nnz, dtype=np.int32)
        val = np.zeros(nnz); dinv = np.zeros(n); freeid = np.zeros(ndof, dtype=np.int32)
        rc = self._L.remo_batch_get_system(self.ctx._h, self._h, ptr(rowptr, C.c_int32), ptr(col, C.c_int32),
                                           ptr(val, C.c_double), ptr(dinv, C.c_double), ptr(freeid, C.c_int32))
        if rc != 0:
            raise RemoError(rc, self.ctx.last_error())
        return rowptr, col, val, dinv, freeid
# ... 120 lines not shown
```

Measured before the change: 180.3.

## Store the PCG search direction in fp32 on the eval-only patch path

On the evaluated-values-only path with the patch operator and deferred q, the PCG search direction p is now stored as fp32 instead of fp64. The patch apply, init, direction and update kernels are templated on the direction type and widen p to fp64 in registers, so the products stay in fp64. The goal is to halve the memory traffic for reading and writing p in the bandwidth-bound solver loop, at the cost of rounding the direction to single precision, which can slow convergence or change the iteration count.

```diff
diff --git a/include/remo3d_hip_debug.h b/include/remo3d_hip_debug.h
--- a/include/remo3d_hip_debug.h
+++ b/include/remo3d_hip_debug.h
@@ -24,6 +24,7 @@
 int remo_debug_sens_group_timing(remo_ctx_t *ctx, double *out4);
 int remo_debug_field_timing(remo_ctx_t *ctx, double *out2);
 int remo_debug_point_location(remo_ctx_t *ctx);
+int remo_debug_direction_bytes(remo_ctx_t *ctx);
 int remo_debug_secondary_timing(remo_ctx_t *ctx, double *ms);
 
 int remo_debug_tune(int32_t key, int32_t value);
diff --git a/remo3d_amd/_lib.py b/remo3d_amd/_lib.py
--- a/remo3d_amd/_lib.py
+++ b/remo3d_amd/_lib.py
@@ -66,7 +66,7 @@
            "remo_batch_eval", "remo_batch_get_system", "remo_batch_get_vectors", "remo_batch_apply_coarse", "remo_batch_spmv",
            "remo_host_element_matrix", "remo_host_element_matrix_tensor", "remo_host_sens_element", "remo_host_factor_error", "remo_host_symbolic",
            "remo_solve_job", "remo_batch_create_job", "remo_host_point_shapes", "remo_host_secondary_element"]
-DEBUG_EXPORTS = ["remo_debug_stream", "remo_debug_clock", "remo_debug_device", "remo_debug_cache_gather", "remo_debug_xcc", "remo_debug_tune", "remo_debug_patch_phases", "remo_debug_patch_phases_p", "remo_debug_grid_barrier", "remo_debug_sens_timing", "remo_debug_sens_group_timing", "remo_debug_field_timing", "remo_debug_point_location", "remo_debug_secondary_timing"]
+DEBUG_EXPORTS = ["remo_debug_stream", "remo_debug_clock", "remo_debug_device", "remo_debug_cache_gather", "remo_debug_xcc", "remo_debug_tune", "remo_debug_patch_phases", "remo_debug_patch_phases_p", "remo_debug_grid_barrier", "remo_debug_sens_timing", "remo_debug_sens_group_timing", "remo_debug_field_timing", "remo_debug_point_location", "remo_debug_secondary_timing", "remo_debug_direction_bytes"]
 
 JOB_HEAD = ["n_mat", "sigma", "n_rhs", "src_ptr", "src_p", "src_I", "eval_ptr", "eval_p"]
 _SENS = ["u_out", "n_fun", "fun_rhs", "fun_ptr", "fun_p", "fun_w"]
@@ -129,6 +129,8 @@
     L.remo_debug_field_timing.argtypes = [vp, dp]
     L.remo_debug_point_location.restype = C.c_int
     L.remo_debug_point_location.argtypes = [vp]
+    L.remo_debug_direction_bytes.restype = C.c_int
+    L.remo_debug_direction_bytes.argtypes = [vp]
     L.remo_host_secondary_element.restype = C.c_int
     L.remo_host_secondary_element.argtypes = [C.c_int32, dp, dp, C.c_double, C.c_double, C.c_double, dp, C.c_int32, dp]
     L.remo_debug_secondary_timing.restype = C.c_int
diff --git a/remo3d_amd/csrc/batch_run.hip b/remo3d_amd/csrc/batch_run.hip
--- a/remo3d_amd/csrc/batch_run.hip
+++ b/remo3d_amd/csrc/batch_run.hip
@@ -102,6 +102,7 @@
 struct Plan {
     int kmax = 0;
     bool x_ev_only = false;
+    bool p32 = false;
     bool want_patch = false, want_amg = false;
     int64_t vertex_block_above = -1;
     size_t field_bytes = 0;
@@ -167,6 +168,7 @@
     p.kmax = std::min<int>(std::max(b->n_rhs, b->sens ? b->sens->n_fun : 0), REMO_MAX_RHS);
     p.x_ev_only = b->eval_only && !b->sens && !b->field && g_tune.x_ev && g_tune.x_in_direction && o.precision == 0;
     p.want_patch = dim == 3 && (o.op == 3 || o.op == 0);
+    p.p32 = p.x_ev_only && p.want_patch && g_tune.p32 && g_tune.defer_q;
     p.want_amg = o.preconditioner != 0 && g_tune.amg != 1 &&
                  (g_tune.amg == 2 || o.coarse == 2 || o.coarse == 3 || (o.coarse == 0 && dim == 2 && o.coarse_degree <= 0));
     p.vertex_block_above = (p.want_patch && o.assemble != 1) ? (o.assemble == 2 ? 0 : 200000) : -1;
@@ -257,7 +259,9 @@
     PcgBuffers &buf = sv.buf;
     buf.x = plan.x_ev_only ? nullptr : ctx->take<double>(n * kmax);
     buf.r = ctx->take<double>(n * kmax);
-    buf.p = ctx->take<double>(n * kmax); buf.q = ctx->take<double>(n * kmax);
+    if (plan.p32) buf.p32 = ctx->take<float>(n * kmax + 4);
+    else buf.p = ctx->take<double>(n * kmax);
+    buf.q = ctx->take<double>(n * kmax);
     buf.dinv = sys.d_dinv;
     buf.part_pq = ctx->take<double>(kMaxPartialBlocks * 8);
     buf.part_rz = ctx->take<double>(kMaxPartialBlocks * 8 * 2);
@@ -674,7 +678,7 @@
     return REMO_OK;
 }
 
-void set_launch_shape(const Run &r, const System &sys, bool patch_op, PcgBuffers &buf) {
+void set_launch_shape(const Run &r, const Plan &plan, const System &sys, bool patch_op, PcgBuffers &buf) {
     remo_batch *b = r.b;
     const int lpr = choose_lanes_per_row(sys.n, b->sym.nnz);
     buf.nb_spmv = spmv_grid(sys.n, lpr);
@@ -683,6 +687,11 @@
     buf.x_in_direction = g_tune.x_in_direction != 0;
     buf.pq_bins = buf.defer_q && g_tune.dot_bins != 0;
     if (patch_op) b->patch64.dot_bins = buf.pq_bins;
+    if (buf.p32 && !(patch_op && buf.defer_q && buf.x_in_direction)) {
+        buf.p32 = nullptr;
+        buf.p = r.ctx->take<double>(sys.n * plan.kmax);
+    }
+    r.ctx->direction_bytes = (buf.p32 || r.o.precision == 1) ? 4 : 8;
 }
 
 MixedBuffers mixed_buffers(const Run &r, const Plan &plan, const System &sys, const Solve &sv, const VertexBlock &vb, bool patch_op) {
@@ -1024,7 +1033,7 @@
 
         std::unique_lock<std::mutex> solve_turn(g_solve_mutex, std::defer_lock);
         if (o.serialize_solves) solve_turn.lock();
-        set_launch_shape(r, sys, patch_op, sv.buf);
+        set_launch_shape(r, plan, sys, patch_op, sv.buf);
         const bool mixed = (o.precision == 1);
         MixedBuffers mx;
         if (mixed) mx = mixed_buffers(r, plan, sys, sv, vb, patch_op);
diff --git a/remo3d_amd/csrc/kernels.h b/remo3d_amd/csrc/kernels.h
--- a/remo3d_amd/csrc/kernels.h
+++ b/remo3d_amd/csrc/kernels.h
@@ -44,6 +44,7 @@
     const int64_t *x_ev_at = nullptr;
     T *x_ev = nullptr;
     int x_ev_n = 0;
+    float *p32 = nullptr;
     PcgProgress *progress;
     int progress_len;
     int nb_spmv, nb_vec;
@@ -120,6 +121,7 @@
 template <class T> void launch_spmm(const CsrViewT<T> &A, int k, const T *x, T *y, double *part, const double *scal, int nblocks, hipStream_t s, int step = 0, bool defer = false);
 
 template <class T> void launch_patch_spmm(const CsrViewT<T> &A, int k, const T *x, T *y, double *part, const double *scal, int nblocks, hipStream_t s, int step, bool defer);
+void launch_patch_spmm_x32(const CsrViewT<double> &A, int k, const float *x, double *part, const double *scal, int nblocks, hipStream_t s, int step);
 template <class T> bool pcg_update_folds(const PcgBuffersT<T> &b);
 void set_slab_masked(int v);
 void set_flat_direction(int v);
diff --git a/remo3d_amd/csrc/patch.hip b/remo3d_amd/csrc/patch.hip
--- a/remo3d_amd/csrc/patch.hip
+++ b/remo3d_amd/csrc/patch.hip
@@ -131,10 +131,12 @@
 #define REMO_LEAN_WAVES 5
 #endif
 constexpr int kPatchPasses2 = 20;
-template <class T, int K, int MODE = 0, bool LEAN = false, int ROUNDS = 1>
-__global__ void __launch_bounds__(kPatchBlock, (LEAN ? REMO_LEAN_WAVES : 1)) k_patch_apply(PatchTables tb, int rows, const T *__restrict__ x, T *__restrict__ y, T *__restrict__ Yb,
+template <class T, int K, int MODE = 0, bool LEAN = false, int ROUNDS = 1, class TX = T>
+__global__ void __launch_bounds__(kPatchBlock, (LEAN ? REMO_LEAN_WAVES : 1)) k_patch_apply(PatchTables tb, int rows, const TX *__restrict__ x, T *__restrict__ y, T *__restrict__ Yb,
                                                      double *__restrict__ ppart, const double *__restrict__ scal, int step, long long *__restrict__ stamps,
                                                      double *__restrict__ pbins) {
+    static_assert(std::is_same<TX, T>::value || (std::is_same<TX, float>::value && std::is_same<T, double>::value && MODE == 0 && !LEAN),
+                  "an x narrower than the rest: fp32 into the fp64 product, plain order");
     (void)y;
     int done_word = 0;
     if (scal) done_word = load_as_vector(reinterpret_cast<const int *>(scal + kDoneSlot));
@@ -145,9 +147,9 @@
     constexpr int U = ROUNDS == 2 ? kPatchPasses2 : kPatchPasses;
     constexpr int BLK = kPatchBlock;
     constexpr int EK = BLK / K;
-    constexpr uint32_t S = sizeof(T);
+    constexpr uint32_t S = sizeof(T), SX = sizeof(TX);
     extern __shared__ double lds_raw[];
-    T *xs = reinterpret_cast<T *>(lds_raw);
+    TX *xs = reinterpret_cast<TX *>(lds_raw);
     __shared__ double smem[16 * K];
     const int tid = threadIdx.x;
     const int64_t per = (tb.npatch + 7) >> 3;
@@ -198,7 +200,7 @@
     const int rows_p = (tb.trim && rows_own < rows) ? rows_own : rows;
     const int npass = (rows_p + EK - 1) / EK;
     REMO_STAMP(1)
-    const rsrc_t rx = make_rsrc(x, uint64_t(tb.n) * K * S);
+    const rsrc_t rx = make_rsrc(x, uint64_t(tb.n) * K * SX);
     const uint32_t slack = uint32_t((rows + 1) * K + c0);
 #define REMO_PASSES_UP_TO_12(fn)                                                                                          \
         case 1: fn(std::integral_constant<int, 1>{}, 0); break;   case 2: fn(std::integral_constant<int, 2>{}, 0); break;   \
@@ -229,7 +231,7 @@
     auto stage = [&](auto np_c, int m0) {
         constexpr int NP = decltype(np_c)::value;
         int32_t r[NP];
-        T v[NP][1];
+        TX v[NP][1];
         if (m0 == 0) {
 #pragma unroll
             for (int u = 0; u < NP; ++u) r[u] = r0[u];
@@ -245,12 +247,12 @@
         for (int u = 0; u < NP; ++u) r[u] = (off_mask == 0 && m0 + el + EK * u < rows_own) ? r[u] : -1;
 #pragma unroll
         for (int u = 0; u < NP; ++u)
-            buf_load<T, 1>(rx, r[u] >= 0 ? __umul24(uint32_t(r[u]), K * S) + uint32_t(c0) * S : kOutOfRange, v[u]);
+            buf_load<TX, 1>(rx, r[u] >= 0 ? __umul24(uint32_t(r[u]), K * SX) + uint32_t(c0) * SX : kOutOfRange, v[u]);
 #pragma unroll
         for (int u = 0; u < NP; ++u) xs[r[u] >= 0 ? uint32_t((m0 + el + EK * u) * K + c0) : slack] = v[u][0];
     };
     REMO_PASSES(stage)
-    if (tid < 2 * K) xs[rows * K + tid] = T(0);
+    if (tid < 2 * K) xs[rows * K + tid] = TX(0);
     __syncthreads();
     REMO_STAMP(2)
     double d0 = 0.0;
@@ -336,14 +338,14 @@
         if (active) {
             T xA[20];
 #pragma unroll
-            for (int i = 0; i < 20; ++i) xA[i] = xs[REMO_PATCH_L(i) * K + c0];
+            for (int i = 0; i < 20; ++i) xA[i] = T(xs[REMO_PATCH_L(i) * K + c0]);
             dA = element(xA, cm, yA);
 #pragma unroll
             for (int i = 0; i < 20; ++i) asm volatile("" : "+v"(yA[i]));
         }
         if (activeB) {
 #pragma unroll
-            for (int i = 0; i < 20; ++i) xB[i] = xs[((liB[i >> 1] >> (16 * (i & 1))) & 0xFFFFu) * K + c0];
+            for (int i = 0; i < 20; ++i) xB[i] = T(xs[((liB[i >> 1] >> (16 * (i & 1))) & 0xFFFFu) * K + c0]);
         }
         __syncthreads();
         REMO_STAMP(3)
@@ -362,7 +364,7 @@
     T xv[20];
     if (active) {
 #pragma unroll
-        for (int i = 0; i < 20; ++i) xv[i] = xs[REMO_PATCH_L(i) * K + c0];
+        for (int i = 0; i < 20; ++i) xv[i] = T(xs[REMO_PATCH_L(i) * K + c0]);
     }
     __syncthreads();
     REMO_STAMP(3)
@@ -644,6 +646,33 @@
         default: patch_dispatch<T, 8>(A, x, y, part, scal, step, nb, s, defer); break;
     }
 }
+template <int K> static void patch_dispatch_x32(const CsrViewT<double> &A, const float *x, double *part, const double *scal, int step, int nb, hipStream_t s) {
+    const PatchOpT<double> &P = *A.patch;
+    const PatchTables &tb = P.t;
+    const int64_t per = (tb.npatch + 7) / 8;
+    double *bins = P.dot_bins ? part + (step & 1) * (kPqBins * 8) : nullptr;
+    const size_t bytes = patch_lds_bytes(P.lds_rows, K);
+    if (tb.rounds == 2)
+        hipLaunchKernelGGL((k_patch_apply<double, K, 0, false, 2, float>), dim3(int(per * 8)), dim3(kPatchBlock), bytes, s, tb, P.lds_rows, x, (double *)nullptr, P.Yb, P.ppart, scal, step, (long long *)nullptr, bins);
+    else
+        hipLaunchKernelGGL((k_patch_apply<double, K, 0, false, 1, float>), dim3(int(per * 8)), dim3(kPatchBlock), bytes, s, tb, P.lds_rows, x, (double *)nullptr, P.Yb, P.ppart, scal, step, (long long *)nullptr, bins);
+    if (!bins) hipLaunchKernelGGL(k_patch_dot<K>, dim3(nb < kPatchDotBlocks ? nb : kPatchDotBlocks), dim3(256), 0, s, tb.npatch, (const double *)P.ppart, part, scal, step);
+}
+
+void launch_patch_spmm_x32(const CsrViewT<double> &A, int k, const float *x, double *part, const double *scal, int nb, hipStream_t s, int step) {
+    if (!patch_applies(A, k) || !part) throw std::logic_error("patch operator on an fp32 direction: no patch tables for this batch");
+    switch (k) {
+        case 1: patch_dispatch_x32<1>(A, x, part, scal, step, nb, s); break;
+        case 2: patch_dispatch_x32<2>(A, x, part, scal, step, nb, s); break;
+        case 3: patch_dispatch_x32<3>(A, x, part, scal, step, nb, s); break;
+        case 4: patch_dispatch_x32<4>(A, x, part, scal, step, nb, s); break;
+        case 5: patch_dispatch_x32<5>(A, x, part, scal, step, nb, s); break;
+        case 6: patch_dispatch_x32<6>(A, x, part, scal, step, nb, s); break;
+        case 7: patch_dispatch_x32<7>(A, x, part, scal, step, nb, s); break;
+        default: patch_dispatch_x32<8>(A, x, part, scal, step, nb, s); break;
+    }
+}
+
 template void launch_patch_spmm<double>(const CsrViewT<double> &, int, const double *, double *, double *, const double *, int, hipStream_t, int, bool);
 template void launch_patch_spmm<float>(const CsrViewT<float> &, int, const float *, float *, double *, const double *, int, hipStream_t, int, bool);
 
diff --git a/remo3d_amd/csrc/pcg_host.hip b/remo3d_amd/csrc/pcg_host.hip
--- a/remo3d_amd/csrc/pcg_host.hip
+++ b/remo3d_amd/csrc/pcg_host.hip
@@ -40,17 +40,26 @@
     volatile int32_t *done_step = &ctx->progress[ctx->progress_len - 1].step;
     int step = 0;
     bool done = false;
+    auto apply = [&]() {
+        if constexpr (std::is_same<T, double>::value) {
+            if (buf.p32) {
+                launch_patch_spmm_x32(A, k, (const float *)buf.p32, buf.part_pq, (const double *)buf.rz0, buf.nb_spmv, s, step);
+                return;
+            }
+        }
+        launch_spmm(A, k, (const T *)buf.p, buf.q, buf.part_pq, (const double *)buf.rz0, buf.nb_spmv, s, step, buf.defer_q);
+    };
     for (; step < maxit && !done;) {
         if (time_kernels > 0 && (step % time_kernels) == (time_kernels / 2) && ev_used + 2 <= ctx->spmv_ev.size()) {
             HIP_TRY(hipEventRecord(ctx->spmv_ev[ev_used], s));
-            launch_spmm(A, k, (const T *)buf.p, buf.q, buf.part_pq, (const double *)buf.rz0, buf.nb_spmv, s, step, buf.defer_q);
+            apply();
             HIP_TRY(hipEventRecord(ctx->spmv_ev[ev_used + 1], s));
             ev_used += 2;
         } else {
-            launch_spmm(A, k, (const T *)buf.p, buf.q, buf.part_pq, (const double *)buf.rz0, buf.nb_spmv, s, step, buf.defer_q);
+            apply();
         }
 #ifdef REMO_PROBES
-        for (int extra = 0; extra < g_tune.extra_apply; ++extra)
+        for (int extra = 0; extra < g_tune.extra_apply && buf.p; ++extra)
             launch_spmm(A, k, (const T *)buf.p, buf.q, (double *)nullptr, (const double *)buf.rz0, buf.nb_spmv, s, step, false);
 #endif
         bool replaced = false;
diff --git a/remo3d_amd/csrc/pcg_kernels.hip b/remo3d_amd/csrc/pcg_kernels.hip
--- a/remo3d_amd/csrc/pcg_kernels.hip
+++ b/remo3d_amd/csrc/pcg_kernels.hip
@@ -2,6 +2,9 @@
 #include "amg.h"
 
 #include <math.h>
+
+#include <stdexcept>
+#include <type_traits>
 
 #include "wave_util.h"
 #include "kutil.h"
@@ -59,9 +62,9 @@
 };
 constexpr int kFloorSlot = 5 * 8;
 
-template <class T, int K>
+template <class T, int K, class TP = T>
 __global__ void __launch_bounds__(256) k_pcg_init(int64_t n, ChebArgsT<T> ch, const T *__restrict__ f, const T *__restrict__ dinv,
-                                                  T *__restrict__ x, T *__restrict__ r, T *__restrict__ p,
+                                                  T *__restrict__ x, T *__restrict__ r, TP *__restrict__ p,
                                                   double *__restrict__ part_rz) {
     __shared__ double smem[16 * K];
     double rz[K];
@@ -76,7 +79,7 @@
             const T zi = d * ri;
             if (x) x[i * K + c] = T(0);
             r[i * K + c] = ri;
-            p[i * K + c] = coarse ? T(0) : zi;
+            p[i * K + c] = TP(coarse ? T(0) : zi);
             rz[c] += coarse ? 0.0 : double(ri) * double(zi);
         }
     }
@@ -85,8 +88,8 @@
 }
 
 
-template <class T, int K>
-__device__ __forceinline__ bool pcg_update_head(const UpdHeadT<T> &hd, const T *__restrict__ p, double (&alpha)[K], double *smem ) {
+template <class T, int K, class TP = T>
+__device__ __forceinline__ bool pcg_update_head(const UpdHeadT<T> &hd, const TP *__restrict__ p, double (&alpha)[K], double *smem ) {
     double *scal = hd.rz0;
     const int step = hd.step;
     if (solve_done(scal, step)) return false;
@@ -129,7 +132,7 @@
         double a = 0.0;
 #pragma unroll
         for (int c = 0; c < K; ++c) a = (c == col) ? alpha[c] : a;
-        const T xv = hd.ev.x[j], pv = p[at];
+        const T xv = hd.ev.x[j], pv = T(p[at]);
         hd.ev.x[j] = xv + T(a) * pv;
     }
     return true;
@@ -228,6 +231,16 @@
     double alpha[K];
     if (!pcg_update_head<T, K>(hd, p, alpha, smem)) return;
     pcg_update_rows<T, K, MASKED, AHEAD>(0, n, int(gridDim.x), nv, alpha, p, q, x, r, dinv, qv, part_rz_next, smem);
+}
+
+template <int K, bool MASKED>
+__global__ void __launch_bounds__(256) k_pcg_update_p32(int64_t n, UpdHeadT<double> hd, int64_t nv, double *__restrict__ part_rz_next,
+                                                        const float *__restrict__ p, const double *__restrict__ q, double *__restrict__ r,
+                                                        const double *__restrict__ dinv, QViewT<double> qv) {
+    __shared__ double smem[16 * 3 * K];
+    double alpha[K];
+    if (!pcg_update_head<double, K, float>(hd, p, alpha, smem)) return;
+    pcg_update_rows<double, K, MASKED, true>(0, n, int(gridDim.x), nv, alpha, (const double *)nullptr, q, (double *)nullptr, r, dinv, qv, part_rz_next, smem);
 }
 
 template <class T, int K>
@@ -306,13 +319,13 @@
     pcg_update_rows<T, K, false, true>(ch.nv, n, fold.nb_flat, ch.nv, alpha, p, q, x, r, dinv, qv, part_rz_next, smem);
 }
 
-template <class T, int K>
+template <class T, int K, class TP = T>
 __global__ void __launch_bounds__(256) k_pcg_update_tile(int64_t n, UpdHeadT<T> hd, int64_t nv, double *__restrict__ part_rz_next,
-                                                         const T *__restrict__ p, T *__restrict__ r, const T *__restrict__ dinv, QViewT<T> qv) {
+                                                         const TP *__restrict__ p, T *__restrict__ r, const T *__restrict__ dinv, QViewT<T> qv) {
     __shared__ double smem[16 * 3 * K];
     __shared__ double ex_lds[4 * 64 * K];
     double alpha[K], acc[K];
-    if (!pcg_update_head<T, K>(hd, p, alpha, smem)) return;
+    if (!pcg_update_head<T, K, TP>(hd, p, alpha, smem)) return;
     constexpr uint32_t S = sizeof(T);
     __syncthreads();
     if (threadIdx.x == 0) {
@@ -532,16 +545,19 @@
     return true;
 }
 
-template <class T, int K>
+template <class T, int K, class TP = T>
 __global__ void __launch_bounds__(256) k_pcg_direction_flat(int64_t n, int first, int step, double tol2, int nb_rz, ChebArgsT<T> ch,
                                                             const double *__restrict__ part_rz_new, double *__restrict__ scal,
-                                                            const T *__restrict__ r, T *__restrict__ p,
+                                                            const T *__restrict__ r, TP *__restrict__ p,
                                                             const T *__restrict__ dinv, T *__restrict__ x) {
     __shared__ double smem[16 * K];
     double beta[K], alpha[K];
     if (!pcg_direction_head<K>(step, tol2, nb_rz, part_rz_new, scal, beta, alpha, smem)) return;
-    constexpr int VEC = 16 / int(sizeof(T));
-    constexpr uint32_t S = sizeof(T);
+    constexpr bool SAME = std::is_same<TP, T>::value;
+    constexpr int VEC = 16 / int(sizeof(TP));
+    constexpr int RV = 16 / int(sizeof(T));
+    constexpr int NR = VEC / RV;
+    constexpr uint32_t S = sizeof(T), SP = sizeof(TP);
     constexpr int UF = 4;
     __syncthreads();
     if (threadIdx.x == 0) {
@@ -550,22 +566,26 @@
     }
     __syncthreads();
     const uint32_t N = uint32_t(n) * K, NV = uint32_t(ch.nv) * K;
-    const rsrc_t rr = make_rsrc(r, uint64_t(N) * S), rz = make_rsrc(ch.z, uint64_t(NV) * S), rp = make_rsrc(p, uint64_t(N) * S),
-                 rd = make_rsrc(dinv, uint64_t(n) * S), rx = make_rsrc(x ? x : p, uint64_t(N) * S);
-    const bool with_x = x != nullptr && !first;
+    const rsrc_t rr = make_rsrc(r, uint64_t(N) * S), rz = make_rsrc(ch.z, uint64_t(NV) * S), rp = make_rsrc(p, uint64_t(N) * SP),
+                 rd = make_rsrc(dinv, uint64_t(n) * S), rx = make_rsrc((SAME && x) ? (const void *)x : (const void *)p, uint64_t(N) * S);
+    const bool with_x = SAME && x != nullptr && !first;
     const uint32_t span = uint32_t(gridDim.x) * blockDim.x * VEC;
     for (uint32_t g0 = (uint32_t(blockIdx.x) * blockDim.x + threadIdx.x) * VEC; g0 < N; g0 += UF * span) {
-        T zv[UF][VEC], pv[UF][VEC], xv[UF][VEC], dv[UF][VEC];
+        T zv[UF][VEC], xv[UF][VEC], dv[UF][VEC];
+        TP pv[UF][VEC];
 #pragma unroll
         for (int u = 0; u < UF; ++u) {
             const uint32_t e0 = g0 + u * span;
-            const uint32_t off = e0 < N ? e0 * S : kOutOfRange;
-            buf_load<T, VEC>(rr, off, zv[u]);
-            {
-                T zz[VEC];
-                buf_load<T, VEC>(rz, e0 < NV ? e0 * S : kOutOfRange, zz);
-#pragma unroll
-                for (int v = 0; v < VEC; ++v) zv[u][v] = (e0 + v < NV) ? zz[v] : zv[u][v];
+            const uint32_t off = e0 < N ? e0 * SP : kOutOfRange;
+#pragma unroll
+            for (int j = 0; j < NR; ++j) {
+                const uint32_t ej = e0 + uint32_t(RV * j);
+                T rj[RV];
+                buf_load<T, RV>(rr, ej < N ? ej * S : kOutOfRange, rj);
+                T zz[RV];
+                buf_load<T, RV>(rz, ej < NV ? ej * S : kOutOfRange, zz);
+#pragma unroll
+                for (int v = 0; v < RV; ++v) zv[u][RV * j + v] = (ej + v < NV) ? zz[v] : rj[v];
             }
 #pragma unroll
             for (int v = 0; v < VEC; ++v) {
@@ -573,10 +593,10 @@
                 buf_load<T, 1>(rd, e0 < N ? ((e0 + v) / uint32_t(K)) * S : kOutOfRange, one);
                 dv[u][v] = one[0];
             }
-            if (!first) buf_load<T, VEC>(rp, off, pv[u]);
+            if (!first) buf_load<TP, VEC>(rp, off, pv[u]);
             else {
 #pragma unroll
-                for (int v = 0; v < VEC; ++v) pv[u][v] = T(0);
+                for (int v = 0; v < VEC; ++v) pv[u][v] = TP(0);
             }
             if (with_x) buf_load<T, VEC>(rx, off, xv[u]);
             else {
@@ -587,28 +607,28 @@
 #pragma unroll
         for (int u = 0; u < UF; ++u) {
             const uint32_t e0 = g0 + u * span;
-            const uint32_t off = e0 < N ? e0 * S : kOutOfRange;
-            T pn[VEC], xn[VEC];
+            const uint32_t off = e0 < N ? e0 * SP : kOutOfRange;
+            TP pn[VEC];
+            T xn[VEC];
 #pragma unroll
             for (int v = 0; v < VEC; ++v) {
                 const uint32_t c = (e0 + v) % uint32_t(K);
-                const T zi = dv[u][v] * zv[u][v];
-                pn[v] = first ? zi : zi + T(smem[c]) * pv[u][v];
-                xn[v] = xv[u][v] + T(smem[K + c]) * pv[u][v];
-            }
-            buf_store<T, VEC>(rp, off, pn);
+                const T zi = dv[u][v] * zv[u][v], po = T(pv[u][v]);
+                pn[v] = TP(first ? zi : zi + T(smem[c]) * po);
+                xn[v] = xv[u][v] + T(smem[K + c]) * po;
+            }
+            buf_store<TP, VEC>(rp, off, pn);
             if (with_x) buf_store<T, VEC>(rx, off, xn);
         }
     }
 }
-
 #ifndef REMO_DIR_U
 #define REMO_DIR_U 4
 #endif
-template <class T, int K>
+template <class T, int K, class TP = T>
 __global__ void __launch_bounds__(256) k_pcg_direction_row(int64_t n, int first, int step, double tol2, int nb_rz, ChebArgsT<T> ch,
                                                            const double *__restrict__ part_rz_new, double *__restrict__ scal,
-                                                           const T *__restrict__ r, T *__restrict__ p,
+                                                           const T *__restrict__ r, TP *__restrict__ p,
                                                            const T *__restrict__ dinv, T *__restrict__ x) {
     __shared__ double smem[16 * K];
     double beta[K], alpha[K];
@@ -636,7 +656,7 @@
                 for (int c = 0; c < K; ++c) zv[u][c] = src[i * K + c];
                 if (!first)
 #pragma unroll
-                    for (int c = 0; c < K; ++c) pv[u][c] = p[i * K + c];
+                    for (int c = 0; c < K; ++c) pv[u][c] = T(p[i * K + c]);
                 if (x && !first)
 #pragma unroll
                     for (int c = 0; c < K; ++c) xv[u][c] = x[i * K + c];
@@ -649,13 +669,12 @@
 #pragma unroll
                 for (int c = 0; c < K; ++c) {
                     const T zi = d[u] * zv[u][c];
-                    p[i * K + c] = first ? zi : zi + T(beta[c]) * pv[u][c];
+                    p[i * K + c] = TP(first ? zi : zi + T(beta[c]) * pv[u][c]);
                     if (x && !first) x[i * K + c] = xv[u][c] + T(alpha[c]) * pv[u][c];
                 }
         }
     }
 }
-
 template <int K>
 __global__ void __launch_bounds__(256) k_pcg_final(int step, int nb_rz, const double *__restrict__ part_rz, const double *__restrict__ scal,
                                                    PcgProgress *progress, int progress_len) {
@@ -880,6 +899,15 @@
     const int64_t n = A.n;
     const int g = b.nb_vec;
     const ChebArgsT<T> ch = cheb_args(b);
+    if constexpr (sizeof(T) == 8) {
+        if (b.p32) {
+            REMO_K_SWITCH(k, hipLaunchKernelGGL((k_pcg_init<double, KK, float>), dim3(g), dim3(256), 0, s, n, ch, f, b.dinv, b.x, b.r, b.p32, b.part_rz));
+            launch_cheb(A, k, 0, b, b.part_rz, s);
+            if (ch.nv > 0)
+                REMO_K_SWITCH(k, hipLaunchKernelGGL((k_pcg_direction_row<double, KK, float>), dim3(g), dim3(256), 0, s, n, 1, 0, 0.0, nb_rz(b), ch, b.part_rz, b.rz0, b.r, b.p32, b.dinv, (double *)nullptr));
+            return;
+        }
+    }
     REMO_K_SWITCH(k, hipLaunchKernelGGL((k_pcg_init<T, KK>), dim3(g), dim3(256), 0, s, n, ch, f, b.dinv, b.x, b.r, b.p, b.part_rz));
     launch_cheb(A, k, 0, b, b.part_rz, s);
     if (ch.nv > 0)
@@ -923,6 +951,16 @@
     qv.skip_x = skip_x ? 1 : 0;
     if (slab) { qv.bptr = A.patch->t.bptr; qv.bslot = A.patch->t.bslot; qv.Yb = A.patch->Yb; }
     if (masked) { qv.slab_bytes = slab_bytes; qv.row4 = A.patch->t.row4; }
+    if constexpr (sizeof(T) == 8) {
+        if (b.p32) {
+            if (!slab || !skip_x || b.x || one_by_one) throw std::logic_error("update launch: an fp32 search direction outside the evaluated-values path of the patch operator");
+            if (tile) { REMO_K_SWITCH(k, hipLaunchKernelGGL((k_pcg_update_tile<double, KK, float>), dim3(g), dim3(256), 0, s, n, hd, ch.nv, nxt, b.p32, b.r, b.dinv, qv)); }
+            else if (masked) { REMO_K_SWITCH(k, hipLaunchKernelGGL((k_pcg_update_p32<KK, true>), dim3(g), dim3(256), 0, s, n, hd, ch.nv, nxt, b.p32, b.q, b.r, b.dinv, qv)); }
+            else { REMO_K_SWITCH(k, hipLaunchKernelGGL((k_pcg_update_p32<KK, false>), dim3(g), dim3(256), 0, s, n, hd, ch.nv, nxt, b.p32, b.q, b.r, b.dinv, qv)); }
+            launch_cheb(A, k, step, b, nxt, s, false);
+            return;
+        }
+    }
     if (folded) {
         FoldArgsT<T> fold;
         const double theta = 0.5 * (b.cheb_lmax + b.cheb_lmin), delta = 0.5 * (b.cheb_lmax - b.cheb_lmin);
@@ -989,6 +1027,13 @@
     const ChebArgsT<T> ch = cheb_args(b);
     T *xp = (add_x && b.x_in_direction) ? b.x : nullptr;
     const bool flat = g_flat_direction && uint64_t(n) * uint64_t(k) * sizeof(T) < 0xFFFFF000ull;
+    if constexpr (sizeof(T) == 8) {
+        if (b.p32) {
+            if (flat) { REMO_K_SWITCH(k, hipLaunchKernelGGL((k_pcg_direction_flat<double, KK, float>), dim3(g), dim3(256), 0, s, n, 0, step, tol2, nb_rz(b), ch, nw, b.rz0, b.r, b.p32, b.dinv, (double *)nullptr)); }
+            else { REMO_K_SWITCH(k, hipLaunchKernelGGL((k_pcg_direction_row<double, KK, float>), dim3(g), dim3(256), 0, s, n, 0, step, tol2, nb_rz(b), ch, nw, b.rz0, b.r, b.p32, b.dinv, (double *)nullptr)); }
+            return;
+        }
+    }
     if (flat) {
         REMO_K_SWITCH(k, hipLaunchKernelGGL((k_pcg_direction_flat<T, KK>), dim3(g), dim3(256), 0, s, n, 0, step, tol2, nb_rz(b), ch, nw, b.rz0, b.r, b.p, b.dinv, xp));
     } else {
diff --git a/remo3d_amd/csrc/remo_debug.hip b/remo3d_amd/csrc/remo_debug.hip
--- a/remo3d_amd/csrc/remo_debug.hip
+++ b/remo3d_amd/csrc/remo_debug.hip
@@ -370,6 +370,7 @@
         case 29: set_slab_masked(value); return 0;
         case 25: g_tune.x_in_direction = value; return 0;
         case 39: g_tune.x_ev = value; return 0;
+        case 41: g_tune.p32 = value; return 0;
         case 22: g_tune.defer_q = value; return 0;
         case 24: g_tune.ell = value; return 0;
         case 40: set_patch_rounds(value); return 0;
@@ -417,6 +418,7 @@
 }
 
 int remo_debug_point_location(remo_ctx_t *ctx) { return ctx ? ctx->point_location : REMO_ERR_ARG; }
+int remo_debug_direction_bytes(remo_ctx_t *ctx) { return ctx ? ctx->direction_bytes : REMO_ERR_ARG; }
 int remo_debug_secondary_timing(remo_ctx_t *ctx, double *ms) {
     if (!ctx || !ms) return REMO_ERR_ARG;
     *ms = ctx->sec_ms;
diff --git a/remo3d_amd/csrc/remo_internal.h b/remo3d_amd/csrc/remo_internal.h
--- a/remo3d_amd/csrc/remo_internal.h
+++ b/remo3d_amd/csrc/remo_internal.h
@@ -48,6 +48,7 @@
     int x_in_direction = 1;
     int dot_bins = 1;
     int x_ev = 1;
+    int p32 = 1;
 #ifdef REMO_PROBES
     int extra_apply = 0;
 #endif
@@ -85,6 +86,7 @@
     hipEvent_t fev[4] = {};
     double sec_ms = 0.0;
     int point_location = 0;
+    int direction_bytes = 0;
     remo::PcgProgress *progress = nullptr;
     remo::PcgProgress *progress_dev = nullptr;
     int progress_len = 0;
diff --git a/remo3d_amd/solver.py b/remo3d_amd/solver.py
--- a/remo3d_amd/solver.py
+++ b/remo3d_amd/solver.py
@@ -303,6 +303,9 @@
     def point_location(self) -> int:
         return int(self._L.remo_debug_point_location(self._h))
 
+    def direction_bytes(self) -> int:
+        return int(self._L.remo_debug_direction_bytes(self._h))
+
     def sens_group_timing(self):
         out = np.zeros(4)
         self._L.remo_debug_sens_group_timing(self._h, ptr(out, C.c_double))
```

Measured after the change: 191.0, median of 6. 1.06x the previous value.
